# Veason-silverbullet/NNR

Hardware: NVIDIA B200
Metric: cne_sue_train_impressions_per_sec (higher is better)
Workload: dtype f32

## Files before the change

### include/nnr_b200.h

```cpp
#ifndef NNR_B200_H
#define NNR_B200_H
#include <stddef.h>
#include <stdint.h>

#ifdef __cplusplus
extern "C" {
#endif

#define NNR_ABI_VERSION 8
#define NNR_SEED_INDIRECT (1ULL << 62)

const char* nnr_last_error(void);
int nnr_abi_version(void);
uint64_t nnr_launch_count(void);
int nnr_profile_enable(int on);
int nnr_profile_read(double* out, int ntags);

int nnr_seq_prepare(uint8_t* mask, int N, int L, int32_t* len, int32_t* off, int32_t* tok_row,
                    void* stream);

int nnr_embed_gather_fwd(const float* table, const int32_t* ids, const int32_t* len,
                         const int32_t* off, int N, int L, int E, int V, float* out, float p_drop,
                         uint64_t seed, void* stream);
int nnr_embed_gather_planes_fwd(const float* table, const int32_t* ids, const int32_t* len,
                                const int32_t* off, int N, int L, int E, int V, int cap, float p_drop,
                                uint64_t seed, int algo, void* planes, size_t planes_bytes, void* stream);
size_t nnr_embed_gather_bwd_workspace_bytes(int N, int L);
int nnr_embed_gather_bwd(const float* dout, const int32_t* ids, const int32_t* len,
                         const int32_t* off, int N, int L, int E, int V, float p_drop,
                         uint64_t seed, float* dtable, int accumulate, void* workspace,
                         size_t workspace_bytes, void* stream);

enum {
  NNR_EPI_NONE = 0,
  NNR_EPI_BIAS = 1,
  NNR_EPI_BIAS_TANH = 2,
  NNR_EPI_BIAS_RELU_RES = 3,
  NNR_EPI_GATE = 4,
  NNR_EPI_ADD_AUX = 5
};
enum {
  NNR_GEMM_AUTO = 0,
  NNR_GEMM_SIMT_FP32 = 1,
  NNR_GEMM_TC_TF32X3 = 2,
  NNR_GEMM_TC_BF16 = 3,
  NNR_GEMM_TC_BF16X3 = 4
};
typedef struct {
  const float* A; int64_t lda; int32_t transA;
  const float* B; int64_t ldb; int32_t transB;
  float* C; int64_t ldc;
  int32_t M, N, K;
  const int32_t* m_dev;
  const int32_t* k_dev;
  int32_t epilogue;
  int32_t accumulate;
  const float* bias;
  const float* aux; int64_t ldaux;
  float* aux_out; int64_t ldaux_out;
  const float* rowbias; int64_t ldrowbias; const int32_t* rowmap;
  float p_drop; uint64_t seed;
  int32_t algo;
  void* workspace; size_t workspace_bytes;
  const void* A_planes; int64_t a_planes_pitch; int64_t a_planes_rows;
  const void* B_planes; int64_t b_planes_pitch; int64_t b_planes_rows;
  void* C_planes; int64_t c_planes_pitch; int64_t c_planes_rows;
} nnr_gemm_args;
size_t nnr_gemm_workspace_bytes(const nnr_gemm_args* args);
int nnr_gemm(const nnr_gemm_args* args, void* stream);
int64_t nnr_tc_split_pitch(int C, int algo);
size_t nnr_tc_split_bytes(int R, int C, int algo);
int nnr_tc_split(const float* X, int64_t ld, int R, int C, const int32_t* r_dev, int algo, void* planes,
                 size_t planes_bytes, void* stream);
typedef struct nnr_split_desc {
  const float* src; int64_t ld; int32_t rows, cols;
  void* planes; int64_t pitch;
} nnr_split_desc;
int nnr_tc_split_many(const nnr_split_desc* descs, int n, int algo, void* stream);

int nnr_length_sort_desc(const int64_t* keys, int N, int max_key, int64_t* sorted_idx, void* stream);

size_t nnr_tc_split_colsum_workspace_bytes(int R, int C, int algo);
int nnr_tc_split_colsum(const float* X, int64_t ld, int R, int C, const int32_t* r_dev, int algo, void* planes,
                        size_t planes_bytes, float* colsum, int accumulate, void* workspace, size_t workspace_bytes,
                        void* stream);
int nnr_relu_bwd_split_colsum(const float* dy, const float* relu_out, int64_t ld, int R, int C, float p_drop,
                              uint64_t seed, float* dy_dropped, int algo, void* planes, size_t planes_bytes,
                              float* colsum, int accumulate, void* workspace, size_t workspace_bytes,
                              void* stream);
int nnr_gemm_default_algo(void);

size_t nnr_colsum_workspace_bytes(int M, int N);
int nnr_colsum(const float* X, int64_t ldx, int M, int N, const int32_t* m_dev, float* out,
               int accumulate, void* workspace, size_t workspace_bytes, void* stream);
int nnr_segment_colsum(const float* X, int64_t ldx, const int32_t* off, int N, int D, float* out,
                       int64_t ldo, void* stream);

int nnr_lstm_fwd(float* gx, const float* w_hh, const int32_t* len, const int32_t* off,
                 const int32_t* order, int N, int L, int H, float* h_out, float* c_stash,
                 float* c_n, int32_t* tile_counters, void* stream);
int nnr_lstm_bwd(float* gates, const float* c_stash, const float* w_hh, const int32_t* len,
                 const int32_t* off, const int32_t* order, int N, int L, int H, const float* dh,
                 const float* dcn, int32_t* tile_counters, void* stream);
int nnr_lstm_fwd_planes_supported(int H, int algo);
int nnr_lstm_fwd_planes(float* gx, const float* w_hh, const int32_t* len, const int32_t* off, const int32_t* order,
                        int N, int L, int H, float* h_out, float* c_stash, float* c_n, int32_t* tile_counters, int cap,
                        int algo, void* planes, size_t planes_bytes, void* stream);
int nnr_lstm_bwd_planes_supported(int H, int algo);
size_t nnr_lstm_bwd_planes_workspace_bytes(int N, int H);
int nnr_lstm_bwd_planes(const float* gates, const float* c_stash, const float* w_hh, const int32_t* len,
                        const int32_t* off, const int32_t* order, int N, int L, int H, const float* dh,
                        const float* dcn, int32_t* tile_counters, int cap, int algo, void* dz_planes,
                        size_t planes_bytes, float* db, void* workspace, size_t workspace_bytes, void* stream);
int nnr_lstm_shift_h(const float* h, const int32_t* len, const int32_t* off,
                     const int32_t* tok_row, int N, int L, int H, float* hprev, void* stream);
int nnr_lstm_shift_h_planes(const float* h, const int32_t* len, const int32_t* off,
                            const int32_t* tok_row, int N, int L, int H, int cap, int algo, void* planes,
                            size_t planes_bytes, void* stream);
int nnr_gate_bwd_pre(const float* dhg, const float* h, const float* g, int64_t n_max,
                     const int32_t* n_dev, int D, float* dz, float* dh0, void* stream);
int nnr_gate_bwd_planes(const float* dhg, const float* h, const float* g, const int32_t* off, int N, int D,
                        int cap, int algo, void* dz_planes, size_t planes_bytes, float* dh0, float* dmproj,
                        int64_t lddm, void* stream);

typedef struct {
  const float* X; int64_t ldx; int32_t D;
  const int32_t* seg_off; int32_t S; int32_t fixed_len; int32_t max_len;
  int32_t mode;
  const float* U; int64_t ldu; int32_t A; const float* w2;
  const float* qvec; int64_t ldq; float scale;
  const uint8_t* mask;
  float* pooled; int64_t ldp;
  float* alpha;
  const float* dpooled; int64_t lddp;
  float* dX; int64_t lddx; int32_t accumulate_dx;
  float* dU; int64_t lddu;
  float* dw2_partial;
  float* dqvec; int64_t lddq;
  const int32_t* seg_order;
} nnr_pool_args;
int nnr_attn_pool_fwd(const nnr_pool_args* args, void* stream);
int nnr_attn_pool_bwd(const nnr_pool_args* args, void* stream);

int nnr_news_fuse_fwd(const float* t_self, const float* t_cross, const float* c_self,
                      const float* c_cross, const float* cat_table, const float* sub_table,
                      const int32_t* cat, const int32_t* sub, int N, int D2, int Ec, int Es,
                      float p_drop, uint64_t seed, float* out, void* stream);
int nnr_news_fuse_bwd(const float* dout, const int32_t* cat, const int32_t* sub, int N, int D2,
                      int Ec, int Es, int n_cat, int n_sub, float p_drop, uint64_t seed,
                      float* d_a, float* d_b, float* dcat_table, float* dsub_table,
                      int accumulate, void* stream);
int nnr_news_fuse_tables_bwd(const float* dout, const int32_t* cat, const int32_t* sub, int N, int Dout, int col0,
// ... 75 lines not shown
```

### nnr_b200/_lib.py

```python
import ctypes as C
import os

_HERE = os.path.dirname(os.path.abspath(__file__))
LIB_PATH = os.environ.get('NNR_B200_LIB') or os.path.join(_HERE, '_lib', 'libnnr_b200.so')

if not os.path.isfile(LIB_PATH):
    raise ImportError('nnr_b200: CUDA library not built (%s missing). Run nnr_b200/csrc/build.sh or '
                      '__graft_entry__.build(); there is no CPU fallback.' % LIB_PATH)

lib = C.CDLL(LIB_PATH)

vp, i32, i64, u64, f32, sz = C.c_void_p, C.c_int32, C.c_int64, C.c_uint64, C.c_float, C.c_size_t


class GemmArgs(C.Structure):
    _fields_ = [('A', vp), ('lda', i64), ('transA', i32),
                ('B', vp), ('ldb', i64), ('transB', i32),
                ('C', vp), ('ldc', i64),
                ('M', i32), ('N', i32), ('K', i32),
                ('m_dev', vp), ('k_dev', vp),
                ('epilogue', i32), ('accumulate', i32),
                ('bias', vp), ('aux', vp), ('ldaux', i64),
                ('aux_out', vp), ('ldaux_out', i64),
                ('rowbias', vp), ('ldrowbias', i64), ('rowmap', vp),
                ('p_drop', f32), ('seed', u64),
                ('algo', i32),
                ('workspace', vp), ('workspace_bytes', sz),
                ('A_planes', vp), ('a_planes_pitch', i64), ('a_planes_rows', i64),
                ('B_planes', vp), ('b_planes_pitch', i64), ('b_planes_rows', i64),
                ('C_planes', vp), ('c_planes_pitch', i64), ('c_planes_rows', i64)]


class PoolArgs(C.Structure):
    _fields_ = [('X', vp), ('ldx', i64), ('D', i32),
                ('seg_off', vp), ('S', i32), ('fixed_len', i32), ('max_len', i32),
                ('mode', i32),
                ('U', vp), ('ldu', i64), ('A', i32), ('w2', vp),
                ('qvec', vp), ('ldq', i64), ('scale', f32),
                ('mask', vp),
                ('pooled', vp), ('ldp', i64),
                ('alpha', vp),
                ('dpooled', vp), ('lddp', i64),
                ('dX', vp), ('lddx', i64), ('accumulate_dx', i32),
                ('dU', vp), ('lddu', i64),
                ('dw2_partial', vp),
                ('dqvec', vp), ('lddq', i64),
                ('seg_order', vp)]


class SplitDesc(C.Structure):
    _fields_ = [('src', vp), ('ld', i64), ('rows', i32), ('cols', i32), ('planes', vp), ('pitch', i64)]


SIGNATURES = {
    'nnr_last_error': (C.c_char_p, []),
    'nnr_abi_version': (C.c_int, []),
    'nnr_launch_count': (u64, []),
    'nnr_profile_enable': (C.c_int, [C.c_int]),
    'nnr_profile_read': (C.c_int, [C.POINTER(C.c_double), C.c_int]),
    'nnr_seq_prepare': (C.c_int, [vp, C.c_int, C.c_int, vp, vp, vp, vp]),
    'nnr_embed_gather_fwd': (C.c_int, [vp, vp, vp, vp, C.c_int, C.c_int, C.c_int, C.c_int, vp, f32, u64, vp]),
    'nnr_embed_gather_planes_fwd': (C.c_int, [vp, vp, vp, vp, C.c_int, C.c_int, C.c_int, C.c_int, C.c_int, f32, u64, C.c_int, vp, sz, vp]),
    'nnr_embed_gather_bwd_workspace_bytes': (sz, [C.c_int, C.c_int]),
    'nnr_embed_gather_bwd': (C.c_int, [vp, vp, vp, vp, C.c_int, C.c_int, C.c_int, C.c_int, f32, u64, vp, C.c_int, vp, sz, vp]),
    'nnr_gemm_workspace_bytes': (sz, [C.POINTER(GemmArgs)]),
    'nnr_gemm': (C.c_int, [C.POINTER(GemmArgs), vp]),
    'nnr_tc_split_pitch': (i64, [C.c_int, C.c_int]),
    'nnr_tc_split_bytes': (sz, [C.c_int, C.c_int, C.c_int]),
    'nnr_tc_split': (C.c_int, [vp, i64, C.c_int, C.c_int, vp, C.c_int, vp, sz, vp]),
    'nnr_tc_split_colsum_workspace_bytes': (sz, [C.c_int, C.c_int, C.c_int]),
    'nnr_tc_split_colsum': (C.c_int, [vp, i64, C.c_int, C.c_int, vp, C.c_int, vp, sz, vp, C.c_int, vp, sz, vp]),
    'nnr_relu_bwd_split_colsum': (C.c_int, [vp, vp, i64, C.c_int, C.c_int, f32, u64, vp, C.c_int, vp, sz, vp, C.c_int, vp, sz, vp]),
    'nnr_length_sort_desc': (C.c_int, [vp, C.c_int, C.c_int, vp, vp]),
    'nnr_tc_split_many': (C.c_int, [vp, C.c_int, C.c_int, vp]),
    'nnr_gemm_default_algo': (C.c_int, []),
    'nnr_colsum_workspace_bytes': (sz, [C.c_int, C.c_int]),
    'nnr_colsum': (C.c_int, [vp, i64, C.c_int, C.c_int, vp, vp, C.c_int, vp, sz, vp]),
    'nnr_segment_colsum': (C.c_int, [vp, i64, vp, C.c_int, C.c_int, vp, i64, vp]),
    'nnr_lstm_fwd': (C.c_int, [vp, vp, vp, vp, vp, C.c_int, C.c_int, C.c_int, vp, vp, vp, vp, vp]),
    'nnr_lstm_bwd': (C.c_int, [vp, vp, vp, vp, vp, vp, C.c_int, C.c_int, C.c_int, vp, vp, vp, vp]),
    'nnr_lstm_bwd_planes_supported': (C.c_int, [C.c_int, C.c_int]),
    'nnr_lstm_fwd_planes_supported': (C.c_int, [C.c_int, C.c_int]),
    'nnr_lstm_fwd_planes': (C.c_int, [vp, vp, vp, vp, vp, C.c_int, C.c_int, C.c_int, vp, vp, vp, vp, C.c_int, C.c_int, vp, sz, vp]),
    'nnr_lstm_bwd_planes_workspace_bytes': (sz, [C.c_int, C.c_int]),
    'nnr_lstm_bwd_planes': (C.c_int, [vp, vp, vp, vp, vp, vp, C.c_int, C.c_int, C.c_int, vp, vp, vp, C.c_int, C.c_int, vp, sz, vp,
                                      vp, sz, vp]),
    'nnr_lstm_shift_h_planes': (C.c_int, [vp, vp, vp, vp, C.c_int, C.c_int, C.c_int, C.c_int, C.c_int, vp, sz, vp]),
    'nnr_lstm_shift_h': (C.c_int, [vp, vp, vp, vp, C.c_int, C.c_int, C.c_int, vp, vp]),
    'nnr_gate_bwd_planes': (C.c_int, [vp, vp, vp, vp, C.c_int, C.c_int, C.c_int, C.c_int, vp, sz, vp, vp, i64, vp]),
    'nnr_gate_bwd_pre': (C.c_int, [vp, vp, vp, i64, vp, C.c_int, vp, vp, vp]),
    'nnr_attn_pool_fwd': (C.c_int, [C.POINTER(PoolArgs), vp]),
    'nnr_attn_pool_bwd': (C.c_int, [C.POINTER(PoolArgs), vp]),
    'nnr_news_fuse_fwd': (C.c_int, [vp, vp, vp, vp, vp, vp, vp, vp, C.c_int, C.c_int, C.c_int, C.c_int, f32, u64, vp, vp]),
    'nnr_news_fuse_bwd': (C.c_int, [vp, vp, vp, C.c_int, C.c_int, C.c_int, C.c_int, C.c_int, C.c_int, f32, u64, vp, vp, vp, vp, C.c_int, vp]),
    'nnr_news_fuse_tables_bwd': (C.c_int, [vp, vp, vp, C.c_int, C.c_int, C.c_int, C.c_int, C.c_int, C.c_int, C.c_int, f32, u64, vp, vp, C.c_int, vp]),
    'nnr_sue_graph_build': (C.c_int, [vp, vp, C.c_int, C.c_int, C.c_int, vp, vp, vp, vp]),
    'nnr_sue_graph_build_ex': (C.c_int, [vp, vp, C.c_int, C.c_int, C.c_int, C.c_int, vp, vp, vp, vp]),
    'nnr_ln_relu_res_fwd': (C.c_int, [vp, vp, vp, vp, C.c_int, C.c_int, f32, f32, u64, vp, vp, vp, vp, vp]),
    'nnr_ln_relu_res_bwd_workspace_bytes': (sz, [C.c_int, C.c_int]),
    'nnr_ln_relu_res_bwd': (C.c_int, [vp, vp, vp, vp, vp, vp, C.c_int, C.c_int, f32, u64, vp, vp, vp, vp, vp, sz, vp]),
    'nnr_graph_to_csr': (C.c_int, [vp, C.c_int, C.c_int, C.c_int, vp, vp, vp, vp]),
    'nnr_gcn_aggregate': (C.c_int, [vp, vp, vp, vp, C.c_int, C.c_int, C.c_int, vp, vp]),
    'nnr_gcn_aggregate_add': (C.c_int, [vp, vp, vp, vp, C.c_int, C.c_int, C.c_int, vp, vp, vp]),
    'nnr_cluster_intra_fwd': (C.c_int, [vp, vp, vp, vp, C.c_int, C.c_int, C.c_int, C.c_int, C.c_int, C.c_int, f32, vp, vp, vp]),
    'nnr_cluster_intra_bwd': (C.c_int, [vp, vp, vp, vp, vp, vp, C.c_int, C.c_int, C.c_int, C.c_int, C.c_int, C.c_int, f32, vp, vp, vp, vp, C.c_int, vp]),
    'nnr_rowdot_fwd': (C.c_int, [vp, vp, C.c_int, C.c_int, vp, vp]),
    'nnr_rowdot_bwd': (C.c_int, [vp, vp, vp, C.c_int, C.c_int, vp, C.c_int, vp, C.c_int, vp]),
    'nnr_topk_merge': (C.c_int, [vp, i64, C.c_int, C.c_int, i64, vp, vp, vp, C.c_int, C.c_int, C.c_int, vp, vp, vp]),
    'nnr_topk_merge_capped': (C.c_int, [vp, i64, C.c_int, C.c_int, i64, vp, vp, vp, C.c_int, C.c_int, C.c_int, vp, C.c_int,
                                        C.c_int, vp, vp, vp, vp]),
    'nnr_topk_merge_lists': (C.c_int, [vp, i64, C.c_int, C.c_int, vp, i64, C.c_int, C.c_int, vp, vp, vp]),
    'nnr_topk_merge_lists_capped': (C.c_int, [vp, i64, C.c_int, C.c_int, vp, i64, vp, i64, C.c_int, C.c_int, C.c_int, C.c_int,
                                              vp, vp, vp, vp]),
    'nnr_dropout': (C.c_int, [vp, i64, f32, u64, vp, vp]),
    'nnr_flat_clip_adam_workspace_bytes': (sz, [i64]),
    'nnr_flat_clip_adam': (C.c_int, [vp, vp, vp, vp, i64, f32, f32, f32, f32, f32, f32, i32, vp, vp, sz, vp]),
    'nnr_flat_clip_adam_dev': (C.c_int, [vp, vp, vp, vp, i64, f32, f32, f32, f32, f32, f32, vp, vp, vp, sz, vp]),
}

for _name, (_res, _args) in SIGNATURES.items():
    _fn = getattr(lib, _name)
    _fn.restype = _res
    _fn.argtypes = _args


def check(rc, what):
    if rc != 0:
        msg = lib.nnr_last_error()
        raise RuntimeError('%s failed (rc=%d): %s' % (what, rc, msg.decode() if msg else ''))


def launch_count():
    return int(lib.nnr_launch_count())
```

### nnr_b200/csrc/gemm_api.cu

```cuda
#include "common.cuh"
#include "../../include/nnr_b200.h"
#include <stdlib.h>
#include <string.h>

size_t nnr_gemm_simt_workspace_bytes(const nnr_gemm_args* a);
int nnr_gemm_simt(const nnr_gemm_args* a, void* stream);
int nnr_gemm_tc_supported(const nnr_gemm_args* a);
size_t nnr_gemm_tc_workspace_bytes(const nnr_gemm_args* a);
int nnr_gemm_tc(const nnr_gemm_args* a, void* stream);

extern "C" int nnr_gemm_default_algo(void);
static int default_algo() {
  static int algo = -1;
  if (algo < 0) {
    const char* e = getenv("NNR_GEMM_ALGO");
    if (e && !strcmp(e, "simt")) algo = NNR_GEMM_SIMT_FP32;
    else if (e && !strcmp(e, "tf32x3")) algo = NNR_GEMM_TC_TF32X3;
    else if (e && !strcmp(e, "bf16")) algo = NNR_GEMM_TC_BF16;
    else if (e && !strcmp(e, "bf16x3")) algo = NNR_GEMM_TC_BF16X3;
    else algo = NNR_GEMM_TC_BF16X3;
  }
  return algo;
}

static int pick_algo(const nnr_gemm_args* a) {
  int algo = a->algo == NNR_GEMM_AUTO ? default_algo() : a->algo;
  if (algo != NNR_GEMM_SIMT_FP32 && !nnr_gemm_tc_supported(a)) {
    if (a->algo == NNR_GEMM_AUTO) algo = NNR_GEMM_SIMT_FP32;
  }
  return algo;
}

static int validate(const nnr_gemm_args* a) {
  NNR_REQUIRE(a && (a->A || a->A_planes) && (a->B || a->B_planes) && a->C, NNR_ERR_ARG, "nnr_gemm: null operand");
  NNR_REQUIRE(a->M > 0 && a->N > 0 && a->K > 0, NNR_ERR_ARG, "nnr_gemm: bad shape M=%d N=%d K=%d", a->M, a->N, a->K);
  NNR_REQUIRE(a->epilogue >= NNR_EPI_NONE && a->epilogue <= NNR_EPI_ADD_AUX, NNR_ERR_ARG, "nnr_gemm: bad epilogue %d", a->epilogue);
  NNR_REQUIRE(a->lda >= (a->transA ? a->M : a->K), NNR_ERR_ARG, "nnr_gemm: lda too small");
  NNR_REQUIRE(a->ldb >= (a->transB ? a->K : a->N), NNR_ERR_ARG, "nnr_gemm: ldb too small");
  NNR_REQUIRE(a->ldc >= a->N, NNR_ERR_ARG, "nnr_gemm: ldc too small");
  if (a->epilogue == NNR_EPI_BIAS || a->epilogue == NNR_EPI_BIAS_TANH)
    NNR_REQUIRE(a->bias, NNR_ERR_ARG, "nnr_gemm: epilogue needs bias");
  if (a->epilogue == NNR_EPI_GATE)
    NNR_REQUIRE(a->rowbias && a->rowmap && a->aux, NNR_ERR_ARG, "nnr_gemm: gate epilogue needs rowbias,rowmap,aux");
  if (a->epilogue == NNR_EPI_ADD_AUX) NNR_REQUIRE(a->aux, NNR_ERR_ARG, "nnr_gemm: add_aux epilogue needs aux");
  NNR_REQUIRE(a->p_drop >= 0.f && a->p_drop < 1.f, NNR_ERR_ARG, "nnr_gemm: p_drop=%f", a->p_drop);
  return 0;
}

extern "C" int nnr_gemm_default_algo(void) { return default_algo(); }

extern "C" size_t nnr_gemm_workspace_bytes(const nnr_gemm_args* a) {
  if (!a || a->M <= 0 || a->N <= 0 || a->K <= 0) return 0;
  size_t s = nnr_gemm_simt_workspace_bytes(a);
  nnr_gemm_args b = *a;
  b.algo = pick_algo(a);
  size_t t = (b.algo != NNR_GEMM_SIMT_FP32 && nnr_gemm_tc_supported(a)) ? nnr_gemm_tc_workspace_bytes(&b) : 0;
  return s > t ? s : t;
}

extern "C" int nnr_gemm(const nnr_gemm_args* a, void* stream) {
  int rc = validate(a);
  if (rc) return rc;
  int algo = pick_algo(a);
  if (algo == NNR_GEMM_SIMT_FP32) {
    NNR_REQUIRE(a->A && a->B, NNR_ERR_UNSUPPORTED, "nnr_gemm: an operand given only as planes needs the tensor-core path");
    NNR_REQUIRE(!a->C_planes, NNR_ERR_UNSUPPORTED, "nnr_gemm: C_planes needs the tensor-core path");
    return nnr_gemm_simt(a, stream);
  }
  NNR_REQUIRE(nnr_gemm_tc_supported(a), NNR_ERR_UNSUPPORTED, "nnr_gemm: tensor-core path does not support this shape/layout");
  nnr_gemm_args b = *a;
  b.algo = algo;
  return nnr_gemm_tc(&b, stream);
}
```

### nnr_b200/csrc/gemm_tc.cu

```cuda
#include "common.cuh"
#include "gemm_epilogue.cuh"
#include <cuda.h>
#include <cuda_bf16.h>

extern "C" int nnr_gemm_default_algo(void);

#define TC_BM 128
#define TC_THREADS 320
#define TC_TMEM_COLS 512
#define TC_ACC_COLS 256
#define TC_EPI_PITCH 80
#define TC_EPI_SCRATCH (8 * 32 * TC_EPI_PITCH)
#define TC_SMEM_BUDGET (205 * 1024)
#define TC_CHAIN_K 2048

__device__ __forceinline__ uint32_t smem_u32(const void* p) { return (uint32_t)__cvta_generic_to_shared(p); }

__device__ __forceinline__ void mbar_init(uint64_t* bar, uint32_t count) {
  asm volatile("mbarrier.init.shared::cta.b64 [%0], %1;" ::"r"(smem_u32(bar)), "r"(count));
}
__device__ __forceinline__ void mbar_expect_tx(uint64_t* bar, uint32_t bytes) {
  asm volatile("mbarrier.arrive.expect_tx.shared::cta.b64 _, [%0], %1;" ::"r"(smem_u32(bar)), "r"(bytes) : "memory");
}
__device__ __forceinline__ void mbar_arrive(uint64_t* bar) {
// ... 32 lines not shown
        "r"(accumulate)
        : "memory");
  } else {
    asm volatile(
        "{\n.reg .pred p;\nsetp.ne.b32 p, %4, 0;\n"
        "tcgen05.mma.cta_group::1.kind::tf32 [%0], %1, %2, %3, p;\n}\n" ::"r"(d_tmem), "l"(a_desc), "l"(b_desc), "r"(idesc),
        "r"(accumulate)
        : "memory");
  }
}
__device__ __forceinline__ uint32_t cluster_ctarank() {
  uint32_t r;
  asm volatile("mov.u32 %0, %%cluster_ctarank;" : "=r"(r));
  return r;
}
__device__ __forceinline__ uint32_t mapa_rank(uint32_t addr, uint32_t rank) {
  uint32_t r;
  asm volatile("mapa.shared::cluster.u32 %0, %1, %2;" : "=r"(r) : "r"(addr), "r"(rank));
  return r;
}
__device__ __forceinline__ void cluster_sync_all() {
  asm volatile("barrier.cluster.arrive.release.aligned;\nbarrier.cluster.wait.acquire.aligned;" ::: "memory");
}
__device__ __forceinline__ void tma_load_3d_pair(const CUtensorMap* map, uint32_t leader_bar, uint32_t dst, int c0, int c1, int c2) {
  asm volatile(
      "cp.async.bulk.tensor.3d.cta_group::2.shared::cluster.global.mbarrier::complete_tx::bytes [%0], [%1, {%3, %4, %5}], [%2];"
      ::"r"(dst), "l"(map), "r"(leader_bar), "r"(c0), "r"(c1), "r"(c2)
      : "memory");
}
__device__ __forceinline__ void tc_commit_pair(uint64_t* bar) {
  asm volatile("tcgen05.commit.cta_group::2.mbarrier::arrive::one.shared::cluster.multicast::cluster.b64 [%0], %1;" ::"r"(smem_u32(bar)),
               "h"((uint16_t)3)
               : "memory");
}
__device__ __forceinline__ void mbar_arrive_cluster(uint32_t cluster_addr) {
  asm volatile("mbarrier.arrive.release.cluster.shared::cluster.b64 _, [%0];" ::"r"(cluster_addr) : "memory");
}
template <bool BF16>
__device__ __forceinline__ void tc_mma_pair(uint32_t d_tmem, uint64_t a_desc, uint64_t b_desc, uint32_t idesc, uint32_t accumulate) {
  if (BF16) {
    asm volatile(
        "{\n.reg .pred p;\nsetp.ne.b32 p, %4, 0;\n"
        "tcgen05.mma.cta_group::2.kind::f16 [%0], %1, %2, %3, p;\n}\n" ::"r"(d_tmem), "l"(a_desc), "l"(b_desc), "r"(idesc),
        "r"(accumulate)
        : "memory");
  } else {
    asm volatile(
        "{\n.reg .pred p;\nsetp.ne.b32 p, %4, 0;\n"
        "tcgen05.mma.cta_group::2.kind::tf32 [%0], %1, %2, %3, p;\n}\n" ::"r"(d_tmem), "l"(a_desc), "l"(b_desc), "r"(idesc),
        "r"(accumulate)
        : "memory");
  }
}

__device__ __forceinline__ void tmem_ld16(uint32_t taddr, float* v) {
  uint32_t r[16];
  asm volatile(
      "tcgen05.ld.sync.aligned.32x32b.x16.b32 {%0, %1, %2, %3, %4, %5, %6, %7, %8, %9, %10, %11, %12, %13, %14, %15}, [%16];"
      : "=r"(r[0]), "=r"(r[1]), "=r"(r[2]), "=r"(r[3]), "=r"(r[4]), "=r"(r[5]), "=r"(r[6]), "=r"(r[7]), "=r"(r[8]), "=r"(r[9]),
        "=r"(r[10]), "=r"(r[11]), "=r"(r[12]), "=r"(r[13]), "=r"(r[14]), "=r"(r[15])
      : "r"(taddr));
  asm volatile("tcgen05.wait::ld.sync.aligned;" ::: "memory");
#pragma unroll
  for (int i = 0; i < 16; ++i) v[i] = __uint_as_float(r[i]);
}

__device__ __forceinline__ uint64_t make_sw128_desc(uint32_t smem_addr, uint32_t lbo_bytes, uint32_t sbo_bytes, uint32_t layout_type) {
  uint64_t d = 0;
  d |= (uint64_t)((smem_addr & 0x3FFFF) >> 4);
  d |= (uint64_t)((lbo_bytes >> 4) & 0x3FFF) << 16;
  d |= (uint64_t)((sbo_bytes >> 4) & 0x3FFF) << 32;
  d |= (uint64_t)1 << 46;
  d |= (uint64_t)layout_type << 61;
  return d;
}

#ifdef NNR_TC_PROF
__device__ unsigned long long g_tc_prof[16];
#define TC_STAMP(i) { if (blockIdx.x == 0) g_tc_prof[i] = clock64(); }
#else
#define TC_STAMP(i) {}
#endif

struct TcParams {
  int M, N, K;
  const int32_t* m_dev;
  const int32_t* k_dev;
  int block_n, stages, nplanes;
  int a_mn, b_mn;
  int split_k;
  int chain_kb;
  uint32_t idesc;
  float* partial;
  int epi_fast;
  __nv_bfloat16* c_planes;
  long long c_pitch, c_pstride;
  int c_lo, c_rows;
  EpiP epi;
};

__device__ __forceinline__ bool al16(const void* p) { return (((uintptr_t)p) & 15) == 0; }

__device__ __forceinline__ void ld4(const float* p, int cnt, float* o) {
  if (cnt == 4 && al16(p)) {
    const float4 t = __ldg(reinterpret_cast<const float4*>(p));
    o[0] = t.x; o[1] = t.y; o[2] = t.z; o[3] = t.w;
  } else {
#pragma unroll
    for (int i = 0; i < 4; ++i) o[i] = (i < cnt) ? __ldg(p + i) : 0.f;
  }
}
__device__ __forceinline__ void st4(float* p, int cnt, const float* o) {
  if (cnt == 4 && al16(p)) {
    *reinterpret_cast<float4*>(p) = make_float4(o[0], o[1], o[2], o[3]);
  } else {
#pragma unroll
    for (int i = 0; i < 4; ++i) if (i < cnt) p[i] = o[i];
  }
}
struct Epi4In { float rb[4], ax[4], cc[4]; };
__device__ __forceinline__ void epi_load4(const EpiP& e, int m, int n, int cnt, Epi4In& in, int rmap) {
  if (e.epilogue == NNR_EPI_GATE) {
    ld4(e.rowbias + (size_t)rmap * e.ldrowbias + n, cnt, in.rb);
    ld4(e.aux + (size_t)m * e.ldaux + n, cnt, in.ax);
  } else if (e.epilogue == NNR_EPI_ADD_AUX || (e.epilogue == NNR_EPI_BIAS_RELU_RES && e.aux)) {
    ld4(e.aux + (size_t)m * e.ldaux + n, cnt, in.ax);
  }
  if (e.accumulate) ld4(e.C + (size_t)m * e.ldc + n, cnt, in.cc);
}
__device__ __forceinline__ void epi_finish4(const EpiP& e, int m, int n, float* v, int cnt, const float* bias4, const Epi4In& in) {
  if (e.epilogue == NNR_EPI_BIAS || e.epilogue == NNR_EPI_BIAS_TANH || e.epilogue == NNR_EPI_BIAS_RELU_RES) {
#pragma unroll
    for (int i = 0; i < 4; ++i) v[i] += bias4[i];
  }
  if (e.epilogue == NNR_EPI_BIAS_TANH) {
#pragma unroll
    for (int i = 0; i < 4; ++i) v[i] = tanh_fast(v[i]);
  } else if (e.epilogue == NNR_EPI_BIAS_RELU_RES) {
#pragma unroll
    for (int i = 0; i < 4; ++i) v[i] = fmaxf(v[i], 0.f);
    if (e.aux_out) st4(e.aux_out + (size_t)m * e.ldaux_out + n, cnt, v);
    if (e.aux) {
#pragma unroll
      for (int i = 0; i < 4; ++i) v[i] += in.ax[i];
    }
    if (e.p_drop > 0.f) {
      const uint64_t seed = nnr_resolve_seed(e.seed);
#pragma unroll
      for (int i = 0; i < 4; ++i) v[i] *= dropout_scale(seed, (uint64_t)m * (uint64_t)e.N + n + i, e.p_drop, e.inv_keep);
    }
  } else if (e.epilogue == NNR_EPI_GATE) {
#pragma unroll
    for (int i = 0; i < 4; ++i) v[i] = sigmoid_fast(v[i] + in.rb[i]);
    if (e.aux_out) st4(e.aux_out + (size_t)m * e.ldaux_out + n, cnt, v);
#pragma unroll
    for (int i = 0; i < 4; ++i) v[i] *= in.ax[i];
  } else if (e.epilogue == NNR_EPI_ADD_AUX) {
#pragma unroll
    for (int i = 0; i < 4; ++i) v[i] += in.ax[i];
  }
  if (e.accumulate) {
#pragma unroll
    for (int i = 0; i < 4; ++i) v[i] += in.cc[i];
  }
  st4(e.C + (size_t)m * e.ldc + n, cnt, v);
}

__device__ __forceinline__ void sts128(uint32_t a, uint32_t x, uint32_t y, uint32_t z, uint32_t w) {
  asm volatile("st.shared.v4.b32 [%0], {%1, %2, %3, %4};" ::"r"(a), "r"(x), "r"(y), "r"(z), "r"(w) : "memory");
}
__device__ __forceinline__ float4 lds128(uint32_t a) {
  float4 v;
  asm volatile("ld.shared.v4.f32 {%0, %1, %2, %3}, [%4];" : "=f"(v.x), "=f"(v.y), "=f"(v.z), "=f"(v.w) : "r"(a) : "memory");
  return v;
}
__device__ __forceinline__ void tmem_ld16_issue(uint32_t taddr, uint32_t (&r)[16]) {
  asm volatile(
      "tcgen05.ld.sync.aligned.32x32b.x16.b32 {%0, %1, %2, %3, %4, %5, %6, %7, %8, %9, %10, %11, %12, %13, %14, %15}, [%16];"
      : "=r"(r[0]), "=r"(r[1]), "=r"(r[2]), "=r"(r[3]), "=r"(r[4]), "=r"(r[5]), "=r"(r[6]), "=r"(r[7]), "=r"(r[8]), "=r"(r[9]),
        "=r"(r[10]), "=r"(r[11]), "=r"(r[12]), "=r"(r[13]), "=r"(r[14]), "=r"(r[15])
      : "r"(taddr));
}
__device__ __forceinline__ void tmem_ld16_wait(uint32_t (&r)[16]) {
  asm volatile("tcgen05.wait::ld.sync.aligned;"
               : "+r"(r[0]), "+r"(r[1]), "+r"(r[2]), "+r"(r[3]), "+r"(r[4]), "+r"(r[5]), "+r"(r[6]), "+r"(r[7]), "+r"(r[8]), "+r"(r[9]),
                 "+r"(r[10]), "+r"(r[11]), "+r"(r[12]), "+r"(r[13]), "+r"(r[14]), "+r"(r[15])
               :
               : "memory");
}

struct EpiTile {
  uint32_t o_c[4], o_aux[4], o_ao[4], o_rb[4];
  uint32_t rvalid;
  int row0;
};
template <int EP>
__device__ __forceinline__ void epi_load_in(const TcParams& p, const EpiTile& t, int n, bool has_bias, bool need_ax, bool acc_early,
                                            float4 (&ax)[4], float4 (&rb)[4], float4& bb) {
  bb = make_float4(0.f, 0.f, 0.f, 0.f);
#pragma unroll
  for (int i = 0; i < 4; ++i) { ax[i] = make_float4(0.f, 0.f, 0.f, 0.f); rb[i] = make_float4(0.f, 0.f, 0.f, 0.f); }
  if (n < p.N) {
    if (has_bias) bb = __ldg(reinterpret_cast<const float4*>(p.epi.bias + n));
#pragma unroll
    for (int i = 0; i < 4; ++i) {
      if (t.rvalid & (1u << i)) {
        if (need_ax) ax[i] = __ldg(reinterpret_cast<const float4*>(p.epi.aux + t.o_aux[i] + n));
        else if (acc_early) ax[i] = *reinterpret_cast<const float4*>(p.epi.C + t.o_c[i] + n);
        if (EP == NNR_EPI_GATE) rb[i] = __ldg(reinterpret_cast<const float4*>(p.epi.rowbias + t.o_rb[i] + n));
      }
    }
  }
}

#define TC_EPK_PARTIAL 6
template <int EP>
__device__ __forceinline__ void epi_tile_fast(const TcParams& p, const EpiTile& t, uint32_t lane_addr, bool has_k, int c_begin, int c_end,
                                              int n0, uint32_t tile_s, int lane, int M, uint64_t drop_seed, float* __restrict__ Cout) {
  const int tr = lane >> 2, tc4 = (lane & 3) * 4;
  constexpr bool PARTIAL = EP == TC_EPK_PARTIAL;
  constexpr bool BIASED = EP == NNR_EPI_BIAS || EP == NNR_EPI_BIAS_TANH || EP == NNR_EPI_BIAS_RELU_RES;
  const bool has_bias = BIASED && p.epi.bias != nullptr;
  const bool need_ax = EP == NNR_EPI_GATE || EP == NNR_EPI_ADD_AUX || (EP == NNR_EPI_BIAS_RELU_RES && p.epi.aux != nullptr);
  const bool accumulate = !PARTIAL && p.epi.accumulate != 0;
  const bool acc_early = accumulate && !need_ax;
  const bool planes = !PARTIAL && p.c_planes != nullptr;
  const bool drop = EP == NNR_EPI_BIAS_RELU_RES && p.epi.p_drop > 0.f;
  const uint32_t my_row = tile_s + (uint32_t)lane * TC_EPI_PITCH;
  const uint32_t rd_row = tile_s + (uint32_t)tr * TC_EPI_PITCH + (uint32_t)tc4 * 4;

  constexpr bool AHEAD = EP != NNR_EPI_GATE;
  uint32_t r[16];
  float4 ax[4], rb[4], bb, axn[4], rbn[4], bbn;
  if (has_k) tmem_ld16_issue(lane_addr + (uint32_t)c_begin, r);
  if (AHEAD) epi_load_in<EP>(p, t, n0 + c_begin + tc4, has_bias, need_ax, acc_early, ax, rb, bb);
  for (int c0 = c_begin; c0 < c_end; c0 += 16) {
    const bool more = c0 + 16 < c_end;
    if (AHEAD) { if (more) epi_load_in<EP>(p, t, n0 + c0 + 16 + tc4, has_bias, need_ax, acc_early, axn, rbn, bbn); }
    else epi_load_in<EP>(p, t, n0 + c0 + tc4, has_bias, need_ax, acc_early, ax, rb, bb);
    if (has_k) tmem_ld16_wait(r);
    else {
#pragma unroll
      for (int i = 0; i < 16; ++i) r[i] = 0u;
    }
#pragma unroll
    for (int qd = 0; qd < 4; ++qd) sts128(my_row + qd * 16, r[4 * qd], r[4 * qd + 1], r[4 * qd + 2], r[4 * qd + 3]);
    if (has_k && more) tmem_ld16_issue(lane_addr + (uint32_t)(c0 + 16), r);
    __syncwarp();
    float4 o[4];
#pragma unroll
    for (int i = 0; i < 4; ++i) o[i] = lds128(rd_row + (uint32_t)(8 * i) * TC_EPI_PITCH);
    const int n = n0 + c0 + tc4;
    if (n < p.N) {
#pragma unroll
      for (int i = 0; i < 4; ++i) {
        if (!(t.rvalid & (1u << i))) continue;
        float4 v = make_float4(o[i].x + bb.x, o[i].y + bb.y, o[i].z + bb.z, o[i].w + bb.w);
        if (EP == NNR_EPI_BIAS_TANH) {
          v.x = tanh_fast(v.x); v.y = tanh_fast(v.y); v.z = tanh_fast(v.z); v.w = tanh_fast(v.w);
        } else if (EP == NNR_EPI_BIAS_RELU_RES) {
          v.x = fmaxf(v.x, 0.f); v.y = fmaxf(v.y, 0.f); v.z = fmaxf(v.z, 0.f); v.w = fmaxf(v.w, 0.f);
          if (p.epi.aux_out) *reinterpret_cast<float4*>(p.epi.aux_out + t.o_ao[i] + n) = v;
          if (need_ax) { v.x += ax[i].x; v.y += ax[i].y; v.z += ax[i].z; v.w += ax[i].w; }
          if (drop) {
            const uint64_t e0 = (uint64_t)(t.row0 + 8 * i) * (uint64_t)p.epi.N + n;
            float ks[4];
            dropout_scale4(drop_seed, e0 >> 2, p.epi.p_drop, p.epi.inv_keep, ks);
            v.x *= ks[0]; v.y *= ks[1]; v.z *= ks[2]; v.w *= ks[3];
          }
        } else if (EP == NNR_EPI_GATE) {
          v.x = sigmoid_fast(v.x + rb[i].x); v.y = sigmoid_fast(v.y + rb[i].y);
          v.z = sigmoid_fast(v.z + rb[i].z); v.w = sigmoid_fast(v.w + rb[i].w);
          if (p.epi.aux_out) *reinterpret_cast<float4*>(p.epi.aux_out + t.o_ao[i] + n) = v;
          v.x *= ax[i].x; v.y *= ax[i].y; v.z *= ax[i].z; v.w *= ax[i].w;
        } else if (EP == NNR_EPI_ADD_AUX) {
          v.x += ax[i].x; v.y += ax[i].y; v.z += ax[i].z; v.w += ax[i].w;
        }
        if (acc_early) { v.x += ax[i].x; v.y += ax[i].y; v.z += ax[i].z; v.w += ax[i].w; }
        else if (accumulate) {
          const float4 cc = *reinterpret_cast<const float4*>(Cout + t.o_c[i] + n);
          v.x += cc.x; v.y += cc.y; v.z += cc.z; v.w += cc.w;
        }
        *reinterpret_cast<float4*>(Cout + t.o_c[i] + n) = v;
        if (planes) {
          const __nv_bfloat162 h01 = __floats2bfloat162_rn(v.x, v.y), h23 = __floats2bfloat162_rn(v.z, v.w);
          __nv_bfloat16* op = p.c_planes + (long long)(t.row0 + 8 * i) * p.c_pitch + n;
          uint2 hv;
          hv.x = *reinterpret_cast<const uint32_t*>(&h01); hv.y = *reinterpret_cast<const uint32_t*>(&h23);
          *reinterpret_cast<uint2*>(op) = hv;
          if (p.c_lo) {
            const __nv_bfloat162 l01 = __floats2bfloat162_rn(v.x - __low2float(h01), v.y - __high2float(h01));
            const __nv_bfloat162 l23 = __floats2bfloat162_rn(v.z - __low2float(h23), v.w - __high2float(h23));
            uint2 lv;
            lv.x = *reinterpret_cast<const uint32_t*>(&l01); lv.y = *reinterpret_cast<const uint32_t*>(&l23);
            *reinterpret_cast<uint2*>(op + p.c_pstride) = lv;
          }
        }
      }
      if (planes) {
        const int mz = min(p.c_rows, (M + 63) & ~63);
#pragma unroll
        for (int i = 0; i < 4; ++i) {
          const int mm = t.row0 + 8 * i;
          if (mm >= M && mm < mz) {
            __nv_bfloat16* op = p.c_planes + (long long)mm * p.c_pitch + n;
            *reinterpret_cast<uint2*>(op) = make_uint2(0u, 0u);
            if (p.c_lo) *reinterpret_cast<uint2*>(op + p.c_pstride) = make_uint2(0u, 0u);
          }
        }
      }
    }
    __syncwarp();
    if (AHEAD && more) {
      bb = bbn;
#pragma unroll
      for (int i = 0; i < 4; ++i) { ax[i] = axn[i]; rb[i] = rbn[i]; }
    }
  }
}

template <bool BF16, bool PAIR, int EPK>
__global__ void __launch_bounds__(TC_THREADS, 1) gemm_tc_kernel(const __grid_constant__ CUtensorMap map_a,
                                                                const __grid_constant__ CUtensorMap map_b, TcParams p) {
  extern __shared__ __align__(1024) unsigned char smem_raw[];
  constexpr int KELEM = BF16 ? 64 : 32;
  constexpr int TILE_M = PAIR ? 2 * TC_BM : TC_BM;
  int M = p.M, K = p.K;
  if (p.m_dev) M = min(M, *p.m_dev);
  if (p.k_dev) K = min(K, *p.k_dev);
  const int warp = threadIdx.x >> 5, lane = threadIdx.x & 31;
  if (threadIdx.x == 0) TC_STAMP(0)
  const uint32_t rank = PAIR ? cluster_ctarank() : 0u;
  const int sched_id = PAIR ? (int)(blockIdx.x >> 1) : (int)blockIdx.x;
  const int sched_n = PAIR ? (int)(gridDim.x >> 1) : (int)gridDim.x;
  const int b_rows = PAIR ? (p.block_n >> 1) : p.block_n;

  const int m_tiles = (M + TILE_M - 1) / TILE_M;
  const int n_tiles = (p.N + p.block_n - 1) / p.block_n;
  const int nkb = (K + KELEM - 1) / KELEM;
  const int kb_per = p.split_k ? p.chain_kb : max(nkb, 1);
  const int splits = p.split_k ? max(1, (nkb + kb_per - 1) / kb_per) : 1;
  const int total_tiles = m_tiles * n_tiles * splits;

  const uint32_t a_tile = TC_BM * 128, b_tile = (uint32_t)b_rows * 128;
  const uint32_t stage_bytes = (uint32_t)p.nplanes * (a_tile + b_tile);
  unsigned char* tiles = (unsigned char*)(((uintptr_t)smem_raw + 1023) & ~(uintptr_t)1023);
  unsigned char* epi_scratch = tiles + (size_t)p.stages * stage_bytes;
  uint64_t* full_bar = reinterpret_cast<uint64_t*>(epi_scratch + TC_EPI_SCRATCH);
  uint64_t* empty_bar = full_bar + p.stages;
  uint64_t* tmem_full = empty_bar + p.stages;
  uint64_t* tmem_empty = tmem_full + 2;
  uint32_t* tmem_slot = reinterpret_cast<uint32_t*>(tmem_empty + 2);

  if (warp == 0 && lane == 0) {
    asm volatile("prefetch.tensormap [%0];" ::"l"(&map_a) : "memory");
    asm volatile("prefetch.tensormap [%0];" ::"l"(&map_b) : "memory");
    for (int s = 0; s < p.stages; ++s) { mbar_init(&full_bar[s], 1); mbar_init(&empty_bar[s], 1); }
    for (int b = 0; b < 2; ++b) { mbar_init(&tmem_full[b], 1); mbar_init(&tmem_empty[b], PAIR ? 16 : 8); }
    asm volatile("fence.mbarrier_init.release.cluster;" ::: "memory");
  }
  if (PAIR) cluster_sync_all();
  if (warp == 1) {
    if (PAIR) {
      asm volatile("tcgen05.alloc.cta_group::2.sync.aligned.shared::cta.b32 [%0], %1;" ::"r"(smem_u32(tmem_slot)), "n"(TC_TMEM_COLS) : "memory");
      asm volatile("tcgen05.relinquish_alloc_permit.cta_group::2.sync.aligned;" ::: "memory");
    } else {
      asm volatile("tcgen05.alloc.cta_group::1.sync.aligned.shared::cta.b32 [%0], %1;" ::"r"(smem_u32(tmem_slot)), "n"(TC_TMEM_COLS) : "memory");
      asm volatile("tcgen05.relinquish_alloc_permit.cta_group::1.sync.aligned;" ::: "memory");
    }
  }
  tc_fence_before();
  __syncthreads();
  tc_fence_after();
  const uint32_t tmem_base = *tmem_slot;
  if (threadIdx.x == 0) TC_STAMP(1)

  if (warp == 0) {
    if (lane == 0) {
      int it = 0;
      for (int tile = sched_id; tile < total_tiles; tile += sched_n) {
        const int n_idx = tile % n_tiles, rest = tile / n_tiles;
        const int m0 = (rest % m_tiles) * TILE_M + (int)rank * TC_BM, n0 = n_idx * p.block_n + (int)rank * b_rows, z = rest / m_tiles;
        const int kb0 = z * kb_per, kb1 = min(nkb, kb0 + kb_per);
        for (int kb = kb0; kb < kb1; ++kb, ++it) {
          const int s = it % p.stages;
          const uint32_t ph = (it / p.stages) & 1;
          mbar_wait(&empty_bar[s], ph ^ 1);
          const uint32_t base = smem_u32(tiles + (size_t)s * stage_bytes);
          if (!PAIR) mbar_expect_tx(&full_bar[s], stage_bytes);
          else if (rank == 0) mbar_expect_tx(&full_bar[s], 2 * stage_bytes);
          const uint32_t lbar = PAIR ? mapa_rank(smem_u32(&full_bar[s]), 0) : 0u;
          auto load_a = [&](uint32_t dst, int c0, int c1, int c2) {
            if (PAIR) tma_load_3d_pair(&map_a, lbar, dst, c0, c1, c2); else tma_load_3d(&map_a, &full_bar[s], dst, c0, c1, c2);
          };
          auto load_b = [&](uint32_t dst, int c0, int c1, int c2) {
            if (PAIR) tma_load_3d_pair(&map_b, lbar, dst, c0, c1, c2); else tma_load_3d(&map_b, &full_bar[s], dst, c0, c1, c2);
          };
          for (int pl = 0; pl < p.nplanes; ++pl) {
            const uint32_t sa = base + pl * a_tile;
            const uint32_t sb = base + p.nplanes * a_tile + pl * b_tile;
            if (!p.a_mn) load_a(sa, kb * KELEM, m0, pl);
            else for (int g = 0; g < TC_BM / KELEM; ++g) load_a(sa + g * (KELEM * 128), m0 + g * KELEM, kb * KELEM, pl);
            if (!p.b_mn) load_b(sb, kb * KELEM, n0, pl);
            else for (int g = 0; g < b_rows / KELEM; ++g) load_b(sb + g * (KELEM * 128), n0 + g * KELEM, kb * KELEM, pl);
          }
        }
      }
    }
  } else if (warp == 1) {
    if (lane == 0 && rank == 0) {
      int it = 0, tl = 0;
      const uint32_t lbo = KELEM * 128;
      const uint64_t a_step = p.a_mn ? (uint64_t)((BF16 ? 2048 : 1024) >> 4) : 2;
      const uint64_t b_step = p.b_mn ? (uint64_t)((BF16 ? 2048 : 1024) >> 4) : 2;
      for (int tile = sched_id; tile < total_tiles; tile += sched_n, ++tl) {
        const int rest = tile / n_tiles;
        const int z = rest / m_tiles;
        const int kb0 = z * kb_per, kb1 = min(nkb, kb0 + kb_per);
        const int buf = tl & 1;
        mbar_wait(&tmem_empty[buf], ((tl >> 1) & 1) ^ 1);
        tc_fence_after();
        const uint32_t d_tmem = tmem_base + buf * TC_ACC_COLS;
        uint32_t first = 1;
        for (int kb = kb0; kb < kb1; ++kb, ++it) {
          const int s = it % p.stages;
          mbar_wait(&full_bar[s], (it / p.stages) & 1);
          tc_fence_after();
          if (it == 0) TC_STAMP(2)
          const uint32_t base = smem_u32(tiles + (size_t)s * stage_bytes);
          const uint32_t a_lt = (p.a_mn && !BF16) ? 1u : 2u, a_sbo = (p.a_mn && !BF16) ? 512u : 1024u;
          const uint32_t b_lt = (p.b_mn && !BF16) ? 1u : 2u, b_sbo = (p.b_mn && !BF16) ? 512u : 1024u;
          const uint64_t a_hi = make_sw128_desc(base, p.a_mn ? lbo : 0, a_sbo, a_lt);
          const uint64_t a_lo = make_sw128_desc(base + a_tile, p.a_mn ? lbo : 0, a_sbo, a_lt);
          const uint64_t b_hi = make_sw128_desc(base + p.nplanes * a_tile, p.b_mn ? lbo : 0, b_sbo, b_lt);
          const uint64_t b_lo = make_sw128_desc(base + p.nplanes * a_tile + b_tile, p.b_mn ? lbo : 0, b_sbo, b_lt);
#pragma unroll
          for (int k = 0; k < 4; ++k) {
            const uint64_t ao = a_step * k, bo = b_step * k;
            if (PAIR) tc_mma_pair<BF16>(d_tmem, a_hi + ao, b_hi + bo, p.idesc, first ? 0u : 1u);
            else tc_mma<BF16>(d_tmem, a_hi + ao, b_hi + bo, p.idesc, first ? 0u : 1u);
            first = 0;
            if (p.nplanes == 2) {
              if (PAIR) {
                tc_mma_pair<BF16>(d_tmem, a_hi + ao, b_lo + bo, p.idesc, 1u);
                tc_mma_pair<BF16>(d_tmem, a_lo + ao, b_hi + bo, p.idesc, 1u);
              } else {
                tc_mma<BF16>(d_tmem, a_hi + ao, b_lo + bo, p.idesc, 1u);
                tc_mma<BF16>(d_tmem, a_lo + ao, b_hi + bo, p.idesc, 1u);
              }
            }
          }
          if (PAIR) tc_commit_pair(&empty_bar[s]); else tc_commit(&empty_bar[s]);
        }
        if (tl < 2) TC_STAMP(3 + tl)
        if (PAIR) tc_commit_pair(&tmem_full[buf]); else tc_commit(&tmem_full[buf]);
      }
    }
  } else {
    const int q = warp & 3;
    const int chalf = (warp - 2) >> 2;
    const uint64_t drop_seed = (p.epi.p_drop > 0.f) ? nnr_resolve_seed(p.epi.seed) : 0ull;
    const int nchunks = p.block_n >> 4;
    const int c_begin = chalf ? ((nchunks + 1) >> 1) << 4 : 0;
    const int c_end = chalf ? p.block_n : ((nchunks + 1) >> 1) << 4;
    int tl = 0;
    for (int tile = sched_id; tile < total_tiles; tile += sched_n, ++tl) {
      const int n_idx = tile % n_tiles, rest = tile / n_tiles;
      const int m0 = (rest % m_tiles) * TILE_M + (int)rank * TC_BM, n0 = n_idx * p.block_n, z = rest / m_tiles;
      const int kb0 = z * kb_per, kb1 = min(nkb, kb0 + kb_per);
      const int buf = tl & 1;
      const uint32_t lane_addr = tmem_base + buf * TC_ACC_COLS + ((uint32_t)(q * 32) << 16);
      unsigned char* my_tile = epi_scratch + (size_t)(warp - 2) * 32 * TC_EPI_PITCH;
      const int tr = lane >> 2, tc4 = (lane & 3) * 4;
      int rmap[4] = {0, 0, 0, 0};
      if ((EPK < 0 || EPK == NNR_EPI_GATE) && p.epi.epilogue == NNR_EPI_GATE && !p.partial) {
#pragma unroll
        for (int i = 0; i < 4; ++i) {
          const int mm = m0 + q * 32 + tr + 8 * i;
          if (mm < M) rmap[i] = __ldg(p.epi.rowmap + mm);
        }
      }
      const bool fast = EPK >= 0;
      uint32_t o_c[4], o_aux[4], o_ao[4], o_rb[4];
      uint32_t rvalid = 0;
      if (fast) {
#pragma unroll
        for (int i = 0; i < 4; ++i) {
          const int mm = m0 + q * 32 + tr + 8 * i;
          if (mm < M) rvalid |= 1u << i;
          const uint32_t mr = (mm < M) ? (uint32_t)mm : 0u;
          o_c[i] = (EPK == TC_EPK_PARTIAL) ? ((uint32_t)z * (uint32_t)M + mr) * (uint32_t)p.N : mr * (uint32_t)p.epi.ldc;
          o_aux[i] = mr * (uint32_t)p.epi.ldaux;
          o_ao[i] = mr * (uint32_t)p.epi.ldaux_out;
          o_rb[i] = (uint32_t)rmap[i] * (uint32_t)p.epi.ldrowbias;
        }
      }
      mbar_wait(&tmem_full[buf], (tl >> 1) & 1);
      tc_fence_after();
      if (warp == 2 && lane == 0 && tl < 2) TC_STAMP(5 + 2 * tl)
      if (EPK >= 0) {
        EpiTile et;
#pragma unroll
        for (int i = 0; i < 4; ++i) { et.o_c[i] = o_c[i]; et.o_aux[i] = o_aux[i]; et.o_ao[i] = o_ao[i]; et.o_rb[i] = o_rb[i]; }
        et.rvalid = rvalid; et.row0 = m0 + q * 32 + tr;
        epi_tile_fast<(EPK >= 0 ? EPK : 0)>(p, et, lane_addr, kb1 > kb0, c_begin, c_end, n0, smem_u32(my_tile), lane, M, drop_seed,
                                            EPK == TC_EPK_PARTIAL ? p.partial : p.epi.C);
      } else
      for (int c0 = c_begin; c0 < c_end; c0 += 16) {
        float v[16];
        if (kb1 > kb0) tmem_ld16(lane_addr + (uint32_t)c0, v);
        else {
#pragma unroll
          for (int i = 0; i < 16; ++i) v[i] = 0.f;
        }
#pragma unroll
        for (int qd = 0; qd < 4; ++qd)
          *reinterpret_cast<float4*>(my_tile + lane * TC_EPI_PITCH + qd * 16) = make_float4(v[4 * qd], v[4 * qd + 1], v[4 * qd + 2], v[4 * qd + 3]);
        __syncwarp();
        const int n = n0 + c0 + tc4;
        const int cnt = min(4, p.N - n);
        float o[4][4];
#pragma unroll
        for (int i = 0; i < 4; ++i) {
          const float4 x = *reinterpret_cast<const float4*>(my_tile + (tr + 8 * i) * TC_EPI_PITCH + tc4 * 4);
          o[i][0] = x.x; o[i][1] = x.y; o[i][2] = x.z; o[i][3] = x.w;
        }
        if (cnt > 0) {
          if (p.partial) {
#pragma unroll
            for (int i = 0; i < 4; ++i) {
              const int mm = m0 + q * 32 + tr + 8 * i;
              if (mm < M) st4(p.partial + ((size_t)z * M + mm) * p.N + n, cnt, o[i]);
            }
          } else {
            Epi4In in[4];
            float bias4[4] = {0.f, 0.f, 0.f, 0.f};
            if (p.epi.bias && (p.epi.epilogue == NNR_EPI_BIAS || p.epi.epilogue == NNR_EPI_BIAS_TANH || p.epi.epilogue == NNR_EPI_BIAS_RELU_RES))
              ld4(p.epi.bias + n, cnt, bias4);
#pragma unroll
            for (int i = 0; i < 4; ++i) {
              const int mm = m0 + q * 32 + tr + 8 * i;
              if (mm < M) epi_load4(p.epi, mm, n, cnt, in[i], rmap[i]);
            }
#pragma unroll
            for (int i = 0; i < 4; ++i) {
              const int mm = m0 + q * 32 + tr + 8 * i;
              if (mm < M) epi_finish4(p.epi, mm, n, o[i], cnt, bias4, in[i]);
            }
          }
        }
        __syncwarp();
      }
      tc_fence_before();
      __syncwarp();
      if (warp == 2 && lane == 0 && tl < 2) TC_STAMP(6 + 2 * tl)
      if (lane == 0) {
        if (PAIR && rank != 0) mbar_arrive_cluster(mapa_rank(smem_u32(&tmem_empty[buf]), 0));
        else mbar_arrive(&tmem_empty[buf]);
      }
    }
  }
  tc_fence_before();
  __syncthreads();
  if (threadIdx.x == 0) TC_STAMP(9)
  if (PAIR) cluster_sync_all();
  if (warp == 1) {
    if (PAIR) asm volatile("tcgen05.dealloc.cta_group::2.sync.aligned.b32 %0, %1;" ::"r"(tmem_base), "n"(TC_TMEM_COLS) : "memory");
    else asm volatile("tcgen05.dealloc.cta_group::1.sync.aligned.b32 %0, %1;" ::"r"(tmem_base), "n"(TC_TMEM_COLS) : "memory");
  }
}

__global__ void tc_splitk_reduce_kernel(const float* __restrict__ partial, int K, const int32_t* __restrict__ k_dev, int kelem,
                                        int chain_kb, int M, int N, const int32_t* __restrict__ m_dev, EpiP epi) {
  if (m_dev) M = min(M, *m_dev);
  if (k_dev) K = min(K, *k_dev);
  const int nkb = (K + kelem - 1) / kelem;
  const int splits = max(1, (nkb + chain_kb - 1) / chain_kb);
  size_t i = (size_t)blockIdx.x * blockDim.x + threadIdx.x;
  if (i >= (size_t)M * N) return;
  int m = (int)(i / N), n = (int)(i - (size_t)m * N);
  float acc = 0.f;
  for (int s = 0; s < splits; ++s) acc += partial[((size_t)s * M + m) * N + n];
  epi_store(epi, m, n, acc);
}
__global__ void __launch_bounds__(256) tc_splitk_reduce4_kernel(const float* __restrict__ partial, int K, const int32_t* __restrict__ k_dev,
                                                                int kelem, int chain_kb, int M, int N, const int32_t* __restrict__ m_dev,
                                                                EpiP epi) {
  if (m_dev) M = min(M, *m_dev);
  if (k_dev) K = min(K, *k_dev);
  const int nkb = (K + kelem - 1) / kelem;
  const int splits = max(1, (nkb + chain_kb - 1) / chain_kb);
  const int N4 = N >> 2;
  const size_t i = (size_t)blockIdx.x * blockDim.x + threadIdx.x;
  if (i >= (size_t)M * N4) return;
  const int m = (int)(i / N4), n = (int)(i - (size_t)m * N4) * 4;
  const size_t plane = (size_t)M * N;
  const float* src = partial + (size_t)m * N + n;
  float4 acc = make_float4(0.f, 0.f, 0.f, 0.f);
  int s = 0;
  for (; s + 4 <= splits; s += 4) {
    float4 v[4];
#pragma unroll
    for (int u = 0; u < 4; ++u) v[u] = __ldg(reinterpret_cast<const float4*>(src + (size_t)(s + u) * plane));
#pragma unroll
    for (int u = 0; u < 4; ++u) { acc.x += v[u].x; acc.y += v[u].y; acc.z += v[u].z; acc.w += v[u].w; }
  }
  for (; s < splits; ++s) {
    const float4 v = __ldg(reinterpret_cast<const float4*>(src + (size_t)s * plane));
    acc.x += v.x; acc.y += v.y; acc.z += v.z; acc.w += v.w;
  }
  float o[4] = {acc.x, acc.y, acc.z, acc.w};
  float bias4[4] = {0.f, 0.f, 0.f, 0.f};
  if (epi.bias && (epi.epilogue == NNR_EPI_BIAS || epi.epilogue == NNR_EPI_BIAS_TANH || epi.epilogue == NNR_EPI_BIAS_RELU_RES))
    ld4(epi.bias + n, 4, bias4);
  Epi4In in;
  epi_load4(epi, m, n, 4, in, epi.epilogue == NNR_EPI_GATE ? __ldg(epi.rowmap + m) : 0);
  epi_finish4(epi, m, n, o, 4, bias4, in);
}

__device__ __forceinline__ float rna_tf32(float x) {
  uint32_t r;
  asm("cvt.rna.tf32.f32 %0, %1;" : "=r"(r) : "f"(x));
  return __uint_as_float(r);
}
template <int MODE>
__global__ void __launch_bounds__(256) tc_split_kernel(const float* __restrict__ src, int64_t ld, int R, int C, int Cp,
                                                       const int32_t* __restrict__ r_dev, bool vec, void* __restrict__ out,
                                                       size_t plane_stride) {
  int Rv = R;
  if (r_dev) Rv = min(R, *r_dev);
  const int Rw = r_dev ? min(R, (Rv + 63) / 64 * 64) : R;
  const int cq_per_row = Cp >> 2;
  const long long total = (long long)Rw * cq_per_row;
  const long long stride = (long long)gridDim.x * blockDim.x;
  for (long long i0 = (long long)blockIdx.x * blockDim.x + threadIdx.x; i0 < total; i0 += 4 * stride) {
    float4 x[4];
    int rr[4], cc[4];
#pragma unroll
    for (int u = 0; u < 4; ++u) {
      const long long i = i0 + u * stride;
      x[u] = make_float4(0.f, 0.f, 0.f, 0.f);
      rr[u] = -1;
      if (i < total) {
        const int r = (int)(i / cq_per_row), cq = (int)(i - (long long)r * cq_per_row) * 4;
        rr[u] = r; cc[u] = cq;
        if (r < Rv) {
          const float* sp = src + (size_t)r * ld + cq;
          if (vec && cq + 3 < C) x[u] = __ldg(reinterpret_cast<const float4*>(sp));
          else {
            if (cq < C) x[u].x = __ldg(sp);
            if (cq + 1 < C) x[u].y = __ldg(sp + 1);
            if (cq + 2 < C) x[u].z = __ldg(sp + 2);
            if (cq + 3 < C) x[u].w = __ldg(sp + 3);
          }
        }
      }
    }
#pragma unroll
    for (int u = 0; u < 4; ++u) {
      if (rr[u] < 0) continue;
      if (MODE >= 1) {
        __nv_bfloat16* ob = reinterpret_cast<__nv_bfloat16*>(out) + (size_t)rr[u] * Cp + cc[u];
        __nv_bfloat162* o = reinterpret_cast<__nv_bfloat162*>(ob);
        const __nv_bfloat162 h01 = __floats2bfloat162_rn(x[u].x, x[u].y), h23 = __floats2bfloat162_rn(x[u].z, x[u].w);
        o[0] = h01;
        o[1] = h23;
        if (MODE == 2) {
          __nv_bfloat162* l = reinterpret_cast<__nv_bfloat162*>(ob + plane_stride);
          l[0] = __floats2bfloat162_rn(x[u].x - __low2float(h01), x[u].y - __high2float(h01));
          l[1] = __floats2bfloat162_rn(x[u].z - __low2float(h23), x[u].w - __high2float(h23));
        }
      } else {
        float* hi = reinterpret_cast<float*>(out) + (size_t)rr[u] * Cp + cc[u];
        float4 h, l;
        h.x = rna_tf32(x[u].x); h.y = rna_tf32(x[u].y); h.z = rna_tf32(x[u].z); h.w = rna_tf32(x[u].w);
        l.x = rna_tf32(x[u].x - h.x); l.y = rna_tf32(x[u].y - h.y); l.z = rna_tf32(x[u].z - h.z); l.w = rna_tf32(x[u].w - h.w);
        *reinterpret_cast<float4*>(hi) = h;
        *reinterpret_cast<float4*>(hi + plane_stride) = l;
// ... 87 lines not shown
                }
              }
            }
          }
        }
      }
#pragma unroll
      for (int u = 0; u < 4; ++u) {
        const int r = rb + u * RS;
        if (r >= r1) continue;
#pragma unroll
        for (int j = 0; j < TCS_MAXG; ++j) {
          const int cq = (g + j * G) * 4;
          if (cq >= Cp) continue;
          tc_split_store4<MODE>(out, plane_stride, Cp, r, cq, x[u][j]);
          acc[j].x += x[u][j].x; acc[j].y += x[u][j].y; acc[j].z += x[u][j].z; acc[j].w += x[u][j].w;
        }
      }
    }
  }
  for (int j = 0; j < TCS_MAXG; ++j) {
    __syncthreads();
    if (active) s_acc[rs * G + g] = acc[j];
    __syncthreads();
    const int cq = (g + j * G) * 4;
    if (rs == 0 && cq < Cp) {
      float4 t = s_acc[g];
      for (int q = 1; q < RS; ++q) { const float4 o = s_acc[q * G + g]; t.x += o.x; t.y += o.y; t.z += o.z; t.w += o.w; }
      float* dst = partial + (size_t)blockIdx.x * Cp + cq;
      *reinterpret_cast<float4*>(dst) = t;
    }
  }
}
__global__ void __launch_bounds__(512) tc_split_colsum_reduce(const float* __restrict__ partial, int nblocks, int R, int C, int Cp,
                                                              const int32_t* __restrict__ r_dev, float* __restrict__ out, int accumulate) {
  __shared__ float s_sum[16][33];
  const int cl = threadIdx.x & 31, sl = threadIdx.x >> 5;
  const int c = blockIdx.x * 32 + cl;
  int Rv = R;
  if (r_dev) Rv = min(R, *r_dev);
  const int nb = min(nblocks, (Rv + tcs_rows(R) - 1) / tcs_rows(R));
  float a0 = 0.f, a1 = 0.f;
  if (c < C) {
    int b = sl;
    for (; b + 16 < nb; b += 32) { a0 += partial[(size_t)b * Cp + c]; a1 += partial[(size_t)(b + 16) * Cp + c]; }
    if (b < nb) a0 += partial[(size_t)b * Cp + c];
  }
  s_sum[sl][cl] = a0 + a1;
  __syncthreads();
  if (sl == 0 && c < C) {
    float acc = 0.f;
#pragma unroll
    for (int q = 0; q < 16; ++q) acc += s_sum[q][cl];
    out[c] = accumulate ? out[c] + acc : acc;
  }
}

typedef CUresult (*EncodeTiledFn)(CUtensorMap*, CUtensorMapDataType, cuuint32_t, void*, const cuuint64_t*, const cuuint64_t*,
                                  const cuuint32_t*, const cuuint32_t*, CUtensorMapInterleave, CUtensorMapSwizzle,
                                  CUtensorMapL2promotion, CUtensorMapFloatOOBfill);
static EncodeTiledFn get_encode() {
  static EncodeTiledFn fn = nullptr;
  static bool tried = false;
  if (!tried) {
    tried = true;
    void* p = nullptr;
    cudaDriverEntryPointQueryResult q;
    if (cudaGetDriverEntryPoint("cuTensorMapEncodeTiled", &p, cudaEnableDefault, &q) == cudaSuccess && q == cudaDriverEntryPointSuccess)
      fn = (EncodeTiledFn)p;
    else (void)cudaGetLastError();
  }
  return fn;
}

static size_t up(size_t x, size_t a) { return (x + a - 1) / a * a; }

struct TcPlan {
  bool bf16;
  int a_mn, b_mn;
  int a_rows, a_cols, b_rows, b_cols;
  int a_cp, b_cp;
  int block_n, stages, split_k, chain_kb, max_splits, nplanes, kelem;
  int pair;
  size_t a_plane, b_plane, a_off, b_off, partial_off, total, smem;
};

static int pick_block_n(int N, int step, int nplanes) {
  int best = step;
  double best_cost = 1e30;
  for (int bn = 256; bn >= 32; bn -= step) {
    double padded = (double)((N + bn - 1) / bn) * bn;
    double cost = padded * (1.0 + 40.0 / bn);
    size_t stage = (size_t)nplanes * ((size_t)TC_BM * 128 + (size_t)bn * 128);
    if (TC_SMEM_BUDGET / stage < 3) cost *= 1.3;
    if (cost < best_cost - 1e-9) { best_cost = cost; best = bn; }
  }
  return best;
}

static int pick_block_n_pair(int N, int step, int nplanes) {
  int best = 0;
  double best_cost = 1e30;
  for (int bn = 256; bn >= 64; bn -= step) {
    size_t stage = (size_t)nplanes * ((size_t)TC_BM * 128 + (size_t)(bn / 2) * 128);
    if (TC_SMEM_BUDGET / stage < 3) continue;
    double padded = (double)((N + bn - 1) / bn) * bn;
    if (padded > 1.15 * N) continue;
    double cost = padded * (1.0 + 40.0 / bn);
    if (cost < best_cost - 1e-9) { best_cost = cost; best = bn; }
  }
  return best;
}

static int algo_mode(int algo) {
  if (algo == NNR_GEMM_AUTO) algo = nnr_gemm_default_algo();
  return algo == NNR_GEMM_TC_BF16 ? 1 : (algo == NNR_GEMM_TC_BF16X3 ? 2 : 0);
}
static TcPlan make_plan(const nnr_gemm_args* a, int mode) {
  TcPlan pl;
  const bool bf16 = mode != 0;
  pl.bf16 = bf16;
  pl.kelem = bf16 ? 64 : 32;
  pl.nplanes = mode == 1 ? 1 : 2;
  pl.a_mn = a->transA ? 1 : 0;
  pl.b_mn = a->transB ? 0 : 1;
  pl.a_rows = a->transA ? a->K : a->M; pl.a_cols = a->transA ? a->M : a->K;
  pl.b_rows = a->transB ? a->N : a->K; pl.b_cols = a->transB ? a->K : a->N;
  const size_t pad = bf16 ? 8 : 4;
  pl.a_cp = (int)up((size_t)pl.a_cols, pad);
  pl.b_cp = (int)up((size_t)pl.b_cols, pad);
  pl.block_n = pick_block_n(a->N, pl.b_mn ? pl.kelem : 16, pl.nplanes);
  pl.pair = 0;
  if (a->M >= 2 * TC_BM * 148 && !(a->transA) && a->k_dev == nullptr) {
    int bnp = pick_block_n_pair(a->N, pl.b_mn ? 2 * pl.kelem : 16, pl.nplanes);
    if (bnp) { pl.pair = 1; pl.block_n = bnp; }
  }
  long tiles = (long)((a->M + TC_BM - 1) / TC_BM) * ((a->N + pl.block_n - 1) / pl.block_n);
  int nkb_cap = (a->K + pl.kelem - 1) / pl.kelem;
  pl.split_k = 0;
  pl.chain_kb = TC_CHAIN_K / pl.kelem;
  if (!pl.pair && tiles * 2 <= 148 && nkb_cap >= 8) {
    int target = (int)((148 + tiles - 1) / tiles);
    int chain = (nkb_cap + target - 1) / target;
    if (chain < 4) chain = 4;
    if (chain > TC_CHAIN_K / pl.kelem) chain = TC_CHAIN_K / pl.kelem;
    if (chain < nkb_cap) { pl.split_k = 1; pl.chain_kb = chain; }
  }
  pl.max_splits = pl.split_k ? (nkb_cap + pl.chain_kb - 1) / pl.chain_kb : 1;
  size_t stage = (size_t)pl.nplanes * ((size_t)TC_BM * 128 + (size_t)(pl.pair ? pl.block_n / 2 : pl.block_n) * 128);
  int stages = (int)(TC_SMEM_BUDGET / stage);
  if (stages < 2) stages = 2;
  if (stages > 6) stages = 6;
  pl.stages = stages;
  pl.smem = 1024 + (size_t)stages * stage + TC_EPI_SCRATCH + (2 * stages + 4) * 8 + 16;
  const size_t esz = bf16 ? 2 : 4;
  pl.a_plane = (size_t)pl.a_rows * pl.a_cp;
  pl.b_plane = (size_t)pl.b_rows * pl.b_cp;
  size_t o = 0;
  pl.a_off = o; if (!a->A_planes) o = up(o + pl.a_plane * esz * pl.nplanes, 1024);
  pl.b_off = o; if (!a->B_planes) o = up(o + pl.b_plane * esz * pl.nplanes, 1024);
  pl.partial_off = o;
  if (pl.split_k) o = up(o + (size_t)pl.max_splits * a->M * a->N * sizeof(float), 1024);
  pl.total = o;
  return pl;
}

int nnr_gemm_tc_supported(const nnr_gemm_args* a) {
  if (!get_encode()) return 0;
  if ((double)a->M * a->N * a->K < 2.0e6 && a->A && a->B) return 0;
  if (a->K < 8) return 0;
  if (a->m_dev && a->transA) return 0;
  if (a->k_dev && !(a->transA && !a->transB)) return 0;
  return 1;
}

size_t nnr_gemm_tc_workspace_bytes(const nnr_gemm_args* a) { return make_plan(a, algo_mode(a->algo)).total; }

static int encode_map(CUtensorMap* map, const void* base, bool bf16, int cols, int64_t pitch, int rows, int64_t plane_rows,
                      int nplanes, int box_c, int box_r, bool mn) {
  cuuint64_t gdim[3] = {(cuuint64_t)cols, (cuuint64_t)rows, (cuuint64_t)nplanes};
  const size_t esz = bf16 ? 2 : 4;
  cuuint64_t gstr[2] = {(cuuint64_t)pitch * esz, (cuuint64_t)pitch * esz * (cuuint64_t)plane_rows};
  cuuint32_t box[3] = {(cuuint32_t)box_c, (cuuint32_t)box_r, 1};
  cuuint32_t estr[3] = {1, 1, 1};
  CUresult r = get_encode()(map, bf16 ? CU_TENSOR_MAP_DATA_TYPE_BFLOAT16 : CU_TENSOR_MAP_DATA_TYPE_FLOAT32, 3, const_cast<void*>(base), gdim, gstr,
                            box, estr, CU_TENSOR_MAP_INTERLEAVE_NONE,
                            (mn && !bf16) ? CU_TENSOR_MAP_SWIZZLE_128B_ATOM_32B : CU_TENSOR_MAP_SWIZZLE_128B,
                            CU_TENSOR_MAP_L2_PROMOTION_L2_256B, CU_TENSOR_MAP_FLOAT_OOB_FILL_NONE);
  if (r != CUDA_SUCCESS) { nnr_set_error("nnr_gemm(tc): cuTensorMapEncodeTiled failed (%d)", (int)r); return NNR_ERR_ARG; }
  return 0;
}

template <int MODE>
static int split_operand(const float* X, int64_t ld, int R, int C, int Cp, const int32_t* r_dev, void* out, size_t plane_stride,
                         cudaStream_t st) {
  bool vec = nnr_aligned16(X) && (ld % 4 == 0);
  long long total = (long long)R * (Cp / 4);
  long long want = (total + 256 * 4 - 1) / (256 * 4);
  int grid = (int)(want < 148 * 16 ? want : 148 * 16);
  if (grid < 1) grid = 1;
  void* ph = nnr_prof_begin(1, 0.0, st);
  tc_split_kernel<MODE><<<grid, 256, 0, st>>>(X, ld, R, C, Cp, r_dev, vec, out, plane_stride);
  nnr_prof_end(ph, st);
  NNR_LAUNCH_CHECK("tc_split_kernel");
  return 0;
}

template <bool BF16, bool PAIR>
static const void* tc_kernel_ptr2(int epk) {
  if (!BF16) return (const void*)gemm_tc_kernel<BF16, PAIR, -1>;
  switch (epk) {
    case NNR_EPI_NONE: return (const void*)gemm_tc_kernel<BF16, PAIR, BF16 ? NNR_EPI_NONE : -1>;
    case NNR_EPI_BIAS: return (const void*)gemm_tc_kernel<BF16, PAIR, BF16 ? NNR_EPI_BIAS : -1>;
    case NNR_EPI_BIAS_TANH: return (const void*)gemm_tc_kernel<BF16, PAIR, BF16 ? NNR_EPI_BIAS_TANH : -1>;
    case NNR_EPI_BIAS_RELU_RES: return (const void*)gemm_tc_kernel<BF16, PAIR, BF16 ? NNR_EPI_BIAS_RELU_RES : -1>;
    case NNR_EPI_GATE: return (const void*)gemm_tc_kernel<BF16, PAIR, BF16 ? NNR_EPI_GATE : -1>;
    case NNR_EPI_ADD_AUX: return (const void*)gemm_tc_kernel<BF16, PAIR, BF16 ? NNR_EPI_ADD_AUX : -1>;
    case TC_EPK_PARTIAL: return (const void*)gemm_tc_kernel<BF16, PAIR, BF16 ? TC_EPK_PARTIAL : -1>;
    default: return (const void*)gemm_tc_kernel<BF16, PAIR, -1>;
  }
}
template <bool BF16>
static const void* tc_kernel_ptr(bool pair, int epk) {
  return pair ? tc_kernel_ptr2<BF16, true>(epk) : tc_kernel_ptr2<BF16, false>(epk);
}

template <int MODE>
static int run_tc(const nnr_gemm_args* a, cudaStream_t st) {
  constexpr bool BF16 = MODE != 0;
  TcPlan pl = make_plan(a, MODE);
  NNR_REQUIRE(pl.total == 0 || (a->workspace && a->workspace_bytes >= pl.total), NNR_ERR_WORKSPACE,
              "nnr_gemm(tc): workspace %zu < %zu", a->workspace_bytes, pl.total);
  NNR_REQUIRE(nnr_aligned16(a->workspace), NNR_ERR_ALIGN, "nnr_gemm(tc): workspace must be 16B aligned");
  NNR_REQUIRE(nnr_aligned16(a->A_planes) && nnr_aligned16(a->B_planes) && a->a_planes_pitch % (BF16 ? 8 : 4) == 0 &&
                  a->b_planes_pitch % (BF16 ? 8 : 4) == 0,
              NNR_ERR_ALIGN, "nnr_gemm(tc): operand planes must be 16B aligned with a 16B pitch");
  NNR_REQUIRE(pl.smem <= 227 * 1024, NNR_ERR_UNSUPPORTED, "nnr_gemm(tc): smem plan too large");
  char* ws = (char*)a->workspace;
  const void* pa = a->A_planes;
  const void* pb = a->B_planes;
  int64_t a_pitch = a->a_planes_pitch, a_prow = a->a_planes_rows, b_pitch = a->b_planes_pitch, b_prow = a->b_planes_rows;
  int rc;
  if (!pa) {
    void* w = ws + pl.a_off;
    rc = split_operand<MODE>(a->A, a->lda, pl.a_rows, pl.a_cols, pl.a_cp, pl.a_mn ? a->k_dev : a->m_dev, w, pl.a_plane, st);
    if (rc) return rc;
    pa = w; a_pitch = pl.a_cp; a_prow = pl.a_rows;
  }
  if (!pb) {
    void* w = ws + pl.b_off;
    rc = split_operand<MODE>(a->B, a->ldb, pl.b_rows, pl.b_cols, pl.b_cp, pl.b_mn ? a->k_dev : nullptr, w, pl.b_plane, st);
    if (rc) return rc;
    pb = w; b_pitch = pl.b_cp; b_prow = pl.b_rows;
  }
  CUtensorMap map_a, map_b;
  const int ke = pl.kelem;
  rc = encode_map(&map_a, pa, BF16, pl.a_cols, a_pitch, pl.a_rows, a_prow, pl.nplanes, ke, pl.a_mn ? ke : TC_BM, pl.a_mn != 0);
  if (rc) return rc;
  rc = encode_map(&map_b, pb, BF16, pl.b_cols, b_pitch, pl.b_rows, b_prow, pl.nplanes, ke,
                  pl.b_mn ? ke : (pl.pair ? pl.block_n / 2 : pl.block_n), pl.b_mn != 0);
  if (rc) return rc;
  TcParams p;
  p.M = a->M; p.N = a->N; p.K = a->K; p.m_dev = a->m_dev; p.k_dev = a->k_dev;
  p.block_n = pl.block_n; p.stages = pl.stages; p.nplanes = pl.nplanes;
  p.a_mn = pl.a_mn; p.b_mn = pl.b_mn; p.split_k = pl.split_k; p.chain_kb = pl.chain_kb;
  const uint32_t fmt = BF16 ? 1u : 2u;
  p.idesc = (1u << 4) | (fmt << 7) | (fmt << 10) | ((uint32_t)pl.a_mn << 15) | ((uint32_t)pl.b_mn << 16) |
            ((uint32_t)(pl.block_n >> 3) << 17) | ((uint32_t)((pl.pair ? 2 * TC_BM : TC_BM) >> 4) << 24);
  p.partial = pl.split_k ? (float*)(ws + pl.partial_off) : nullptr;
  p.epi = make_epi(a);
  {
    auto ok = [](const void* ptr, int64_t ld) { return !ptr || (nnr_aligned16(ptr) && ld % 4 == 0); };
    p.epi_fast = (a->N % 4 == 0) && ok(a->C, a->ldc) && ok(a->aux, a->ldaux) && ok(a->aux_out, a->ldaux_out) &&
                 ok(a->rowbias, a->ldrowbias) && ok(a->bias, 4);
    if (a->epilogue == NNR_EPI_GATE && !(a->rowbias && a->rowmap && a->aux)) p.epi_fast = 0;
    if (a->epilogue == NNR_EPI_ADD_AUX && !a->aux) p.epi_fast = 0;
    const double lim = 4294967296.0;
    if ((double)a->M * (double)a->ldc >= lim || (double)a->M * (double)a->ldaux >= lim || (double)a->M * (double)a->ldaux_out >= lim ||
        (double)a->M * (double)a->ldrowbias >= lim)
      p.epi_fast = 0;
  }
  p.c_planes = nullptr; p.c_pitch = 0; p.c_pstride = 0; p.c_lo = 0; p.c_rows = 0;
  if (a->C_planes) {
    NNR_REQUIRE(BF16 && p.epi_fast && !pl.split_k && a->N % 8 == 0 && a->c_planes_pitch >= a->N && a->c_planes_pitch % 8 == 0 &&
                    a->c_planes_rows >= a->M && nnr_aligned16(a->C_planes),
                NNR_ERR_UNSUPPORTED, "nnr_gemm: C_planes needs a bf16 tensor-core algo, N %% 8 == 0, aligned epilogue operands, no split-K");
    p.c_planes = (__nv_bfloat16*)a->C_planes;
    p.c_pitch = a->c_planes_pitch;
    p.c_pstride = a->c_planes_rows * a->c_planes_pitch;
    p.c_lo = pl.nplanes == 2;
    p.c_rows = (int)a->c_planes_rows;
  }
  static bool attr_set[16][2][2][8] = {};
  static int num_sms_tab[16] = {};
  int dev = 0;
  NNR_CUDA(cudaGetDevice(&dev));
  dev &= 15;
  int epk = (BF16 && p.epi_fast && !pl.split_k) ? a->epilogue : -1;
  if (BF16 && pl.split_k && a->N % 4 == 0 && nnr_aligned16(p.partial) &&
      (double)pl.max_splits * (double)a->M * (double)a->N < 4294967296.0)
    epk = TC_EPK_PARTIAL;
  const void* kernel = tc_kernel_ptr<BF16>(pl.pair != 0, epk);
  if (!attr_set[dev][BF16 ? 1 : 0][pl.pair][epk + 1]) {
    NNR_CUDA(cudaFuncSetAttribute(kernel, cudaFuncAttributeMaxDynamicSharedMemorySize, 227 * 1024));
    attr_set[dev][BF16 ? 1 : 0][pl.pair][epk + 1] = true;
  }
  if (num_sms_tab[dev] == 0) NNR_CUDA(cudaDeviceGetAttribute(&num_sms_tab[dev], cudaDevAttrMultiProcessorCount, dev));
  const int num_sms = num_sms_tab[dev];
  void* ph = nnr_prof_begin(0, -1.0, st);
  {
    cudaLaunchConfig_t cfg = {};
    cudaLaunchAttribute attr[1];
    if (pl.pair) {
      long cap_tiles = (long)((a->M + 2 * TC_BM - 1) / (2 * TC_BM)) * ((a->N + pl.block_n - 1) / pl.block_n);
      long pairs = cap_tiles < num_sms / 2 ? cap_tiles : num_sms / 2;
      attr[0].id = cudaLaunchAttributeClusterDimension;
      attr[0].val.clusterDim.x = 2; attr[0].val.clusterDim.y = 1; attr[0].val.clusterDim.z = 1;
      cfg.attrs = attr; cfg.numAttrs = 1;
      cfg.gridDim = dim3((unsigned)(2 * pairs));
    } else {
      long cap_tiles = (long)((a->M + TC_BM - 1) / TC_BM) * ((a->N + pl.block_n - 1) / pl.block_n) * pl.max_splits;
      cfg.gridDim = dim3((unsigned)(cap_tiles < num_sms ? cap_tiles : num_sms));
    }
    cfg.blockDim = dim3(TC_THREADS); cfg.dynamicSmemBytes = pl.smem; cfg.stream = st;
    void* kargs[] = {(void*)&map_a, (void*)&map_b, (void*)&p};
    cudaError_t e = cudaLaunchKernelExC(&cfg, kernel, kargs);
    nnr_count_launch(1);
    if (e != cudaSuccess) { nnr_set_error("gemm_tc_kernel(%s): launch failed: %s", pl.pair ? "pair" : "single", cudaGetErrorString(e)); return (int)e; }
    nnr_prof_end(ph, st);
  }
  if (pl.split_k) {
    size_t tot = (size_t)a->M * a->N;
    void* ph2 = nnr_prof_begin(2, 0.0, st);
    if (a->N % 4 == 0 && nnr_aligned16(p.partial))
      tc_splitk_reduce4_kernel<<<(unsigned)((tot / 4 + 255) / 256), 256, 0, st>>>(p.partial, a->K, a->k_dev, pl.kelem, pl.chain_kb, a->M,
                                                                                 a->N, a->m_dev, p.epi);
    else
      tc_splitk_reduce_kernel<<<(unsigned)((tot + 255) / 256), 256, 0, st>>>(p.partial, a->K, a->k_dev, pl.kelem, pl.chain_kb, a->M,
                                                                            a->N, a->m_dev, p.epi);
    nnr_prof_end(ph2, st);
    NNR_LAUNCH_CHECK("tc_splitk_reduce_kernel");
  }
  return 0;
}

int nnr_gemm_tc(const nnr_gemm_args* a, void* stream) {
  cudaStream_t st = (cudaStream_t)stream;
  const int mode = algo_mode(a->algo);
  if (mode == 1) return run_tc<1>(a, st);
  if (mode == 2) return run_tc<2>(a, st);
  return run_tc<0>(a, st);
}

extern "C" int64_t nnr_tc_split_pitch(int C, int algo) { return (int64_t)up((size_t)C, algo_mode(algo) ? 8 : 4); }
extern "C" size_t nnr_tc_split_bytes(int R, int C, int algo) {
  if (R <= 0 || C <= 0) return 0;
  const int mode = algo_mode(algo);
  return (size_t)R * (size_t)nnr_tc_split_pitch(C, algo) * (mode == 0 ? 8 : (mode == 1 ? 2 : 4));
}
extern "C" int nnr_tc_split(const float* X, int64_t ld, int R, int C, const int32_t* r_dev, int algo, void* planes,
                            size_t planes_bytes, void* stream) {
  NNR_REQUIRE(X && planes && R > 0 && C > 0 && ld >= C, NNR_ERR_ARG, "nnr_tc_split: bad arguments");
  NNR_REQUIRE(planes_bytes >= nnr_tc_split_bytes(R, C, algo), NNR_ERR_WORKSPACE, "nnr_tc_split: planes buffer too small");
  NNR_REQUIRE(nnr_aligned16(planes), NNR_ERR_ALIGN, "nnr_tc_split: planes must be 16B aligned");
  const int mode = algo_mode(algo);
  int Cp = (int)nnr_tc_split_pitch(C, algo);
  if (mode == 1) return split_operand<1>(X, ld, R, C, Cp, r_dev, planes, (size_t)R * Cp, (cudaStream_t)stream);
  if (mode == 2) return split_operand<2>(X, ld, R, C, Cp, r_dev, planes, (size_t)R * Cp, (cudaStream_t)stream);
  return split_operand<0>(X, ld, R, C, Cp, r_dev, planes, (size_t)R * Cp, (cudaStream_t)stream);
}

extern "C" size_t nnr_tc_split_colsum_workspace_bytes(int R, int C, int algo) {
  if (R <= 0 || C <= 0) return 0;
  return (size_t)((R + tcs_rows(R) - 1) / tcs_rows(R)) * (size_t)nnr_tc_split_pitch(C, algo) * sizeof(float);
}
extern "C" int nnr_tc_split_colsum(const float* X, int64_t ld, int R, int C, const int32_t* r_dev, int algo, void* planes,
                                   size_t planes_bytes, float* colsum, int accumulate, void* workspace, size_t workspace_bytes,
                                   void* stream) {
  NNR_REQUIRE(X && planes && colsum && workspace && R > 0 && C > 0 && ld >= C, NNR_ERR_ARG, "nnr_tc_split_colsum: bad arguments");
  NNR_REQUIRE(planes_bytes >= nnr_tc_split_bytes(R, C, algo), NNR_ERR_WORKSPACE, "nnr_tc_split_colsum: planes buffer too small");
  NNR_REQUIRE(workspace_bytes >= nnr_tc_split_colsum_workspace_bytes(R, C, algo), NNR_ERR_WORKSPACE,
              "nnr_tc_split_colsum: workspace too small");
  NNR_REQUIRE(nnr_aligned16(planes) && nnr_aligned16(workspace) && nnr_aligned16(X) && ld % 4 == 0, NNR_ERR_ALIGN,
              "nnr_tc_split_colsum: X, planes, workspace must be 16B aligned and ld %% 4 == 0");
  const int mode = algo_mode(algo);
  const int Cp = (int)nnr_tc_split_pitch(C, algo);
  NNR_REQUIRE(Cp <= 4 * 256 * TCS_MAXG, NNR_ERR_UNSUPPORTED, "nnr_tc_split_colsum: more than %d columns", 4 * 256 * TCS_MAXG);
  cudaStream_t st = (cudaStream_t)stream;
  const int nblocks = (R + tcs_rows(R) - 1) / tcs_rows(R);
  void* ph = nnr_prof_begin(1, 0.0, st);
  if (mode == 1) tc_split_colsum_kernel<1, false><<<nblocks, 256, 0, st>>>(X, ld, R, C, Cp, r_dev, planes, (size_t)R * Cp, (float*)workspace, SplitPre{});
  else if (mode == 2) tc_split_colsum_kernel<2, false><<<nblocks, 256, 0, st>>>(X, ld, R, C, Cp, r_dev, planes, (size_t)R * Cp, (float*)workspace, SplitPre{});
  else tc_split_colsum_kernel<0, false><<<nblocks, 256, 0, st>>>(X, ld, R, C, Cp, r_dev, planes, (size_t)R * Cp, (float*)workspace, SplitPre{});
  nnr_prof_end(ph, st);
  NNR_LAUNCH_CHECK("tc_split_colsum_kernel");
  tc_split_colsum_reduce<<<(C + 31) / 32, 512, 0, st>>>((const float*)workspace, nblocks, R, C, Cp, r_dev, colsum, accumulate);
  NNR_LAUNCH_CHECK("tc_split_colsum_reduce");
  return 0;
}

extern "C" int nnr_relu_bwd_split_colsum(const float* dy, const float* relu_out, int64_t ld, int R, int C, float p_drop,
                                         uint64_t seed, float* dy_dropped, int algo, void* planes, size_t planes_bytes,
                                         float* colsum, int accumulate, void* workspace, size_t workspace_bytes, void* stream) {
  NNR_REQUIRE(dy && relu_out && planes && colsum && workspace && R > 0 && C > 0 && ld >= C, NNR_ERR_ARG,
              "nnr_relu_bwd_split_colsum: bad arguments");
  NNR_REQUIRE(p_drop >= 0.f && p_drop < 1.f, NNR_ERR_ARG, "nnr_relu_bwd_split_colsum: p_drop=%f", p_drop);
  NNR_REQUIRE(algo == NNR_GEMM_TC_TF32X3 || algo == NNR_GEMM_TC_BF16 || algo == NNR_GEMM_TC_BF16X3, NNR_ERR_UNSUPPORTED,
              "nnr_relu_bwd_split_colsum: planes exist only for the tensor-core GEMM algorithms");
  NNR_REQUIRE(planes_bytes >= nnr_tc_split_bytes(R, C, algo), NNR_ERR_WORKSPACE, "nnr_relu_bwd_split_colsum: planes buffer too small");
  NNR_REQUIRE(workspace_bytes >= nnr_tc_split_colsum_workspace_bytes(R, C, algo), NNR_ERR_WORKSPACE,
              "nnr_relu_bwd_split_colsum: workspace too small");
  NNR_REQUIRE(nnr_aligned16(planes) && nnr_aligned16(workspace) && nnr_aligned16(dy) && ld % 4 == 0, NNR_ERR_ALIGN,
              "nnr_relu_bwd_split_colsum: dy, planes, workspace must be 16B aligned and ld %% 4 == 0");
  const int mode = algo_mode(algo);
  const int Cp = (int)nnr_tc_split_pitch(C, algo);
  NNR_REQUIRE(Cp <= 4 * 256 * TCS_MAXG, NNR_ERR_UNSUPPORTED, "nnr_relu_bwd_split_colsum: more than %d columns", 4 * 256 * TCS_MAXG);
  cudaStream_t st = (cudaStream_t)stream;
  const int nblocks = (R + tcs_rows(R) - 1) / tcs_rows(R);
  SplitPre pre;
  pre.relu_out = relu_out; pre.dropped = dy_dropped; pre.p = p_drop; pre.inv_keep = 1.0f / (1.0f - p_drop); pre.seed = seed;
  if (mode == 1) tc_split_colsum_kernel<1, true><<<nblocks, 256, 0, st>>>(dy, ld, R, C, Cp, nullptr, planes, (size_t)R * Cp, (float*)workspace, pre);
  else if (mode == 2) tc_split_colsum_kernel<2, true><<<nblocks, 256, 0, st>>>(dy, ld, R, C, Cp, nullptr, planes, (size_t)R * Cp, (float*)workspace, pre);
  else tc_split_colsum_kernel<0, true><<<nblocks, 256, 0, st>>>(dy, ld, R, C, Cp, nullptr, planes, (size_t)R * Cp, (float*)workspace, pre);
  NNR_LAUNCH_CHECK("tc_split_colsum_kernel");
  tc_split_colsum_reduce<<<(C + 31) / 32, 512, 0, st>>>((const float*)workspace, nblocks, R, C, Cp, nullptr, colsum, accumulate);
  NNR_LAUNCH_CHECK("tc_split_colsum_reduce");
  return 0;
}

template <int MODE>
__global__ void __launch_bounds__(256) embed_gather_planes_kernel(const float* __restrict__ table, const int32_t* __restrict__ ids,
                                                                  const int32_t* __restrict__ len, const int32_t* __restrict__ off,
                                                                  int N, int L, int E, int V, int cap, int Cp, void* __restrict__ out,
                                                                  size_t plane_stride, float p, float inv_keep, uint64_t seed) {
// ... 220 lines not shown
```

### nnr_b200/engine.py

```python
import math
import os
import weakref

import torch

from . import ops
from .ops import (EPI_ADD_AUX, EPI_BIAS, EPI_BIAS_RELU_RES, EPI_BIAS_TANH, EPI_GATE, EPI_NONE)

sort_fn = torch.sort

class SeedSource:
    INDIRECT = 1 << 62
    _GOLDEN = 0x9E3779B97F4A7C15 - (1 << 64)

    def __init__(self, device):
        self.base = torch.randint(0, 2 ** 62, (1,), dtype=torch.int64).to(device)
        self.site = 0

    def advance(self):
        self.base.add_(self._GOLDEN)
        self.site = 0

    def next(self):
        self.site += 1
# ... 77 lines not shown


_weight_planes = {}
_weight_epoch = 0


grads_ready = None


def _notify(stage):
    if grads_ready is not None:
        grads_ready(stage)


def _param_grads(P, names, G):
    if _flat_grads(P, names):
        live = [k for k in names if G.get(k) is not None]
        torch._foreach_add_([P[k].grad for k in live], [G[k] for k in live])
        return (None,) * len(names)
    return tuple(G.get(k) for k in names)


def _shared_split(x, rows, cols, colsum_out=None):
    return ops.tc_split(x, rows, cols, x.stride(0), colsum_out=colsum_out)


def _fused_relu_bwd(dy, cols):
    return (ops.default_algo() != ops.ALGO_SIMT and cols <= 2048 and cols % 4 == 0 and dy.is_contiguous()
            and dy.data_ptr() % 16 == 0)


def _flat_grads(P, names):
    return all(getattr(P[k], '_nnr_flat_grad', False) and P[k].grad is not None for k in names)


def weights_changed():
    global _weight_epoch
    _weight_epoch += 1
    _weight_planes.clear()


def install_weight_planes(W, planes):
    _weight_planes[id(W)] = ((_weight_epoch, W._version, W.data_ptr(), W.shape[0], W.shape[1], W.stride(0)), planes, weakref.ref(W))


def weight_planes(W):
    if not (isinstance(W, torch.nn.Parameter) or (W.is_leaf and W.requires_grad)) or W.dim() != 2 or W.stride(1) != 1 or not W.is_cuda:
        return None
    key = id(W)
    tag = (_weight_epoch, W._version, W.data_ptr(), W.shape[0], W.shape[1], W.stride(0))
    hit = _weight_planes.get(key)
    if hit is not None and hit[0] == tag and hit[2]() is W:
        return hit[1]
    planes = ops.tc_split(W, W.shape[0], W.shape[1], W.stride(0))
    if len(_weight_planes) > 4096:
        _weight_planes.clear()
    _weight_planes[key] = (tag, planes, weakref.ref(W))
    return planes


def linear(x, W, M, m_dev=None, bias=None, epilogue=None, out=None, x_planes=None, w_planes=None, **epi):
    N, K = W.shape
    if out is None:
        out = _empty((M, N), W.device)
    if epilogue is None:
        epilogue = EPI_BIAS if bias is not None else EPI_NONE
    ops.gemm(x, W, out, M, N, K, x.stride(0) if x is not None else K, W.stride(0), out.stride(0), False, True, epilogue, bias=bias,
             m_dev=m_dev, a_planes=x_planes, b_planes=w_planes if w_planes is not None else weight_planes(W), **epi)
    return out


def matmul_nn(x, W, M, m_dev=None, out=None, x_planes=None, w_planes=None, **epi):
    N, K = W.shape
    if out is None:
        out = _empty((M, K), W.device)
    ops.gemm(x, W, out, M, K, N, x.stride(0) if x is not None else x_planes.pitch, W.stride(0), out.stride(0), False, False, m_dev=m_dev,
             a_planes=x_planes, b_planes=w_planes if w_planes is not None else weight_planes(W), **epi)
    return out


def wgrad(dy, x, M, N, K, k_dev=None, out=None, accumulate=False, dy_planes=None, x_planes=None):
    if out is None:
        out = _empty((N, K), dy.device if dy is not None else dy_planes.buf.device)
    ops.gemm(dy, x, out, N, K, M, dy.stride(0) if dy is not None else dy_planes.pitch, x.stride(0) if x is not None else K,
             out.stride(0), True, False, k_dev=k_dev,
             accumulate=accumulate, a_planes=dy_planes, b_planes=x_planes)
    return out


def split_tokens(x, cap, cols, ntok, colsum_out=None):
    return ops.tc_split(x, cap, cols, x.stride(0), ntok, colsum_out=colsum_out)


def colsum(X, M, N, m_dev=None, out=None, accumulate=False):
    if out is None:
        out = _empty((N,), X.device)
    ops.colsum(X, X.stride(0), M, N, out, accumulate, m_dev)
    return out


CNE_PARAM_NAMES = (
    ['word_embedding.weight', 'category_embedding.weight', 'subCategory_embedding.weight']
    + ['%s_lstm.%s_l0%s' % (x, w, s) for x in ('title', 'content') for s in ('', '_reverse')
       for w in ('weight_ih', 'weight_hh', 'bias_ih', 'bias_hh')]
    + ['%s_%s' % (x, w) for x in ('title', 'content') for w in ('H.weight', 'M.weight', 'M.bias')]
    + ['%s_self_attention.%s' % (x, w) for x in ('title', 'content') for w in ('affine1.weight', 'affine1.bias', 'affine2.weight')]
)
CNE_CROSS_PARAM_NAMES = ['%s_cross_attention.%s' % (x, w) for x in ('title', 'content') for w in ('K.weight', 'Q.weight', 'Q.bias')]
CNE_GATE_PARAM_NAMES = ['%s_%s' % (x, w) for x in ('title', 'content') for w in ('H.weight', 'M.weight', 'M.bias')]


def cne_param_names(cross_attention=True, gate=True, modalities=('title', 'content')):
    single = len(modalities) == 1
    names = [n for n in CNE_PARAM_NAMES if (gate and not single) or n not in CNE_GATE_PARAM_NAMES]
    names += CNE_CROSS_PARAM_NAMES if (cross_attention and not single) else []
    if single:
        drop = 'content_' if modalities[0] == 'title' else 'title_'
        names = [n for n in names if not n.startswith(drop)]
    return names


class _Mod:
    pass


def _sort_desc(keys, max_key):
    if sort_fn is torch.sort and keys.is_cuda and keys.numel() <= 8192 and max_key <= 1024:
        return ops.length_sort_desc(keys.contiguous(), max_key)
    return sort_fn(keys, descending=True)[1]


def _domain_sorts(len64, domains, max_key):
    sorted_idx, desorted_idx = [], []
    for start, count in domains:
        si = _sort_desc(len64[start:start + count], max_key)
        di = torch.empty_like(si).scatter_(0, si, torch.arange(count, device=si.device))
        sorted_idx.append(si + start)
        desorted_idx.append(di)
    return sorted_idx, desorted_idx


def _cne_prepare(ids, mask_u8, N, L, domains):
    dev = ids.device
    cap = N * L
    m = _Mod()
    m.L, m.cap, m.ids = L, cap, ids
    m.len = _empty((N,), dev, torch.int32)
    m.off = _empty((N + 1,), dev, torch.int32)
    m.tok_row = _empty((cap,), dev, torch.int32)
    ops.seq_prepare(mask_u8, m.len, m.off, m.tok_row)
    m.ntok = m.off[N:]
    len64 = m.len.long()
    m.sorted_idx, m.desorted_idx = _domain_sorts(len64, domains, L)
    if len(domains) == 1:
        m.order = m.sorted_idx[0].to(torch.int32)
    else:
        m.order = _sort_desc(len64, L).to(torch.int32)
    return m


def _cne_recurrent(P, x, m, N, E, Hd, training, p_drop, seed, want_h_planes=False):
    dev = m.ids.device
    ids, L, cap = m.ids, m.L, m.cap
    m.seed = seed
    m.p = p_drop if training else 0.0
    table = P['word_embedding.weight']
    fused_planes = ops.default_algo() != ops.ALGO_SIMT and E % 4 == 0 and table.data_ptr() % 16 == 0
    if fused_planes:
        m.emb = None
        m.emb_pl = ops.embed_gather_planes_fwd(table, ids, m.len, m.off, cap, m.p, seed)
# ... 182 lines not shown
            return matmul_nn(dq, P[ca + 'Q.weight'], N, epilogue=EPI_ADD_AUX, aux=d_out[other[x]], ldaux=D2, x_planes=dq_pl)

        if cross:
            r = staged(cross_bwd)
            d_self = {'content': r['title'], 'title': r['content']}

        def self_gate_bwd(x, m, d_self_x):
            sa = x + '_self_attention.'
            dU = _empty((m.cap, A), dev)
            dw2p = _empty((N, A), dev)
            ops.attn_pool_bwd(X=m.hg, ldx=D2, D=D2, S=N, max_len=m.L, mode=0, seg_off=m.off, seg_order=m.order, U=m.u, ldu=A, A=A,
                              w2=P[sa + 'affine2.weight'], alpha=m.alpha_self, dpooled=d_self_x, lddp=D2, dX=m.dhg,
                              lddx=D2, accumulate_dx=dhg_written[x], dU=dU, lddu=A, dw2_partial=dw2p)
            G[sa + 'affine2.weight'] = colsum(dw2p, N, A).view(1, A)
            db1 = _empty((A,), dev)
            dU_pl = split_tokens(dU, m.cap, A, m.ntok, colsum_out=db1)
            matmul_nn(dU, P[sa + 'affine1.weight'], m.cap, m.ntok, out=m.dhg, accumulate=True, x_planes=dU_pl)
            G[sa + 'affine1.weight'] = lanes.leaf(wgrad, dU, m.hg, m.cap, A, D2, k_dev=m.ntok, dy_planes=dU_pl, x_planes=m.hg_pl)
            G[sa + 'affine1.bias'] = db1
            lanes.keep.extend((dU, dU_pl, m.hg_pl))
            m.hg_pl = None
            if not gate:
                m.dh = m.dhg
                return None
            dh0 = _empty((m.cap, D2), dev)
            dmproj = _empty((N, D2), dev)
            if ops.default_algo() != ops.ALGO_SIMT:
                dz = None
                dz_pl = ops.gate_bwd_planes(m.dhg, m.h, m.g, m.off, N, D2, m.cap, dh0, dmproj)
            else:
                dz = _empty((m.cap, D2), dev)
                ops.gate_bwd_pre(m.dhg, m.h, m.g, m.cap * D2, m.ntok, D2, dz, dh0)
                dz_pl = split_tokens(dz, m.cap, D2, m.ntok)
                ops.segment_colsum(dz, D2, m.off, N, D2, dmproj, D2)
            m.dh = matmul_nn(dz, P[x + '_H.weight'], m.cap, m.ntok, epilogue=EPI_ADD_AUX, aux=dh0, ldaux=D2, out=m.dhg,
                             x_planes=dz_pl)
            G[x + '_H.weight'] = lanes.leaf(wgrad, dz, m.h, m.cap, D2, D2, k_dev=m.ntok, dy_planes=dz_pl, x_planes=m.h_pl)
            lanes.keep.extend((m.h_pl, dz, dz_pl))
            m.h_pl = None
            dbm = _empty((D2,), dev)
            dmproj_pl = _shared_split(dmproj, N, D2, colsum_out=dbm)
            G[x + '_M.weight'] = wgrad(dmproj, m.cm_sel, N, D2, D2, dy_planes=dmproj_pl, x_planes=m.cm_sel_pl)
            G[x + '_M.bias'] = dbm
            return matmul_nn(dmproj, P[x + '_M.weight'], N, x_planes=dmproj_pl)

        d_cm_sel = staged(self_gate_bwd, d_self)
        if gate:
            dcn = {'content': d_cm_sel['title'].index_select(0, c.partner),
                   'title': d_cm_sel['content'].index_select(0, t.partner)}
        else:
            dcn = {x: torch.zeros(N, D2, device=dev) for x in mods}

        in_place = _flat_grads(P, ctx.names) and wemb.grad.is_contiguous() and wemb.grad.data_ptr() % 16 == 0
        dtable = wemb.grad if in_place else _empty(wemb.shape, dev)
        first = [not in_place]

        def recurrence_bwd(x, m, dcn_x):
            db = _empty((8 * Hd,), dev)
            if m.emb is None and ops.lstm_bwd_planes_supported(Hd):
                dz = None
                dz_pl = ops.lstm_bwd_planes(m.gates, m.c_stash, m.w_hh, m.len, m.off, m.order, N, m.L, Hd, m.dh,
                                            dcn_x.contiguous(), m.cap, db)
            else:
                ops.lstm_bwd(m.gates, m.c_stash, m.w_hh, m.len, m.off, m.order, N, m.L, Hd, m.dh, dcn_x.contiguous())
                dz = m.gates
                dz_pl = split_tokens(dz, m.cap, 8 * Hd, m.ntok, colsum_out=db)
            demb = matmul_nn(dz, m.w_ih, m.cap, m.ntok, x_planes=dz_pl, w_planes=m.w_ih_pl)
            return dz, dz_pl, db, demb

        def scatter(x, m, demb):
            ops.embed_gather_bwd(demb, m.ids, m.len, m.off, dtable, m.p, m.seed, not first[0])
            first[0] = False

        def shifted_h(m, planes):
            if planes:
                return None, ops.lstm_shift_h_planes(m.h, m.len, m.off, m.tok_row, N, m.L, Hd, m.cap)
            hprev = _empty((m.cap, D2), dev)
            ops.lstm_shift_h(m.h, m.len, m.off, m.tok_row, N, m.L, Hd, hprev)
            return hprev, None

        def weight_grads(x, m, dz, dz_pl, db, hp=None):
            pre = x + '_lstm.'
            hprev, hprev_pl = hp if hp is not None else shifted_h(m, dz_pl is not None and Hd % 8 == 0)
            for d, sfx in enumerate(('', '_reverse')):
                G[pre + 'weight_hh_l0' + sfx] = wgrad(dz[:, d * 4 * Hd:(d + 1) * 4 * Hd] if dz is not None else None,
                                                     hprev[:, d * Hd:(d + 1) * Hd] if hprev is not None else None,
                                                     m.cap, 4 * Hd, Hd, k_dev=m.ntok,
                                                     dy_planes=dz_pl.cols(d * 4 * Hd, (d + 1) * 4 * Hd) if dz_pl else None,
                                                     x_planes=hprev_pl.cols(d * Hd, (d + 1) * Hd) if hprev_pl else None)
            dwih = wgrad(dz, m.emb, m.cap, 8 * Hd, E, k_dev=m.ntok, dy_planes=dz_pl, x_planes=m.emb_pl)
            lanes.keep.extend((m.emb_pl, hprev, hprev_pl))
            m.emb_pl = None
            for d, sfx in enumerate(('', '_reverse')):
                G[pre + 'weight_ih_l0' + sfx] = dwih[d * 4 * Hd:(d + 1) * 4 * Hd]
                G[pre + 'bias_ih_l0' + sfx] = db[d * 4 * Hd:(d + 1) * 4 * Hd]
                G[pre + 'bias_hh_l0' + sfx] = db[d * 4 * Hd:(d + 1) * 4 * Hd]

        if single:
            x = modalities[0]
            dz, dz_pl, db, demb = recurrence_bwd(x, mods[x], dcn[x])
            scatter(x, mods[x], demb)
            weight_grads(x, mods[x], dz, dz_pl, db)
        else:
            lanes.fork()
            planes = t.emb is None and ops.lstm_bwd_planes_supported(Hd)
            thp = lanes.on_side(shifted_h, t, planes)
            dz, dz_pl, db, demb = recurrence_bwd('content', c, dcn['content'])
            tz, tz_pl, tdb, tdemb = lanes.on_side(recurrence_bwd, 'title', t, dcn['title'])
            lanes.on_side(scatter, 'title', t, tdemb)
            lanes.fork(2, after=1)
            lanes.on_side(weight_grads, 'title', t, tz, tz_pl, tdb, thp, lane=2)
            lanes.keep.extend((tz, tz_pl, tdemb, dz, dz_pl, demb, thp))
            lanes.fork()
            lanes.on_side(scatter, 'content', c, demb)
            if in_place:
                lanes.on_side(_notify, 'table')
            weight_grads('content', c, dz, dz_pl, db)
        lanes.join()
        G['word_embedding.weight'] = None if in_place else dtable
        ctx.t = ctx.c = None
        pg = _param_grads(P, ctx.names, G)
        if in_place:
            _notify('cne')
            if single:
                _notify('table')
        return (None,) * 7 + pg


def _gcn_param_names(L, layer_norm=False):
    names = []
    for l in range(L):
        names += ['gcn.gcn_layers.%d.W.weight' % l, 'gcn.gcn_layers.%d.W.bias' % l]
        if layer_norm:
            names += ['gcn.gcn_layers.%d.layer_normalization.weight' % l, 'gcn.gcn_layers.%d.layer_normalization.bias' % l]
    return names


def sue_param_names(L, layer_norm=False):
    return (['proxy_node_embedding'] + _gcn_param_names(L, layer_norm)
            + ['intraCluster_K.weight', 'intraCluster_Q.weight', 'intraCluster_Q.bias', 'clusterFeatureAffine.weight',
               'clusterFeatureAffine.bias', 'interClusterAttention.K.weight', 'interClusterAttention.Q.weight',
               'interClusterAttention.Q.bias'])


def sue_wo_gcn_param_names():
    return ['intraCluster_K.weight', 'intraCluster_K.bias', 'intraCluster_Q.weight', 'intraCluster_Q.bias',
            'clusterFeatureAffine.weight', 'clusterFeatureAffine.bias', 'interClusterAttention.K.weight',
            'interClusterAttention.Q.weight', 'interClusterAttention.Q.bias']


def sue_wo_hca_param_names(L, layer_norm=False):
    return (['proxy_node_embedding'] + _gcn_param_names(L, layer_norm)
            + ['attention.affine1.weight', 'attention.affine1.bias', 'attention.affine2.weight'])


def sue_names(meta):
    gcn, ln = meta.get('gcn', True), meta.get('layer_norm', False)
    L = meta['gcn_layers'] if gcn else 0
    return (sue_param_names(L, ln) if meta['hca'] else sue_wo_hca_param_names(L, ln)) if gcn else sue_wo_gcn_param_names()


class SUEFunction(torch.autograd.Function):

    @staticmethod
    def forward(ctx, meta, hist, cand, graph, cmask, cidx, *params):
        hca = meta['hca']
        gcn = meta.get('gcn', True)
        L = meta['gcn_layers'] if gcn else 0
        names = sue_names(meta)
        P = dict(zip(names, params))
        B, H, D = hist.shape
        n = cand.shape[1]
        C = P['proxy_node_embedding'].shape[0] if gcn else meta['category_num']
        Gn, C1 = H + C, C + 1
        dev = hist.device
        training, p = meta['training'], meta['p_drop']
        pe = p if training else 0.0
        seeds = [fresh_seed() for _ in range(L + 2)] if pe > 0 else [0] * (L + 2)
        hist = hist.contiguous()
        cand = cand.contiguous()
        if not gcn:
            return SUEFunction._clusters_forward(ctx, meta, P, names, hist, cand, cmask, cidx, seeds, (B, H, D, n, C, Gn, C1), L, pe)
        lanes = Lanes(dev)
        pre = None
        if hca:
            lanes.fork()
            pre = lanes.on_side(SUEFunction._cand_side, P, cand, B, n, D)
        gfeat, graph, xs, rs, aggs, lns = SUEFunction._gcn(meta, P, hist, graph, seeds, L, pe)
        ctx.meta, ctx.P, ctx.names = meta, P, names
        ctx.dims = (B, H, D, n, C, Gn, C1)
        ctx.seeds, ctx.graph = seeds, graph
        ctx.xs, ctx.rs, ctx.aggs, ctx.lns = xs, rs, aggs, lns
        ctx.gfeat, ctx.cand = gfeat, cand
        if not hca:
            pooled, ctx.u, ctx.alpha = SUEFunction._history_pool(P, gfeat)
            return pooled.unsqueeze(1).repeat(1, n, 1)
        lanes.join()
        return SUEFunction._clusters_tail(ctx, P, gfeat, cand, cmask, cidx, seeds, (B, H, D, n, C, Gn, C1), L, pe, pre)

    @staticmethod
# ... 300 lines not shown
```

### nnr_b200/ops.py

```python
import ctypes as C

import torch

from . import _lib
from ._lib import GemmArgs, PoolArgs, check, lib

EPI_NONE, EPI_BIAS, EPI_BIAS_TANH, EPI_BIAS_RELU_RES, EPI_GATE, EPI_ADD_AUX = range(6)
ALGO_AUTO, ALGO_SIMT, ALGO_TF32X3, ALGO_BF16, ALGO_BF16X3 = range(5)

_F32, _I32, _I64, _U8 = torch.float32, torch.int32, torch.int64, torch.uint8


def _p(t, dtype=None):
    if t is None:
        return None
    if not t.is_cuda:
        raise RuntimeError('nnr_b200 ops need CUDA tensors (no CPU fallback)')
    if dtype is not None and t.dtype != dtype:
        if not (dtype == _U8 and t.dtype == torch.bool):
            raise RuntimeError('nnr_b200: expected %s, got %s' % (dtype, t.dtype))
    return t.data_ptr()


_raw_stream = getattr(torch._C, '_cuda_getCurrentRawStream', None)
# ... 61 lines not shown

    def ptr(self):
        return self.buf.data_ptr() + self.col_off * self.esz

    def cols(self, a, b):
        return Planes(self.buf, self.rows, b - a, self.pitch, self.esz, self.col_off + a)


def default_algo():
    return int(lib.nnr_gemm_default_algo())


def planes_empty(rows, cols, device):
    algo = default_algo()
    if algo not in (ALGO_BF16, ALGO_BF16X3):
        return None
    buf = torch.empty(int(lib.nnr_tc_split_bytes(rows, cols, algo)), dtype=torch.uint8, device=device)
    return Planes(buf, rows, cols, int(lib.nnr_tc_split_pitch(cols, algo)), 2)


def tc_split(x, rows, cols, ld, r_dev=None, colsum_out=None, accumulate=False):
    algo = default_algo()
    if algo == ALGO_SIMT:
        if colsum_out is not None:
            colsum(x, ld, rows, cols, colsum_out, accumulate, r_dev)
        return None
    nbytes = int(lib.nnr_tc_split_bytes(rows, cols, algo))
    buf = torch.empty(nbytes, dtype=torch.uint8, device=x.device)
    if colsum_out is not None and cols <= 2048 and ld % 4 == 0 and x.data_ptr() % 16 == 0:
        wsb = int(lib.nnr_tc_split_colsum_workspace_bytes(rows, cols, algo))
        ws = workspace(wsb, x.device, 'split_colsum')
        check(lib.nnr_tc_split_colsum(_p(x, _F32), ld, rows, cols, _p(r_dev, _I32), algo, buf.data_ptr(), nbytes,
                                      _p(colsum_out, _F32), int(accumulate), ws.data_ptr(), ws.numel(), _stream()),
              'nnr_tc_split_colsum')
        return Planes(buf, rows, cols, int(lib.nnr_tc_split_pitch(cols, algo)), 2 if algo in (ALGO_BF16, ALGO_BF16X3) else 4)
    if colsum_out is not None:
        colsum(x, ld, rows, cols, colsum_out, accumulate, r_dev)
    check(lib.nnr_tc_split(_p(x, _F32), ld, rows, cols, _p(r_dev, _I32), algo, buf.data_ptr(), nbytes, _stream()),
          'nnr_tc_split')
    return Planes(buf, rows, cols, int(lib.nnr_tc_split_pitch(cols, algo)), 2 if algo in (ALGO_BF16, ALGO_BF16X3) else 4)


def relu_bwd_split_colsum(dy, relu_out, rows, cols, p_drop, seed, dy_dropped, colsum_out):
    algo = default_algo()
    nbytes = int(lib.nnr_tc_split_bytes(rows, cols, algo))
    buf = torch.empty(nbytes, dtype=torch.uint8, device=dy.device)
    wsb = int(lib.nnr_tc_split_colsum_workspace_bytes(rows, cols, algo))
    ws = workspace(wsb, dy.device, 'split_colsum')
    check(lib.nnr_relu_bwd_split_colsum(_p(dy, _F32), _p(relu_out, _F32), dy.stride(0), rows, cols, float(p_drop), int(seed),
                                        _p(dy_dropped, _F32), algo, buf.data_ptr(), nbytes, _p(colsum_out, _F32), 0,
                                        ws.data_ptr(), ws.numel(), _stream()), 'nnr_relu_bwd_split_colsum')
    return Planes(buf, rows, cols, int(lib.nnr_tc_split_pitch(cols, algo)), 2 if algo in (ALGO_BF16, ALGO_BF16X3) else 4)


class SplitMany:

    def __init__(self, mats):
        import ctypes as C_
        from ._lib import SplitDesc
        self.algo = default_algo()
        self.planes = []
        self.n = 0
        if self.algo == ALGO_SIMT or not mats:
            return
        dev = mats[0].device
        arr = (SplitDesc * len(mats))()
        esz = 2 if self.algo in (ALGO_BF16, ALGO_BF16X3) else 4
        for i, w in enumerate(mats):
            rows, cols = w.shape
            pitch = int(lib.nnr_tc_split_pitch(cols, self.algo))
            buf = torch.empty(int(lib.nnr_tc_split_bytes(rows, cols, self.algo)), dtype=torch.uint8, device=dev)
            arr[i].src, arr[i].ld, arr[i].rows, arr[i].cols = w.data_ptr(), w.stride(0), rows, cols
            arr[i].planes, arr[i].pitch = buf.data_ptr(), pitch
            self.planes.append(Planes(buf, rows, cols, pitch, esz))
        raw = bytes(arr)
        self.descs = torch.frombuffer(bytearray(raw), dtype=torch.uint8).to(dev)
        self.n = len(mats)

    def refresh(self):
        if self.n:
            check(lib.nnr_tc_split_many(self.descs.data_ptr(), self.n, self.algo, _stream()), 'nnr_tc_split_many')


def gemm(A, B, Cout, M, N, K, lda, ldb, ldc, transA, transB, epilogue=EPI_NONE, accumulate=False, bias=None,
         aux=None, ldaux=0, aux_out=None, ldaux_out=0, rowbias=None, ldrowbias=0, rowmap=None, m_dev=None,
         k_dev=None, p_drop=0.0, seed=0, algo=ALGO_AUTO, a_planes=None, b_planes=None, c_planes=None):
    a = GemmArgs()
    a.A, a.lda, a.transA = _p(A, _F32), lda, int(transA)
    a.B, a.ldb, a.transB = _p(B, _F32), ldb, int(transB)
    a.C, a.ldc = _p(Cout, _F32), ldc
    a.M, a.N, a.K = M, N, K
    a.m_dev, a.k_dev = _p(m_dev, _I32), _p(k_dev, _I32)
    a.epilogue, a.accumulate = epilogue, int(accumulate)
    a.bias = _p(bias, _F32)
    a.aux, a.ldaux = _p(aux, _F32), ldaux
    a.aux_out, a.ldaux_out = _p(aux_out, _F32), ldaux_out
    a.rowbias, a.ldrowbias, a.rowmap = _p(rowbias, _F32), ldrowbias, _p(rowmap, _I32)
    a.p_drop, a.seed, a.algo = float(p_drop), int(seed), algo
    if a_planes is not None and algo == ALGO_AUTO:
        a.A_planes, a.a_planes_pitch, a.a_planes_rows = a_planes.ptr(), a_planes.pitch, a_planes.rows
    if b_planes is not None and algo == ALGO_AUTO:
        a.B_planes, a.b_planes_pitch, a.b_planes_rows = b_planes.ptr(), b_planes.pitch, b_planes.rows
    if c_planes is not None:
        a.C_planes, a.c_planes_pitch, a.c_planes_rows = c_planes.ptr(), c_planes.pitch, c_planes.rows
    nbytes = lib.nnr_gemm_workspace_bytes(C.byref(a))
    if nbytes:
        ws = workspace(nbytes, Cout.device, 'gemm')
        a.workspace, a.workspace_bytes = ws.data_ptr(), ws.numel()
    check(lib.nnr_gemm(C.byref(a), _stream()), 'nnr_gemm')


def colsum(X, ldx, M, N, out, accumulate=False, m_dev=None):
    nbytes = lib.nnr_colsum_workspace_bytes(M, N)
    ws = workspace(nbytes, X.device, 'colsum')
    check(lib.nnr_colsum(_p(X, _F32), ldx, M, N, _p(m_dev, _I32), _p(out, _F32), int(accumulate), ws.data_ptr(),
                         ws.numel(), _stream()), 'nnr_colsum')


def length_sort_desc(len64, max_key):
    N = len64.numel()
    out = torch.empty(N, dtype=torch.int64, device=len64.device)
    check(lib.nnr_length_sort_desc(_p(len64, _I64), N, int(max_key), _p(out, _I64), _stream()), 'nnr_length_sort_desc')
    return out


def segment_colsum(X, ldx, off, N, D, out, ldo):
    check(lib.nnr_segment_colsum(_p(X, _F32), ldx, _p(off, _I32), N, D, _p(out, _F32), ldo, _stream()),
          'nnr_segment_colsum')


def _tile_counters(dev):
    return workspace(64, dev, 'lstm_counters').view(torch.int32)


def lstm_fwd(gx, w_hh, len_, off, order, N, L, H, h_out, c_stash, c_n):
    check(lib.nnr_lstm_fwd(_p(gx, _F32), _p(w_hh, _F32), _p(len_, _I32), _p(off, _I32), _p(order, _I32), N, L, H,
                           _p(h_out, _F32), _p(c_stash, _F32), _p(c_n, _F32), _tile_counters(gx.device).data_ptr(),
                           _stream()), 'nnr_lstm_fwd')


def lstm_fwd_planes_supported(H):
    return bool(lib.nnr_lstm_fwd_planes_supported(H, default_algo()))


def lstm_fwd_planes(gx, w_hh, len_, off, order, N, L, H, h_out, c_stash, c_n, cap):
    algo = default_algo()
    nbytes = int(lib.nnr_tc_split_bytes(cap, 2 * H, algo))
    buf = torch.empty(nbytes, dtype=torch.uint8, device=gx.device)
    check(lib.nnr_lstm_fwd_planes(_p(gx, _F32), _p(w_hh, _F32), _p(len_, _I32), _p(off, _I32), _p(order, _I32), N, L, H,
                                  _p(h_out, _F32), _p(c_stash, _F32), _p(c_n, _F32), _tile_counters(gx.device).data_ptr(), cap, algo,
                                  buf.data_ptr(), nbytes, _stream()), 'nnr_lstm_fwd_planes')
    return Planes(buf, cap, 2 * H, int(lib.nnr_tc_split_pitch(2 * H, algo)), 2)


def lstm_bwd(gates, c_stash, w_hh, len_, off, order, N, L, H, dh, dcn):
    check(lib.nnr_lstm_bwd(_p(gates, _F32), _p(c_stash, _F32), _p(w_hh, _F32), _p(len_, _I32), _p(off, _I32),
                           _p(order, _I32), N, L, H, _p(dh, _F32), _p(dcn, _F32), _tile_counters(gates.device).data_ptr(),
                           _stream()), 'nnr_lstm_bwd')


def lstm_bwd_planes_supported(H):
    return bool(lib.nnr_lstm_bwd_planes_supported(H, default_algo()))


def lstm_bwd_planes(gates, c_stash, w_hh, len_, off, order, N, L, H, dh, dcn, cap, db):
    algo = default_algo()
    nbytes = int(lib.nnr_tc_split_bytes(cap, 8 * H, algo))
    buf = torch.empty(nbytes, dtype=torch.uint8, device=gates.device)
    wsb = int(lib.nnr_lstm_bwd_planes_workspace_bytes(N, H))
    ws = workspace(wsb, gates.device, 'lstm_db')
    check(lib.nnr_lstm_bwd_planes(_p(gates, _F32), _p(c_stash, _F32), _p(w_hh, _F32), _p(len_, _I32), _p(off, _I32),
                                  _p(order, _I32), N, L, H, _p(dh, _F32), _p(dcn, _F32),
                                  _tile_counters(gates.device).data_ptr(), cap, algo, buf.data_ptr(), nbytes, _p(db, _F32),
                                  ws.data_ptr(), ws.numel(), _stream()), 'nnr_lstm_bwd_planes')
    return Planes(buf, cap, 8 * H, int(lib.nnr_tc_split_pitch(8 * H, algo)), 2)


def lstm_shift_h(h, len_, off, tok_row, N, L, H, hprev):
    check(lib.nnr_lstm_shift_h(_p(h, _F32), _p(len_, _I32), _p(off, _I32), _p(tok_row, _I32), N, L, H,
                               _p(hprev, _F32), _stream()), 'nnr_lstm_shift_h')


def lstm_shift_h_planes(h, len_, off, tok_row, N, L, H, cap):
    algo = default_algo()
    nbytes = int(lib.nnr_tc_split_bytes(cap, 2 * H, algo))
    buf = torch.empty(nbytes, dtype=torch.uint8, device=h.device)
    check(lib.nnr_lstm_shift_h_planes(_p(h, _F32), _p(len_, _I32), _p(off, _I32), _p(tok_row, _I32), N, L, H, cap, algo,
                                      buf.data_ptr(), nbytes, _stream()), 'nnr_lstm_shift_h_planes')
    return Planes(buf, cap, 2 * H, int(lib.nnr_tc_split_pitch(2 * H, algo)), 2 if algo in (ALGO_BF16, ALGO_BF16X3) else 4)


def gate_bwd_pre(dhg, h, g, n_max, n_dev, D, dz, dh0):
# ... 278 lines not shown
```

### nnr_b200/profiler.py

```python
import contextlib
import ctypes
import json
import os

import torch

from . import _lib, ops

_KERNEL_TAGS = ['gemm_tc_kernel', 'tc_split_kernel', 'tc_splitk_reduce_kernel', 'gemm_simt_kernel']


def _tc_class(M, N, K, transA, transB, m_dev, k_dev):
    if os.environ.get('NNR_GEMM_ALGO') == 'simt':
        return False
    if float(M) * N * K < 2.0e6 or K < 8:
        return False
    if m_dev is not None and transA:
        return False
    if k_dev is not None and not (transA and not transB):
        return False
    return True

_TIMED = ['seq_prepare', 'embed_gather_fwd', 'embed_gather_planes_fwd', 'embed_gather_bwd', 'gemm', 'colsum', 'segment_colsum', 'lstm_fwd', 'lstm_fwd_planes',
          'lstm_bwd', 'lstm_bwd_planes', 'lstm_shift_h', 'lstm_shift_h_planes', 'gate_bwd_pre', 'gate_bwd_planes', 'attn_pool_fwd', 'attn_pool_bwd', 'news_fuse_fwd', 'news_fuse_bwd', 'news_fuse_split_bwd', 'news_fuse_tables_bwd',
          'graph_to_csr', 'gcn_aggregate', 'cluster_intra_fwd', 'cluster_intra_bwd', 'rowdot_fwd', 'rowdot_bwd',
          'dropout', 'flat_clip_adam', 'sue_graph_build', 'relu_bwd_split_colsum']


def _dev_int(t):
    return int(t.item()) if t is not None else None


class Capture:
    def __init__(self):
        self.records = []
        self.t0 = self.t1 = None

    def _work(self, name, args, kw):
        if name == 'gemm':
            A, B, C, M, N, K = args[:6]
            m_dev, k_dev = kw.get('m_dev'), kw.get('k_dev')
            tc = _tc_class(M, N, K, args[9], args[10], m_dev, k_dev)
            return lambda: (2.0 * (min(M, _dev_int(m_dev)) if m_dev is not None else M) * N *
                            (min(K, _dev_int(k_dev)) if k_dev is not None else K), None, tc)
        if name in ('lstm_fwd', 'lstm_fwd_planes', 'lstm_bwd', 'lstm_bwd_planes'):
            if name in ('lstm_fwd', 'lstm_fwd_planes'):
                off, N, H = args[3], args[5], args[7]
            else:
                off, N, H = args[4], args[6], args[8]
            return lambda: (2.0 * 4 * H * H * 2 * int(off[N].item()), None)
        if name in ('embed_gather_fwd', 'embed_gather_planes_fwd'):
            table, ids, len_, off = args[:4]
            E = table.shape[1]
            return lambda: (None, float(off[ids.shape[0]].item()) * (4 + 8 * E))
        if name == 'embed_gather_bwd':
            dout, ids, len_, off, dtable = args[:5]
            V, E = dtable.shape
            return lambda: (None, float(off[ids.shape[0]].item()) * (4 + 4 * E) + V * E * 4.0)
        if name in ('attn_pool_fwd', 'attn_pool_bwd'):
            S, D, A = kw['S'], kw['D'], kw.get('A', 0) or 0
            seg_off, fixed = kw.get('seg_off'), kw.get('fixed_len', 0)
            mode0 = kw.get('mode') == 0
            fwd = name == 'attn_pool_fwd'
            acc = bool(kw.get('accumulate_dx', False))

            def pool_bytes():
                rows = float(seg_off[S].item()) if seg_off is not None else float(S * fixed)
                per_row = D * 4 + (A * 4 if mode0 else 0) + 4
                if not fwd:
                    per_row += D * 4 * (2 if acc else 1) + (A * 4 if mode0 else 0)
                return (None, rows * per_row + S * D * 4.0)
            return pool_bytes
        if name == 'colsum':
            X, ldx, M, N = args[:4]
            m_dev = kw.get('m_dev', args[6] if len(args) > 6 else None)
            return lambda: (None, (min(M, _dev_int(m_dev)) if m_dev is not None else M) * N * 4.0)
        if name == 'flat_clip_adam':
            n = args[0].numel()
            return lambda: (None, n * 28.0)
        if name == 'gcn_aggregate':
            B, Gn, D = args[4], args[5], args[6]
            return lambda: (None, 2.0 * B * Gn * D * 4)
        return lambda: (None, None)

    def wrap(self, name, fn):
        def wrapped(*args, **kw):
            e0, e1 = torch.cuda.Event(enable_timing=True), torch.cuda.Event(enable_timing=True)
            work = self._work(name, args, kw)
            e0.record()
            r = fn(*args, **kw)
            e1.record()
            label = name
            if name == 'gemm':
                label = 'gemm[%dx%dx%d %s%s e%d]' % (args[3], args[4], args[5], 'T' if args[9] else 'N', 'T' if args[10] else 'N',
                                                   kw.get('epilogue', args[11] if len(args) > 11 else 0))
            alias = {'embed_gather_planes_fwd': 'embed_gather_fwd', 'lstm_bwd_planes': 'lstm_bwd', 'lstm_fwd_planes': 'lstm_fwd', 'lstm_shift_h_planes': 'lstm_shift_h',
                     'gate_bwd_planes': 'gate_bwd_pre'}
            self.records.append((alias.get(name, name), e0, e1, work, label))
            return r
        return wrapped

    def summary(self, steps=1):
        torch.cuda.synchronize()
        agg = {}
        self.detail = {}
        tc_flops = simt_flops = 0.0
        for name, e0, e1, work, label in self.records:
            ms = e0.elapsed_time(e1)
            w = work()
            fl, by = w[0], w[1]
            if name == 'gemm':
                if w[2]:
                    tc_flops += fl
                else:
                    simt_flops += fl
            for key, table in ((name, agg), (label, self.detail)):
                a = table.setdefault(key, {'ms': 0.0, 'calls': 0, 'flops': 0.0, 'bytes': 0.0})
                a['ms'] += ms
                a['calls'] += 1
                a['flops'] += fl or 0.0
                a['bytes'] += by or 0.0
        self.detail = {k: {'ms': round(a['ms'] / steps, 3), 'calls': a['calls'] / steps,
                           'tflops': round(a['flops'] / max(a['ms'], 1e-9) / 1e9, 1)}
                       for k, a in sorted(self.detail.items(), key=lambda kv: -kv[1]['ms']) if k.startswith('gemm[')}
        buf = (ctypes.c_double * (3 * len(_KERNEL_TAGS)))()
        _lib.lib.nnr_profile_read(buf, len(_KERNEL_TAGS))
        if 'gemm' in agg:
            agg['gemm (op total: split + main + reduce)'] = agg.pop('gemm')
            agg['gemm (op total: split + main + reduce)']['flops'] = 0.0
        for i, tag in enumerate(_KERNEL_TAGS):
            if buf[3 * i + 1] > 0:
                agg[tag] = {'ms': buf[3 * i], 'calls': buf[3 * i + 1], 'bytes': 0.0,
                            'flops': tc_flops if tag == 'gemm_tc_kernel' else (simt_flops if tag == 'gemm_simt_kernel' else 0.0)}
        out = {}
        for k, a in sorted(agg.items(), key=lambda kv: -kv[1]['ms'] if not kv[0].startswith('gemm (op') else 1.0):
            out[k] = {'ms': a['ms'] / steps, 'calls': a['calls'] / steps}
            if a['flops']:
                out[k]['tflops'] = a['flops'] / (a['ms'] * 1e-3) / 1e12
            if a['bytes']:
                out[k]['gbs'] = a['bytes'] / (a['ms'] * 1e-3) / 1e9
        return out


@contextlib.contextmanager
def capture():
    from . import engine
    cap = Capture()
    _lib.lib.nnr_profile_enable(1)
    saved = {}
    lanes_were = engine.concurrent
    engine.concurrent = False
    for name in _TIMED:
        saved[name] = getattr(ops, name)
        setattr(ops, name, cap.wrap(name, saved[name]))
    try:
        yield cap
    finally:
        _lib.lib.nnr_profile_enable(0)
        engine.concurrent = lanes_were
        for name, fn in saved.items():
            setattr(ops, name, fn)


def measured_peaks(root):
    path = os.path.join(root, 'MEASURED_PEAKS.json')
    if os.path.isfile(path):
        with open(path) as f:
            p = json.load(f)
        return {'hbm_gbs': p['hbm_gbs'], 'bf16_tflops': p.get('bf16_tflops_sustained', p['bf16_tflops']), 'source': 'measured'}
    return {'hbm_gbs': 6650.0, 'bf16_tflops': 1400.0, 'source': 'fallback'}


def _ncu_traffic(root, kernel):
    path = os.path.join(root, 'profiles', 'traffic.json')
    if not os.path.isfile(path):
        return None
    with open(path) as f:
        entry = json.load(f).get(kernel)
    return entry['dram_bytes_per_launch'] if entry else None


def _ncu_traffic_source(root, kernel):
    path = os.path.join(root, 'profiles', 'traffic.json')
    if not os.path.isfile(path):
        return None
    with open(path) as f:
        entry = json.load(f).get(kernel)
    return ('static: ' + entry['source']) if entry else None


def roofline(breakdown, tokens_per_step, batch, root):
    if not breakdown:
        return None
    name, top = next(iter(breakdown.items()))
# ... 43 lines not shown
```

Baseline: 9688.

## Group LSTM weight-gradient GEMMs into a single persistent tensor-core launch

Adds a grouped weight-gradient entry point that runs up to four transposed-A GEMMs sharing one K and token count in a single persistent tcgen05 kernel. Work units from all problems are spread over one grid through a per-CTA schedule table. The backward pass uses it to merge the two hh-weight grads and the ih-weight grad per LSTM, and reorders side-stream work so the shifted-h for the content LSTM is computed on a side lane. The aim is fewer launches and better SM fill for small split-K wgrad GEMMs, at the cost of a more complex scheduler and larger kernel parameters.

```diff
diff --git a/include/nnr_b200.h b/include/nnr_b200.h
--- a/include/nnr_b200.h
+++ b/include/nnr_b200.h
@@ -7,7 +7,7 @@
 extern "C" {
 #endif
 
-#define NNR_ABI_VERSION 8
+#define NNR_ABI_VERSION 9
 #define NNR_SEED_INDIRECT (1ULL << 62)
 
 const char* nnr_last_error(void);
@@ -68,6 +68,9 @@
 } nnr_gemm_args;
 size_t nnr_gemm_workspace_bytes(const nnr_gemm_args* args);
 int nnr_gemm(const nnr_gemm_args* args, void* stream);
+#define NNR_WGRAD_GROUP_MAX 4
+size_t nnr_wgrad_group_workspace_bytes(const nnr_gemm_args* args, int n);
+int nnr_wgrad_group(const nnr_gemm_args* args, int n, void* workspace, size_t workspace_bytes, void* stream);
 int64_t nnr_tc_split_pitch(int C, int algo);
 size_t nnr_tc_split_bytes(int R, int C, int algo);
 int nnr_tc_split(const float* X, int64_t ld, int R, int C, const int32_t* r_dev, int algo, void* planes,
diff --git a/nnr_b200/_lib.py b/nnr_b200/_lib.py
--- a/nnr_b200/_lib.py
+++ b/nnr_b200/_lib.py
@@ -65,6 +65,8 @@
     'nnr_embed_gather_bwd': (C.c_int, [vp, vp, vp, vp, C.c_int, C.c_int, C.c_int, C.c_int, f32, u64, vp, C.c_int, vp, sz, vp]),
     'nnr_gemm_workspace_bytes': (sz, [C.POINTER(GemmArgs)]),
     'nnr_gemm': (C.c_int, [C.POINTER(GemmArgs), vp]),
+    'nnr_wgrad_group_workspace_bytes': (sz, [C.POINTER(GemmArgs), C.c_int]),
+    'nnr_wgrad_group': (C.c_int, [C.POINTER(GemmArgs), C.c_int, vp, sz, vp]),
     'nnr_tc_split_pitch': (i64, [C.c_int, C.c_int]),
     'nnr_tc_split_bytes': (sz, [C.c_int, C.c_int, C.c_int]),
     'nnr_tc_split': (C.c_int, [vp, i64, C.c_int, C.c_int, vp, C.c_int, vp, sz, vp]),
diff --git a/nnr_b200/csrc/gemm_api.cu b/nnr_b200/csrc/gemm_api.cu
--- a/nnr_b200/csrc/gemm_api.cu
+++ b/nnr_b200/csrc/gemm_api.cu
@@ -8,6 +8,8 @@
 int nnr_gemm_tc_supported(const nnr_gemm_args* a);
 size_t nnr_gemm_tc_workspace_bytes(const nnr_gemm_args* a);
 int nnr_gemm_tc(const nnr_gemm_args* a, void* stream);
+int nnr_gemm_tc_split_k(const nnr_gemm_args* a);
+int nnr_gemm_tc_group(const nnr_gemm_args* a, int n, void* stream);
 
 extern "C" int nnr_gemm_default_algo(void);
 static int default_algo() {
@@ -72,3 +74,55 @@
   b.algo = algo;
   return nnr_gemm_tc(&b, stream);
 }
+
+static int validate_group(const nnr_gemm_args* a, int n) {
+  NNR_REQUIRE(a && n >= 1 && n <= NNR_WGRAD_GROUP_MAX, NNR_ERR_ARG, "nnr_wgrad_group: need 1 <= n <= %d problems", NNR_WGRAD_GROUP_MAX);
+  for (int g = 0; g < n; ++g) {
+    int rc = validate(&a[g]);
+    if (rc) return rc;
+    NNR_REQUIRE(a[g].transA && !a[g].transB, NNR_ERR_ARG, "nnr_wgrad_group: problem %d: weight gradients take transA = 1, transB = 0", g);
+    NNR_REQUIRE(a[g].k_dev, NNR_ERR_ARG, "nnr_wgrad_group: problem %d: k_dev (device token count) is required", g);
+    NNR_REQUIRE(a[g].k_dev == a[0].k_dev && a[g].K == a[0].K, NNR_ERR_ARG, "nnr_wgrad_group: problem %d: K / k_dev differ from problem 0", g);
+    NNR_REQUIRE(a[g].algo == a[0].algo, NNR_ERR_ARG, "nnr_wgrad_group: problem %d: algo differs from problem 0", g);
+    NNR_REQUIRE(!a[g].m_dev && !a[g].C_planes, NNR_ERR_ARG, "nnr_wgrad_group: problem %d: m_dev and C_planes are not supported", g);
+  }
+  return 0;
+}
+
+static bool in_group_launch(const nnr_gemm_args* a, nnr_gemm_args* b) {
+  *b = *a;
+  b->algo = pick_algo(a);
+  return b->algo != NNR_GEMM_SIMT_FP32 && nnr_gemm_tc_supported(a) && nnr_gemm_tc_split_k(b);
+}
+
+static size_t up1024(size_t x) { return (x + 1023) & ~(size_t)1023; }
+
+extern "C" size_t nnr_wgrad_group_workspace_bytes(const nnr_gemm_args* args, int n) {
+  if (validate_group(args, n)) return 0;
+  size_t o = 0;
+  for (int g = 0; g < n; ++g) o = up1024(o + nnr_gemm_workspace_bytes(&args[g]));
+  return o;
+}
+
+extern "C" int nnr_wgrad_group(const nnr_gemm_args* args, int n, void* workspace, size_t workspace_bytes, void* stream) {
+  int rc = validate_group(args, n);
+  if (rc) return rc;
+  const size_t need = nnr_wgrad_group_workspace_bytes(args, n);
+  NNR_REQUIRE(need == 0 || (workspace && workspace_bytes >= need), NNR_ERR_WORKSPACE, "nnr_wgrad_group: workspace %zu < %zu",
+              workspace_bytes, need);
+  NNR_REQUIRE(nnr_aligned16(workspace), NNR_ERR_ALIGN, "nnr_wgrad_group: workspace must be 16B aligned");
+  nnr_gemm_args grp[NNR_WGRAD_GROUP_MAX];
+  int ng = 0;
+  size_t o = 0;
+  for (int g = 0; g < n; ++g) {
+    const size_t bytes = nnr_gemm_workspace_bytes(&args[g]);
+    nnr_gemm_args b;
+    const bool grouped = in_group_launch(&args[g], &b);
+    b.workspace = bytes ? (char*)workspace + o : nullptr;
+    b.workspace_bytes = bytes;
+    o = up1024(o + bytes);
+    if (grouped) grp[ng++] = b;
+    else if ((rc = nnr_gemm(&b, stream))) return rc;
+  }
+  return ng ? nnr_gemm_tc_group(grp, ng, stream) : 0;
+}
diff --git a/nnr_b200/csrc/gemm_tc.cu b/nnr_b200/csrc/gemm_tc.cu
--- a/nnr_b200/csrc/gemm_tc.cu
+++ b/nnr_b200/csrc/gemm_tc.cu
@@ -138,21 +138,32 @@
 #define TC_STAMP(i) {}
 #endif
 
-struct TcParams {
-  int M, N, K;
-  const int32_t* m_dev;
-  const int32_t* k_dev;
-  int block_n, stages, nplanes;
-  int a_mn, b_mn;
+#define TC_GROUP_MAX NNR_WGRAD_GROUP_MAX
+struct TcProb {
+  int M, N;
+  int block_n;
   int split_k;
   int chain_kb;
   uint32_t idesc;
   float* partial;
+  EpiP epi;
+};
+struct TcParams {
+  int K;
+  const int32_t* m_dev;
+  const int32_t* k_dev;
+  int ng;
+  int stages, nplanes;
+  uint32_t stage_bytes;
+  int a_mn, b_mn;
   int epi_fast;
   __nv_bfloat16* c_planes;
   long long c_pitch, c_pstride;
   int c_lo, c_rows;
-  EpiP epi;
+  TcProb pr[TC_GROUP_MAX];
+};
+struct TcMaps {
+  CUtensorMap a[TC_GROUP_MAX], b[TC_GROUP_MAX];
 };
 
 __device__ __forceinline__ bool al16(const void* p) { return (((uintptr_t)p) & 15) == 0; }
@@ -251,19 +262,19 @@
   int row0;
 };
 template <int EP>
-__device__ __forceinline__ void epi_load_in(const TcParams& p, const EpiTile& t, int n, bool has_bias, bool need_ax, bool acc_early,
+__device__ __forceinline__ void epi_load_in(const TcProb& q, const EpiTile& t, int n, bool has_bias, bool need_ax, bool acc_early,
                                             float4 (&ax)[4], float4 (&rb)[4], float4& bb) {
   bb = make_float4(0.f, 0.f, 0.f, 0.f);
 #pragma unroll
   for (int i = 0; i < 4; ++i) { ax[i] = make_float4(0.f, 0.f, 0.f, 0.f); rb[i] = make_float4(0.f, 0.f, 0.f, 0.f); }
-  if (n < p.N) {
-    if (has_bias) bb = __ldg(reinterpret_cast<const float4*>(p.epi.bias + n));
+  if (n < q.N) {
+    if (has_bias) bb = __ldg(reinterpret_cast<const float4*>(q.epi.bias + n));
 #pragma unroll
     for (int i = 0; i < 4; ++i) {
       if (t.rvalid & (1u << i)) {
-        if (need_ax) ax[i] = __ldg(reinterpret_cast<const float4*>(p.epi.aux + t.o_aux[i] + n));
-        else if (acc_early) ax[i] = *reinterpret_cast<const float4*>(p.epi.C + t.o_c[i] + n);
-        if (EP == NNR_EPI_GATE) rb[i] = __ldg(reinterpret_cast<const float4*>(p.epi.rowbias + t.o_rb[i] + n));
+        if (need_ax) ax[i] = __ldg(reinterpret_cast<const float4*>(q.epi.aux + t.o_aux[i] + n));
+        else if (acc_early) ax[i] = *reinterpret_cast<const float4*>(q.epi.C + t.o_c[i] + n);
+        if (EP == NNR_EPI_GATE) rb[i] = __ldg(reinterpret_cast<const float4*>(q.epi.rowbias + t.o_rb[i] + n));
       }
     }
   }
@@ -271,17 +282,17 @@
 
 #define TC_EPK_PARTIAL 6
 template <int EP>
-__device__ __forceinline__ void epi_tile_fast(const TcParams& p, const EpiTile& t, uint32_t lane_addr, bool has_k, int c_begin, int c_end,
+__device__ __forceinline__ void epi_tile_fast(const TcParams& p, const TcProb& q, const EpiTile& t, uint32_t lane_addr, bool has_k, int c_begin, int c_end,
                                               int n0, uint32_t tile_s, int lane, int M, uint64_t drop_seed, float* __restrict__ Cout) {
   const int tr = lane >> 2, tc4 = (lane & 3) * 4;
   constexpr bool PARTIAL = EP == TC_EPK_PARTIAL;
   constexpr bool BIASED = EP == NNR_EPI_BIAS || EP == NNR_EPI_BIAS_TANH || EP == NNR_EPI_BIAS_RELU_RES;
-  const bool has_bias = BIASED && p.epi.bias != nullptr;
-  const bool need_ax = EP == NNR_EPI_GATE || EP == NNR_EPI_ADD_AUX || (EP == NNR_EPI_BIAS_RELU_RES && p.epi.aux != nullptr);
-  const bool accumulate = !PARTIAL && p.epi.accumulate != 0;
+  const bool has_bias = BIASED && q.epi.bias != nullptr;
+  const bool need_ax = EP == NNR_EPI_GATE || EP == NNR_EPI_ADD_AUX || (EP == NNR_EPI_BIAS_RELU_RES && q.epi.aux != nullptr);
+  const bool accumulate = !PARTIAL && q.epi.accumulate != 0;
   const bool acc_early = accumulate && !need_ax;
   const bool planes = !PARTIAL && p.c_planes != nullptr;
-  const bool drop = EP == NNR_EPI_BIAS_RELU_RES && p.epi.p_drop > 0.f;
+  const bool drop = EP == NNR_EPI_BIAS_RELU_RES && q.epi.p_drop > 0.f;
   const uint32_t my_row = tile_s + (uint32_t)lane * TC_EPI_PITCH;
   const uint32_t rd_row = tile_s + (uint32_t)tr * TC_EPI_PITCH + (uint32_t)tc4 * 4;
 
@@ -289,11 +300,11 @@
   uint32_t r[16];
   float4 ax[4], rb[4], bb, axn[4], rbn[4], bbn;
   if (has_k) tmem_ld16_issue(lane_addr + (uint32_t)c_begin, r);
-  if (AHEAD) epi_load_in<EP>(p, t, n0 + c_begin + tc4, has_bias, need_ax, acc_early, ax, rb, bb);
+  if (AHEAD) epi_load_in<EP>(q, t, n0 + c_begin + tc4, has_bias, need_ax, acc_early, ax, rb, bb);
   for (int c0 = c_begin; c0 < c_end; c0 += 16) {
     const bool more = c0 + 16 < c_end;
-    if (AHEAD) { if (more) epi_load_in<EP>(p, t, n0 + c0 + 16 + tc4, has_bias, need_ax, acc_early, axn, rbn, bbn); }
-    else epi_load_in<EP>(p, t, n0 + c0 + tc4, has_bias, need_ax, acc_early, ax, rb, bb);
+    if (AHEAD) { if (more) epi_load_in<EP>(q, t, n0 + c0 + 16 + tc4, has_bias, need_ax, acc_early, axn, rbn, bbn); }
+    else epi_load_in<EP>(q, t, n0 + c0 + tc4, has_bias, need_ax, acc_early, ax, rb, bb);
     if (has_k) tmem_ld16_wait(r);
     else {
 #pragma unroll
@@ -307,7 +318,7 @@
 #pragma unroll
     for (int i = 0; i < 4; ++i) o[i] = lds128(rd_row + (uint32_t)(8 * i) * TC_EPI_PITCH);
     const int n = n0 + c0 + tc4;
-    if (n < p.N) {
+    if (n < q.N) {
 #pragma unroll
       for (int i = 0; i < 4; ++i) {
         if (!(t.rvalid & (1u << i))) continue;
@@ -316,18 +327,18 @@
           v.x = tanh_fast(v.x); v.y = tanh_fast(v.y); v.z = tanh_fast(v.z); v.w = tanh_fast(v.w);
         } else if (EP == NNR_EPI_BIAS_RELU_RES) {
           v.x = fmaxf(v.x, 0.f); v.y = fmaxf(v.y, 0.f); v.z = fmaxf(v.z, 0.f); v.w = fmaxf(v.w, 0.f);
-          if (p.epi.aux_out) *reinterpret_cast<float4*>(p.epi.aux_out + t.o_ao[i] + n) = v;
+          if (q.epi.aux_out) *reinterpret_cast<float4*>(q.epi.aux_out + t.o_ao[i] + n) = v;
           if (need_ax) { v.x += ax[i].x; v.y += ax[i].y; v.z += ax[i].z; v.w += ax[i].w; }
           if (drop) {
-            const uint64_t e0 = (uint64_t)(t.row0 + 8 * i) * (uint64_t)p.epi.N + n;
+            const uint64_t e0 = (uint64_t)(t.row0 + 8 * i) * (uint64_t)q.epi.N + n;
             float ks[4];
-            dropout_scale4(drop_seed, e0 >> 2, p.epi.p_drop, p.epi.inv_keep, ks);
+            dropout_scale4(drop_seed, e0 >> 2, q.epi.p_drop, q.epi.inv_keep, ks);
             v.x *= ks[0]; v.y *= ks[1]; v.z *= ks[2]; v.w *= ks[3];
           }
         } else if (EP == NNR_EPI_GATE) {
           v.x = sigmoid_fast(v.x + rb[i].x); v.y = sigmoid_fast(v.y + rb[i].y);
           v.z = sigmoid_fast(v.z + rb[i].z); v.w = sigmoid_fast(v.w + rb[i].w);
-          if (p.epi.aux_out) *reinterpret_cast<float4*>(p.epi.aux_out + t.o_ao[i] + n) = v;
+          if (q.epi.aux_out) *reinterpret_cast<float4*>(q.epi.aux_out + t.o_ao[i] + n) = v;
           v.x *= ax[i].x; v.y *= ax[i].y; v.z *= ax[i].z; v.w *= ax[i].w;
         } else if (EP == NNR_EPI_ADD_AUX) {
           v.x += ax[i].x; v.y += ax[i].y; v.z += ax[i].z; v.w += ax[i].w;
@@ -375,31 +386,45 @@
   }
 }
 
+struct TcGroupTab {
+  int m_tiles[TC_GROUP_MAX], n_tiles[TC_GROUP_MAX], splits[TC_GROUP_MAX], kb_per[TC_GROUP_MAX], M[TC_GROUP_MAX], wsum[TC_GROUP_MAX];
+  int total;
+};
+struct TcUnit { int g, m_idx, n_idx, z; };
+__device__ __forceinline__ TcUnit tc_unit(const TcGroupTab& t, int ng, int u) {
+  TcUnit r;
+  int zlo = 0, j = 0;
+  r.z = 0;
+  for (; j < ng; ++j) {
+    const int seg = (t.splits[j] - zlo) * t.wsum[j];
+    if (u < seg) { r.z = zlo + u / t.wsum[j]; u -= (r.z - zlo) * t.wsum[j]; break; }
+    u -= seg;
+    zlo = t.splits[j];
+  }
+  int g = j;
+  while (g + 1 < ng && u >= t.m_tiles[g] * t.n_tiles[g]) { u -= t.m_tiles[g] * t.n_tiles[g]; ++g; }
+  r.g = g;
+  r.m_idx = u / t.n_tiles[g];
+  r.n_idx = u - r.m_idx * t.n_tiles[g];
+  return r;
+}
+
 template <bool BF16, bool PAIR, int EPK>
-__global__ void __launch_bounds__(TC_THREADS, 1) gemm_tc_kernel(const __grid_constant__ CUtensorMap map_a,
-                                                                const __grid_constant__ CUtensorMap map_b, TcParams p) {
+__global__ void __launch_bounds__(TC_THREADS, 1) gemm_tc_kernel(const __grid_constant__ TcMaps maps, const __grid_constant__ TcParams p) {
   extern __shared__ __align__(1024) unsigned char smem_raw[];
   constexpr int KELEM = BF16 ? 64 : 32;
   constexpr int TILE_M = PAIR ? 2 * TC_BM : TC_BM;
-  int M = p.M, K = p.K;
-  if (p.m_dev) M = min(M, *p.m_dev);
+  int K = p.K;
   if (p.k_dev) K = min(K, *p.k_dev);
   const int warp = threadIdx.x >> 5, lane = threadIdx.x & 31;
   if (threadIdx.x == 0) TC_STAMP(0)
   const uint32_t rank = PAIR ? cluster_ctarank() : 0u;
   const int sched_id = PAIR ? (int)(blockIdx.x >> 1) : (int)blockIdx.x;
   const int sched_n = PAIR ? (int)(gridDim.x >> 1) : (int)gridDim.x;
-  const int b_rows = PAIR ? (p.block_n >> 1) : p.block_n;
-
-  const int m_tiles = (M + TILE_M - 1) / TILE_M;
-  const int n_tiles = (p.N + p.block_n - 1) / p.block_n;
   const int nkb = (K + KELEM - 1) / KELEM;
-  const int kb_per = p.split_k ? p.chain_kb : max(nkb, 1);
-  const int splits = p.split_k ? max(1, (nkb + kb_per - 1) / kb_per) : 1;
-  const int total_tiles = m_tiles * n_tiles * splits;
-
-  const uint32_t a_tile = TC_BM * 128, b_tile = (uint32_t)b_rows * 128;
-  const uint32_t stage_bytes = (uint32_t)p.nplanes * (a_tile + b_tile);
+
+  const uint32_t a_tile = TC_BM * 128;
+  const uint32_t stage_bytes = p.stage_bytes;
   unsigned char* tiles = (unsigned char*)(((uintptr_t)smem_raw + 1023) & ~(uintptr_t)1023);
   unsigned char* epi_scratch = tiles + (size_t)p.stages * stage_bytes;
   uint64_t* full_bar = reinterpret_cast<uint64_t*>(epi_scratch + TC_EPI_SCRATCH);
@@ -407,13 +432,31 @@
   uint64_t* tmem_full = empty_bar + p.stages;
   uint64_t* tmem_empty = tmem_full + 2;
   uint32_t* tmem_slot = reinterpret_cast<uint32_t*>(tmem_empty + 2);
+  TcGroupTab* tab = reinterpret_cast<TcGroupTab*>(tmem_empty + 4);
 
   if (warp == 0 && lane == 0) {
-    asm volatile("prefetch.tensormap [%0];" ::"l"(&map_a) : "memory");
-    asm volatile("prefetch.tensormap [%0];" ::"l"(&map_b) : "memory");
+    for (int g = 0; g < p.ng; ++g) {
+      asm volatile("prefetch.tensormap [%0];" ::"l"(&maps.a[g]) : "memory");
+      asm volatile("prefetch.tensormap [%0];" ::"l"(&maps.b[g]) : "memory");
+    }
     for (int s = 0; s < p.stages; ++s) { mbar_init(&full_bar[s], 1); mbar_init(&empty_bar[s], 1); }
     for (int b = 0; b < 2; ++b) { mbar_init(&tmem_full[b], 1); mbar_init(&tmem_empty[b], PAIR ? 16 : 8); }
     asm volatile("fence.mbarrier_init.release.cluster;" ::: "memory");
+    int total = 0;
+    for (int g = 0; g < p.ng; ++g) {
+      const TcProb& q = p.pr[g];
+      const int M = p.m_dev ? min(q.M, *p.m_dev) : q.M;
+      const int kb_per = q.split_k ? q.chain_kb : max(nkb, 1);
+      tab->M[g] = M;
+      tab->m_tiles[g] = (M + TILE_M - 1) / TILE_M;
+      tab->n_tiles[g] = (q.N + q.block_n - 1) / q.block_n;
+      tab->kb_per[g] = kb_per;
+      tab->splits[g] = q.split_k ? max(1, (nkb + kb_per - 1) / kb_per) : 1;
+      total += tab->m_tiles[g] * tab->n_tiles[g] * tab->splits[g];
+    }
+    int w = 0;
+    for (int g = p.ng - 1; g >= 0; --g) { w += tab->m_tiles[g] * tab->n_tiles[g]; tab->wsum[g] = w; }
+    tab->total = total;
   }
   if (PAIR) cluster_sync_all();
   if (warp == 1) {
@@ -429,28 +472,35 @@
   __syncthreads();
   tc_fence_after();
   const uint32_t tmem_base = *tmem_slot;
+  const int total_units = tab->total;
   if (threadIdx.x == 0) TC_STAMP(1)
 
   if (warp == 0) {
     if (lane == 0) {
       int it = 0;
-      for (int tile = sched_id; tile < total_tiles; tile += sched_n) {
-        const int n_idx = tile % n_tiles, rest = tile / n_tiles;
-        const int m0 = (rest % m_tiles) * TILE_M + (int)rank * TC_BM, n0 = n_idx * p.block_n + (int)rank * b_rows, z = rest / m_tiles;
-        const int kb0 = z * kb_per, kb1 = min(nkb, kb0 + kb_per);
+      for (int unit = sched_id; unit < total_units; unit += sched_n) {
+        const TcUnit u = tc_unit(*tab, p.ng, unit);
+        const int bn = p.pr[u.g].block_n;
+        const int b_rows = PAIR ? (bn >> 1) : bn;
+        const uint32_t b_tile = (uint32_t)b_rows * 128;
+        const uint32_t tx_bytes = (uint32_t)p.nplanes * (a_tile + b_tile);
+        const CUtensorMap* map_a = &maps.a[u.g];
+        const CUtensorMap* map_b = &maps.b[u.g];
+        const int m0 = u.m_idx * TILE_M + (int)rank * TC_BM, n0 = u.n_idx * bn + (int)rank * b_rows;
+        const int kb0 = u.z * tab->kb_per[u.g], kb1 = min(nkb, kb0 + tab->kb_per[u.g]);
         for (int kb = kb0; kb < kb1; ++kb, ++it) {
           const int s = it % p.stages;
           const uint32_t ph = (it / p.stages) & 1;
           mbar_wait(&empty_bar[s], ph ^ 1);
           const uint32_t base = smem_u32(tiles + (size_t)s * stage_bytes);
-          if (!PAIR) mbar_expect_tx(&full_bar[s], stage_bytes);
-          else if (rank == 0) mbar_expect_tx(&full_bar[s], 2 * stage_bytes);
+          if (!PAIR) mbar_expect_tx(&full_bar[s], tx_bytes);
+          else if (rank == 0) mbar_expect_tx(&full_bar[s], 2 * tx_bytes);
           const uint32_t lbar = PAIR ? mapa_rank(smem_u32(&full_bar[s]), 0) : 0u;
           auto load_a = [&](uint32_t dst, int c0, int c1, int c2) {
-            if (PAIR) tma_load_3d_pair(&map_a, lbar, dst, c0, c1, c2); else tma_load_3d(&map_a, &full_bar[s], dst, c0, c1, c2);
+            if (PAIR) tma_load_3d_pair(map_a, lbar, dst, c0, c1, c2); else tma_load_3d(map_a, &full_bar[s], dst, c0, c1, c2);
           };
           auto load_b = [&](uint32_t dst, int c0, int c1, int c2) {
-            if (PAIR) tma_load_3d_pair(&map_b, lbar, dst, c0, c1, c2); else tma_load_3d(&map_b, &full_bar[s], dst, c0, c1, c2);
+            if (PAIR) tma_load_3d_pair(map_b, lbar, dst, c0, c1, c2); else tma_load_3d(map_b, &full_bar[s], dst, c0, c1, c2);
           };
           for (int pl = 0; pl < p.nplanes; ++pl) {
             const uint32_t sa = base + pl * a_tile;
@@ -469,10 +519,11 @@
       const uint32_t lbo = KELEM * 128;
       const uint64_t a_step = p.a_mn ? (uint64_t)((BF16 ? 2048 : 1024) >> 4) : 2;
       const uint64_t b_step = p.b_mn ? (uint64_t)((BF16 ? 2048 : 1024) >> 4) : 2;
-      for (int tile = sched_id; tile < total_tiles; tile += sched_n, ++tl) {
-        const int rest = tile / n_tiles;
-        const int z = rest / m_tiles;
-        const int kb0 = z * kb_per, kb1 = min(nkb, kb0 + kb_per);
+      for (int unit = sched_id; unit < total_units; unit += sched_n, ++tl) {
+        const TcUnit u = tc_unit(*tab, p.ng, unit);
+        const uint32_t idesc = p.pr[u.g].idesc;
+        const uint32_t b_tile = (uint32_t)(PAIR ? (p.pr[u.g].block_n >> 1) : p.pr[u.g].block_n) * 128;
+        const int kb0 = u.z * tab->kb_per[u.g], kb1 = min(nkb, kb0 + tab->kb_per[u.g]);
         const int buf = tl & 1;
         mbar_wait(&tmem_empty[buf], ((tl >> 1) & 1) ^ 1);
         tc_fence_after();
@@ -493,16 +544,16 @@
 #pragma unroll
           for (int k = 0; k < 4; ++k) {
             const uint64_t ao = a_step * k, bo = b_step * k;
-            if (PAIR) tc_mma_pair<BF16>(d_tmem, a_hi + ao, b_hi + bo, p.idesc, first ? 0u : 1u);
-            else tc_mma<BF16>(d_tmem, a_hi + ao, b_hi + bo, p.idesc, first ? 0u : 1u);
+            if (PAIR) tc_mma_pair<BF16>(d_tmem, a_hi + ao, b_hi + bo, idesc, first ? 0u : 1u);
+            else tc_mma<BF16>(d_tmem, a_hi + ao, b_hi + bo, idesc, first ? 0u : 1u);
             first = 0;
             if (p.nplanes == 2) {
               if (PAIR) {
-                tc_mma_pair<BF16>(d_tmem, a_hi + ao, b_lo + bo, p.idesc, 1u);
-                tc_mma_pair<BF16>(d_tmem, a_lo + ao, b_hi + bo, p.idesc, 1u);
+                tc_mma_pair<BF16>(d_tmem, a_hi + ao, b_lo + bo, idesc, 1u);
+                tc_mma_pair<BF16>(d_tmem, a_lo + ao, b_hi + bo, idesc, 1u);
               } else {
-                tc_mma<BF16>(d_tmem, a_hi + ao, b_lo + bo, p.idesc, 1u);
-                tc_mma<BF16>(d_tmem, a_lo + ao, b_hi + bo, p.idesc, 1u);
+                tc_mma<BF16>(d_tmem, a_hi + ao, b_lo + bo, idesc, 1u);
+                tc_mma<BF16>(d_tmem, a_lo + ao, b_hi + bo, idesc, 1u);
               }
             }
           }
@@ -515,25 +566,27 @@
   } else {
     const int q = warp & 3;
     const int chalf = (warp - 2) >> 2;
-    const uint64_t drop_seed = (p.epi.p_drop > 0.f) ? nnr_resolve_seed(p.epi.seed) : 0ull;
-    const int nchunks = p.block_n >> 4;
-    const int c_begin = chalf ? ((nchunks + 1) >> 1) << 4 : 0;
-    const int c_end = chalf ? p.block_n : ((nchunks + 1) >> 1) << 4;
+    const uint64_t drop_seed = (p.pr[0].epi.p_drop > 0.f) ? nnr_resolve_seed(p.pr[0].epi.seed) : 0ull;
     int tl = 0;
-    for (int tile = sched_id; tile < total_tiles; tile += sched_n, ++tl) {
-      const int n_idx = tile % n_tiles, rest = tile / n_tiles;
-      const int m0 = (rest % m_tiles) * TILE_M + (int)rank * TC_BM, n0 = n_idx * p.block_n, z = rest / m_tiles;
-      const int kb0 = z * kb_per, kb1 = min(nkb, kb0 + kb_per);
+    for (int unit = sched_id; unit < total_units; unit += sched_n, ++tl) {
+      const TcUnit u = tc_unit(*tab, p.ng, unit);
+      const TcProb& pr = p.pr[u.g];
+      const int M = tab->M[u.g];
+      const int nchunks = pr.block_n >> 4;
+      const int c_begin = chalf ? ((nchunks + 1) >> 1) << 4 : 0;
+      const int c_end = chalf ? pr.block_n : ((nchunks + 1) >> 1) << 4;
+      const int m0 = u.m_idx * TILE_M + (int)rank * TC_BM, n0 = u.n_idx * pr.block_n, z = u.z;
+      const int kb0 = z * tab->kb_per[u.g], kb1 = min(nkb, kb0 + tab->kb_per[u.g]);
       const int buf = tl & 1;
       const uint32_t lane_addr = tmem_base + buf * TC_ACC_COLS + ((uint32_t)(q * 32) << 16);
       unsigned char* my_tile = epi_scratch + (size_t)(warp - 2) * 32 * TC_EPI_PITCH;
       const int tr = lane >> 2, tc4 = (lane & 3) * 4;
       int rmap[4] = {0, 0, 0, 0};
-      if ((EPK < 0 || EPK == NNR_EPI_GATE) && p.epi.epilogue == NNR_EPI_GATE && !p.partial) {
+      if ((EPK < 0 || EPK == NNR_EPI_GATE) && pr.epi.epilogue == NNR_EPI_GATE && !pr.partial) {
 #pragma unroll
         for (int i = 0; i < 4; ++i) {
           const int mm = m0 + q * 32 + tr + 8 * i;
-          if (mm < M) rmap[i] = __ldg(p.epi.rowmap + mm);
+          if (mm < M) rmap[i] = __ldg(pr.epi.rowmap + mm);
         }
       }
       const bool fast = EPK >= 0;
@@ -545,10 +598,10 @@
           const int mm = m0 + q * 32 + tr + 8 * i;
           if (mm < M) rvalid |= 1u << i;
           const uint32_t mr = (mm < M) ? (uint32_t)mm : 0u;
-          o_c[i] = (EPK == TC_EPK_PARTIAL) ? ((uint32_t)z * (uint32_t)M + mr) * (uint32_t)p.N : mr * (uint32_t)p.epi.ldc;
-          o_aux[i] = mr * (uint32_t)p.epi.ldaux;
-          o_ao[i] = mr * (uint32_t)p.epi.ldaux_out;
-          o_rb[i] = (uint32_t)rmap[i] * (uint32_t)p.epi.ldrowbias;
+          o_c[i] = (EPK == TC_EPK_PARTIAL) ? ((uint32_t)z * (uint32_t)M + mr) * (uint32_t)pr.N : mr * (uint32_t)pr.epi.ldc;
+          o_aux[i] = mr * (uint32_t)pr.epi.ldaux;
+          o_ao[i] = mr * (uint32_t)pr.epi.ldaux_out;
+          o_rb[i] = (uint32_t)rmap[i] * (uint32_t)pr.epi.ldrowbias;
         }
       }
       mbar_wait(&tmem_full[buf], (tl >> 1) & 1);
@@ -559,8 +612,8 @@
 #pragma unroll
         for (int i = 0; i < 4; ++i) { et.o_c[i] = o_c[i]; et.o_aux[i] = o_aux[i]; et.o_ao[i] = o_ao[i]; et.o_rb[i] = o_rb[i]; }
         et.rvalid = rvalid; et.row0 = m0 + q * 32 + tr;
-        epi_tile_fast<(EPK >= 0 ? EPK : 0)>(p, et, lane_addr, kb1 > kb0, c_begin, c_end, n0, smem_u32(my_tile), lane, M, drop_seed,
-                                            EPK == TC_EPK_PARTIAL ? p.partial : p.epi.C);
+        epi_tile_fast<(EPK >= 0 ? EPK : 0)>(p, pr, et, lane_addr, kb1 > kb0, c_begin, c_end, n0, smem_u32(my_tile), lane, M, drop_seed,
+                                            EPK == TC_EPK_PARTIAL ? pr.partial : pr.epi.C);
       } else
       for (int c0 = c_begin; c0 < c_end; c0 += 16) {
         float v[16];
@@ -574,7 +627,7 @@
           *reinterpret_cast<float4*>(my_tile + lane * TC_EPI_PITCH + qd * 16) = make_float4(v[4 * qd], v[4 * qd + 1], v[4 * qd + 2], v[4 * qd + 3]);
         __syncwarp();
         const int n = n0 + c0 + tc4;
-        const int cnt = min(4, p.N - n);
+        const int cnt = min(4, pr.N - n);
         float o[4][4];
 #pragma unroll
         for (int i = 0; i < 4; ++i) {
@@ -582,26 +635,26 @@
           o[i][0] = x.x; o[i][1] = x.y; o[i][2] = x.z; o[i][3] = x.w;
         }
         if (cnt > 0) {
-          if (p.partial) {
+          if (pr.partial) {
 #pragma unroll
             for (int i = 0; i < 4; ++i) {
               const int mm = m0 + q * 32 + tr + 8 * i;
-              if (mm < M) st4(p.partial + ((size_t)z * M + mm) * p.N + n, cnt, o[i]);
+              if (mm < M) st4(pr.partial + ((size_t)z * M + mm) * pr.N + n, cnt, o[i]);
             }
           } else {
             Epi4In in[4];
             float bias4[4] = {0.f, 0.f, 0.f, 0.f};
-            if (p.epi.bias && (p.epi.epilogue == NNR_EPI_BIAS || p.epi.epilogue == NNR_EPI_BIAS_TANH || p.epi.epilogue == NNR_EPI_BIAS_RELU_RES))
-              ld4(p.epi.bias + n, cnt, bias4);
+            if (pr.epi.bias && (pr.epi.epilogue == NNR_EPI_BIAS || pr.epi.epilogue == NNR_EPI_BIAS_TANH || pr.epi.epilogue == NNR_EPI_BIAS_RELU_RES))
+              ld4(pr.epi.bias + n, cnt, bias4);
 #pragma unroll
             for (int i = 0; i < 4; ++i) {
               const int mm = m0 + q * 32 + tr + 8 * i;
-              if (mm < M) epi_load4(p.epi, mm, n, cnt, in[i], rmap[i]);
+              if (mm < M) epi_load4(pr.epi, mm, n, cnt, in[i], rmap[i]);
             }
 #pragma unroll
             for (int i = 0; i < 4; ++i) {
               const int mm = m0 + q * 32 + tr + 8 * i;
-              if (mm < M) epi_finish4(p.epi, mm, n, o[i], cnt, bias4, in[i]);
+              if (mm < M) epi_finish4(pr.epi, mm, n, o[i], cnt, bias4, in[i]);
             }
           }
         }
@@ -626,30 +679,38 @@
   }
 }
 
-__global__ void tc_splitk_reduce_kernel(const float* __restrict__ partial, int K, const int32_t* __restrict__ k_dev, int kelem,
-                                        int chain_kb, int M, int N, const int32_t* __restrict__ m_dev, EpiP epi) {
-  if (m_dev) M = min(M, *m_dev);
-  if (k_dev) K = min(K, *k_dev);
-  const int nkb = (K + kelem - 1) / kelem;
-  const int splits = max(1, (nkb + chain_kb - 1) / chain_kb);
-  size_t i = (size_t)blockIdx.x * blockDim.x + threadIdx.x;
-  if (i >= (size_t)M * N) return;
-  int m = (int)(i / N), n = (int)(i - (size_t)m * N);
-  float acc = 0.f;
-  for (int s = 0; s < splits; ++s) acc += partial[((size_t)s * M + m) * N + n];
-  epi_store(epi, m, n, acc);
-}
-__global__ void __launch_bounds__(256) tc_splitk_reduce4_kernel(const float* __restrict__ partial, int K, const int32_t* __restrict__ k_dev,
-                                                                int kelem, int chain_kb, int M, int N, const int32_t* __restrict__ m_dev,
-                                                                EpiP epi) {
-  if (m_dev) M = min(M, *m_dev);
-  if (k_dev) K = min(K, *k_dev);
-  const int nkb = (K + kelem - 1) / kelem;
-  const int splits = max(1, (nkb + chain_kb - 1) / chain_kb);
+struct TcReduceGroup {
+  int ng, K, kelem;
+  const int32_t* k_dev;
+  const int32_t* m_dev;
+  long long item0[TC_GROUP_MAX + 1];
+  int M[TC_GROUP_MAX], N[TC_GROUP_MAX], chain_kb[TC_GROUP_MAX], vec[TC_GROUP_MAX];
+  const float* partial[TC_GROUP_MAX];
+  EpiP epi[TC_GROUP_MAX];
+};
+__global__ void __launch_bounds__(256) tc_splitk_reduce_kernel(const __grid_constant__ TcReduceGroup r) {
+  const long long i = (long long)blockIdx.x * blockDim.x + threadIdx.x;
+  int g = 0;
+  while (g + 1 < r.ng && i >= r.item0[g + 1]) ++g;
+  if (i >= r.item0[g + 1]) return;
+  const int K = r.k_dev ? min(r.K, *r.k_dev) : r.K;
+  const int M = r.m_dev ? min(r.M[g], *r.m_dev) : r.M[g], N = r.N[g];
+  const int nkb = (K + r.kelem - 1) / r.kelem;
+  const int splits = max(1, (nkb + r.chain_kb[g] - 1) / r.chain_kb[g]);
+  const float* partial = r.partial[g];
+  const EpiP& epi = r.epi[g];
+  const long long j = i - r.item0[g];
+  if (!r.vec[g]) {
+    if (j >= (long long)M * N) return;
+    const int m = (int)(j / N), n = (int)(j - (long long)m * N);
+    float acc = 0.f;
+    for (int s = 0; s < splits; ++s) acc += partial[((size_t)s * M + m) * N + n];
+    epi_store(epi, m, n, acc);
+    return;
+  }
   const int N4 = N >> 2;
-  const size_t i = (size_t)blockIdx.x * blockDim.x + threadIdx.x;
-  if (i >= (size_t)M * N4) return;
-  const int m = (int)(i / N4), n = (int)(i - (size_t)m * N4) * 4;
+  if (j >= (long long)M * N4) return;
+  const int m = (int)(j / N4), n = (int)(j - (long long)m * N4) * 4;
   const size_t plane = (size_t)M * N;
   const float* src = partial + (size_t)m * N + n;
   float4 acc = make_float4(0.f, 0.f, 0.f, 0.f);
@@ -903,8 +964,12 @@
   int a_cp, b_cp;
   int block_n, stages, split_k, chain_kb, max_splits, nplanes, kelem;
   int pair;
-  size_t a_plane, b_plane, a_off, b_off, partial_off, total, smem;
+  size_t stage, a_plane, b_plane, a_off, b_off, partial_off, total, smem;
 };
+
+static size_t tc_smem(int stages, size_t stage) {
+  return 1024 + (size_t)stages * stage + TC_EPI_SCRATCH + (2 * stages + 4) * 8 + 16 + sizeof(TcGroupTab);
+}
 
 static int pick_block_n(int N, int step, int nplanes) {
   int best = step;
@@ -973,7 +1038,8 @@
   if (stages < 2) stages = 2;
   if (stages > 6) stages = 6;
   pl.stages = stages;
-  pl.smem = 1024 + (size_t)stages * stage + TC_EPI_SCRATCH + (2 * stages + 4) * 8 + 16;
+  pl.stage = stage;
+  pl.smem = tc_smem(stages, stage);
   const size_t esz = bf16 ? 2 : 4;
   pl.a_plane = (size_t)pl.a_rows * pl.a_cp;
   pl.b_plane = (size_t)pl.b_rows * pl.b_cp;
@@ -1046,10 +1112,19 @@
   return pair ? tc_kernel_ptr2<BF16, true>(epk) : tc_kernel_ptr2<BF16, false>(epk);
 }
 
+struct TcProbHost {
+  TcPlan pl;
+  CUtensorMap map_a, map_b;
+  TcProb q;
+  int vec;
+  int partial_epk;
+};
+
 template <int MODE>
-static int run_tc(const nnr_gemm_args* a, cudaStream_t st) {
+static int tc_prepare(const nnr_gemm_args* a, cudaStream_t st, TcProbHost& h) {
   constexpr bool BF16 = MODE != 0;
-  TcPlan pl = make_plan(a, MODE);
+  TcPlan& pl = h.pl;
+  pl = make_plan(a, MODE);
   NNR_REQUIRE(pl.total == 0 || (a->workspace && a->workspace_bytes >= pl.total), NNR_ERR_WORKSPACE,
               "nnr_gemm(tc): workspace %zu < %zu", a->workspace_bytes, pl.total);
   NNR_REQUIRE(nnr_aligned16(a->workspace), NNR_ERR_ALIGN, "nnr_gemm(tc): workspace must be 16B aligned");
@@ -1074,22 +1149,107 @@
     if (rc) return rc;
     pb = w; b_pitch = pl.b_cp; b_prow = pl.b_rows;
   }
-  CUtensorMap map_a, map_b;
   const int ke = pl.kelem;
-  rc = encode_map(&map_a, pa, BF16, pl.a_cols, a_pitch, pl.a_rows, a_prow, pl.nplanes, ke, pl.a_mn ? ke : TC_BM, pl.a_mn != 0);
+  rc = encode_map(&h.map_a, pa, BF16, pl.a_cols, a_pitch, pl.a_rows, a_prow, pl.nplanes, ke, pl.a_mn ? ke : TC_BM, pl.a_mn != 0);
   if (rc) return rc;
-  rc = encode_map(&map_b, pb, BF16, pl.b_cols, b_pitch, pl.b_rows, b_prow, pl.nplanes, ke,
+  rc = encode_map(&h.map_b, pb, BF16, pl.b_cols, b_pitch, pl.b_rows, b_prow, pl.nplanes, ke,
                   pl.b_mn ? ke : (pl.pair ? pl.block_n / 2 : pl.block_n), pl.b_mn != 0);
   if (rc) return rc;
+  TcProb& q = h.q;
+  q.M = a->M; q.N = a->N;
+  q.block_n = pl.block_n; q.split_k = pl.split_k; q.chain_kb = pl.chain_kb;
+  const uint32_t fmt = BF16 ? 1u : 2u;
+  q.idesc = (1u << 4) | (fmt << 7) | (fmt << 10) | ((uint32_t)pl.a_mn << 15) | ((uint32_t)pl.b_mn << 16) |
+            ((uint32_t)(pl.block_n >> 3) << 17) | ((uint32_t)((pl.pair ? 2 * TC_BM : TC_BM) >> 4) << 24);
+  q.partial = pl.split_k ? (float*)(ws + pl.partial_off) : nullptr;
+  q.epi = make_epi(a);
+  h.vec = a->N % 4 == 0 && nnr_aligned16(q.partial);
+  h.partial_epk = BF16 && pl.split_k && a->N % 4 == 0 && nnr_aligned16(q.partial) &&
+                  (double)pl.max_splits * (double)a->M * (double)a->N < 4294967296.0;
+  return 0;
+}
+
+template <int MODE>
+static int tc_launch(TcProbHost* h, int ng, TcParams& p, int epk, const int32_t* m_dev, const int32_t* k_dev, int K, cudaStream_t st) {
+  constexpr bool BF16 = MODE != 0;
+  const bool pair = h[0].pl.pair != 0;
+  TcMaps maps;
+  p.K = K; p.m_dev = m_dev; p.k_dev = k_dev; p.ng = ng;
+  p.nplanes = h[0].pl.nplanes; p.a_mn = h[0].pl.a_mn; p.b_mn = h[0].pl.b_mn;
+  size_t stage = 0;
+  long cap_units = 0;
+  for (int g = 0; g < ng; ++g) {
+    maps.a[g] = h[g].map_a; maps.b[g] = h[g].map_b; p.pr[g] = h[g].q;
+    stage = stage > h[g].pl.stage ? stage : h[g].pl.stage;
+    cap_units += (long)((h[g].q.M + TC_BM - 1) / TC_BM) * ((h[g].q.N + h[g].pl.block_n - 1) / h[g].pl.block_n) * h[g].pl.max_splits;
+  }
+  int stages = (int)(TC_SMEM_BUDGET / stage);
+  if (stages < 2) stages = 2;
+  if (stages > 6) stages = 6;
+  p.stages = stages;
+  p.stage_bytes = (uint32_t)stage;
+  const size_t smem = tc_smem(stages, stage);
+  NNR_REQUIRE(smem <= 227 * 1024, NNR_ERR_UNSUPPORTED, "nnr_gemm(tc): smem plan too large");
+  static bool attr_set[16][2][2][8] = {};
+  static int num_sms_tab[16] = {};
+  int dev = 0;
+  NNR_CUDA(cudaGetDevice(&dev));
+  dev &= 15;
+  const void* kernel = tc_kernel_ptr<BF16>(pair, epk);
+  if (!attr_set[dev][BF16 ? 1 : 0][pair][epk + 1]) {
+    NNR_CUDA(cudaFuncSetAttribute(kernel, cudaFuncAttributeMaxDynamicSharedMemorySize, 227 * 1024));
+    attr_set[dev][BF16 ? 1 : 0][pair][epk + 1] = true;
+  }
+  if (num_sms_tab[dev] == 0) NNR_CUDA(cudaDeviceGetAttribute(&num_sms_tab[dev], cudaDevAttrMultiProcessorCount, dev));
+  const int num_sms = num_sms_tab[dev];
+  void* ph = nnr_prof_begin(0, -1.0, st);
+  {
+    cudaLaunchConfig_t cfg = {};
+    cudaLaunchAttribute attr[1];
+    if (pair) {
+      long cap_tiles = (long)((h[0].q.M + 2 * TC_BM - 1) / (2 * TC_BM)) * ((h[0].q.N + h[0].pl.block_n - 1) / h[0].pl.block_n);
+      long pairs = cap_tiles < num_sms / 2 ? cap_tiles : num_sms / 2;
+      attr[0].id = cudaLaunchAttributeClusterDimension;
+      attr[0].val.clusterDim.x = 2; attr[0].val.clusterDim.y = 1; attr[0].val.clusterDim.z = 1;
+      cfg.attrs = attr; cfg.numAttrs = 1;
+      cfg.gridDim = dim3((unsigned)(2 * pairs));
+    } else {
+      cfg.gridDim = dim3((unsigned)(cap_units < num_sms ? cap_units : num_sms));
+    }
+    cfg.blockDim = dim3(TC_THREADS); cfg.dynamicSmemBytes = smem; cfg.stream = st;
+    void* kargs[] = {(void*)&maps, (void*)&p};
+    cudaError_t e = cudaLaunchKernelExC(&cfg, kernel, kargs);
+    nnr_count_launch(1);
+    if (e != cudaSuccess) { nnr_set_error("gemm_tc_kernel(%s): launch failed: %s", pair ? "pair" : "single", cudaGetErrorString(e)); return (int)e; }
+    nnr_prof_end(ph, st);
+  }
+  TcReduceGroup r;
+  r.ng = 0; r.K = K; r.kelem = h[0].pl.kelem; r.k_dev = k_dev; r.m_dev = m_dev;
+  r.item0[0] = 0;
+  for (int g = 0; g < ng; ++g) {
+    if (!h[g].pl.split_k) continue;
+    const int j = r.ng++;
+    r.M[j] = h[g].q.M; r.N[j] = h[g].q.N; r.chain_kb[j] = h[g].pl.chain_kb; r.vec[j] = h[g].vec;
+    r.partial[j] = h[g].q.partial; r.epi[j] = h[g].q.epi;
+    r.item0[j + 1] = r.item0[j] + (long long)h[g].q.M * (h[g].vec ? h[g].q.N / 4 : h[g].q.N);
+  }
+  if (r.ng) {
+    void* ph2 = nnr_prof_begin(2, 0.0, st);
+    tc_splitk_reduce_kernel<<<(unsigned)((r.item0[r.ng] + 255) / 256), 256, 0, st>>>(r);
+    nnr_prof_end(ph2, st);
+    NNR_LAUNCH_CHECK("tc_splitk_reduce_kernel");
+  }
+  return 0;
+}
+
+template <int MODE>
+static int run_tc(const nnr_gemm_args* a, cudaStream_t st) {
+  constexpr bool BF16 = MODE != 0;
+  TcProbHost h;
+  int rc = tc_prepare<MODE>(a, st, h);
+  if (rc) return rc;
+  const TcPlan& pl = h.pl;
   TcParams p;
-  p.M = a->M; p.N = a->N; p.K = a->K; p.m_dev = a->m_dev; p.k_dev = a->k_dev;
-  p.block_n = pl.block_n; p.stages = pl.stages; p.nplanes = pl.nplanes;
-  p.a_mn = pl.a_mn; p.b_mn = pl.b_mn; p.split_k = pl.split_k; p.chain_kb = pl.chain_kb;
-  const uint32_t fmt = BF16 ? 1u : 2u;
-  p.idesc = (1u << 4) | (fmt << 7) | (fmt << 10) | ((uint32_t)pl.a_mn << 15) | ((uint32_t)pl.b_mn << 16) |
-            ((uint32_t)(pl.block_n >> 3) << 17) | ((uint32_t)((pl.pair ? 2 * TC_BM : TC_BM) >> 4) << 24);
-  p.partial = pl.split_k ? (float*)(ws + pl.partial_off) : nullptr;
-  p.epi = make_epi(a);
   {
     auto ok = [](const void* ptr, int64_t ld) { return !ptr || (nnr_aligned16(ptr) && ld % 4 == 0); };
     p.epi_fast = (a->N % 4 == 0) && ok(a->C, a->ldc) && ok(a->aux, a->ldaux) && ok(a->aux_out, a->ldaux_out) &&
@@ -1112,57 +1272,9 @@
     p.c_lo = pl.nplanes == 2;
     p.c_rows = (int)a->c_planes_rows;
   }
-  static bool attr_set[16][2][2][8] = {};
-  static int num_sms_tab[16] = {};
-  int dev = 0;
-  NNR_CUDA(cudaGetDevice(&dev));
-  dev &= 15;
   int epk = (BF16 && p.epi_fast && !pl.split_k) ? a->epilogue : -1;
-  if (BF16 && pl.split_k && a->N % 4 == 0 && nnr_aligned16(p.partial) &&
-      (double)pl.max_splits * (double)a->M * (double)a->N < 4294967296.0)
-    epk = TC_EPK_PARTIAL;
-  const void* kernel = tc_kernel_ptr<BF16>(pl.pair != 0, epk);
-  if (!attr_set[dev][BF16 ? 1 : 0][pl.pair][epk + 1]) {
-    NNR_CUDA(cudaFuncSetAttribute(kernel, cudaFuncAttributeMaxDynamicSharedMemorySize, 227 * 1024));
-    attr_set[dev][BF16 ? 1 : 0][pl.pair][epk + 1] = true;
-  }
-  if (num_sms_tab[dev] == 0) NNR_CUDA(cudaDeviceGetAttribute(&num_sms_tab[dev], cudaDevAttrMultiProcessorCount, dev));
-  const int num_sms = num_sms_tab[dev];
-  void* ph = nnr_prof_begin(0, -1.0, st);
-  {
-    cudaLaunchConfig_t cfg = {};
-    cudaLaunchAttribute attr[1];
-    if (pl.pair) {
-      long cap_tiles = (long)((a->M + 2 * TC_BM - 1) / (2 * TC_BM)) * ((a->N + pl.block_n - 1) / pl.block_n);
-      long pairs = cap_tiles < num_sms / 2 ? cap_tiles : num_sms / 2;
-      attr[0].id = cudaLaunchAttributeClusterDimension;
-      attr[0].val.clusterDim.x = 2; attr[0].val.clusterDim.y = 1; attr[0].val.clusterDim.z = 1;
-      cfg.attrs = attr; cfg.numAttrs = 1;
-      cfg.gridDim = dim3((unsigned)(2 * pairs));
-    } else {
-      long cap_tiles = (long)((a->M + TC_BM - 1) / TC_BM) * ((a->N + pl.block_n - 1) / pl.block_n) * pl.max_splits;
-      cfg.gridDim = dim3((unsigned)(cap_tiles < num_sms ? cap_tiles : num_sms));
-    }
-    cfg.blockDim = dim3(TC_THREADS); cfg.dynamicSmemBytes = pl.smem; cfg.stream = st;
-    void* kargs[] = {(void*)&map_a, (void*)&map_b, (void*)&p};
-    cudaError_t e = cudaLaunchKernelExC(&cfg, kernel, kargs);
-    nnr_count_launch(1);
-    if (e != cudaSuccess) { nnr_set_error("gemm_tc_kernel(%s): launch failed: %s", pl.pair ? "pair" : "single", cudaGetErrorString(e)); return (int)e; }
-    nnr_prof_end(ph, st);
-  }
-  if (pl.split_k) {
-    size_t tot = (size_t)a->M * a->N;
-    void* ph2 = nnr_prof_begin(2, 0.0, st);
-    if (a->N % 4 == 0 && nnr_aligned16(p.partial))
-      tc_splitk_reduce4_kernel<<<(unsigned)((tot / 4 + 255) / 256), 256, 0, st>>>(p.partial, a->K, a->k_dev, pl.kelem, pl.chain_kb, a->M,
-                                                                                 a->N, a->m_dev, p.epi);
-    else
-      tc_splitk_reduce_kernel<<<(unsigned)((tot + 255) / 256), 256, 0, st>>>(p.partial, a->K, a->k_dev, pl.kelem, pl.chain_kb, a->M,
-                                                                            a->N, a->m_dev, p.epi);
-    nnr_prof_end(ph2, st);
-    NNR_LAUNCH_CHECK("tc_splitk_reduce_kernel");
-  }
-  return 0;
+  if (h.partial_epk) epk = TC_EPK_PARTIAL;
+  return tc_launch<MODE>(&h, 1, p, epk, a->m_dev, a->k_dev, a->K, st);
 }
 
 int nnr_gemm_tc(const nnr_gemm_args* a, void* stream) {
@@ -1171,6 +1283,32 @@
   if (mode == 1) return run_tc<1>(a, st);
   if (mode == 2) return run_tc<2>(a, st);
   return run_tc<0>(a, st);
+}
+
+int nnr_gemm_tc_split_k(const nnr_gemm_args* a) { return make_plan(a, algo_mode(a->algo)).split_k; }
+
+template <int MODE>
+static int run_tc_group(const nnr_gemm_args* a, int n, cudaStream_t st) {
+  TcProbHost h[TC_GROUP_MAX];
+  for (int g = 0; g < n; ++g) {
+    int rc = tc_prepare<MODE>(&a[g], st, h[g]);
+    if (rc) return rc;
+    for (int j = g; j > 0 && h[j - 1].pl.chain_kb < h[j].pl.chain_kb; --j) { TcProbHost t = h[j]; h[j] = h[j - 1]; h[j - 1] = t; }
+  }
+  TcParams p;
+  p.epi_fast = 0;
+  p.c_planes = nullptr; p.c_pitch = 0; p.c_pstride = 0; p.c_lo = 0; p.c_rows = 0;
+  int epk = TC_EPK_PARTIAL;
+  for (int g = 0; g < n; ++g) if (!h[g].partial_epk) epk = -1;
+  return tc_launch<MODE>(h, n, p, epk, nullptr, a[0].k_dev, a[0].K, st);
+}
+
+int nnr_gemm_tc_group(const nnr_gemm_args* a, int n, void* stream) {
+  cudaStream_t st = (cudaStream_t)stream;
+  const int mode = algo_mode(a[0].algo);
+  if (mode == 1) return run_tc_group<1>(a, n, st);
+  if (mode == 2) return run_tc_group<2>(a, n, st);
+  return run_tc_group<0>(a, n, st);
 }
 
 extern "C" int64_t nnr_tc_split_pitch(int C, int algo) { return (int64_t)up((size_t)C, algo_mode(algo) ? 8 : 4); }
diff --git a/nnr_b200/engine.py b/nnr_b200/engine.py
--- a/nnr_b200/engine.py
+++ b/nnr_b200/engine.py
@@ -183,10 +183,15 @@
 def wgrad(dy, x, M, N, K, k_dev=None, out=None, accumulate=False, dy_planes=None, x_planes=None):
     if out is None:
         out = _empty((N, K), dy.device if dy is not None else dy_planes.buf.device)
-    ops.gemm(dy, x, out, N, K, M, dy.stride(0) if dy is not None else dy_planes.pitch, x.stride(0) if x is not None else K,
-             out.stride(0), True, False, k_dev=k_dev,
-             accumulate=accumulate, a_planes=dy_planes, b_planes=x_planes)
+    a, kw = wgrad_args(dy, x, M, N, K, out, k_dev, accumulate, dy_planes, x_planes)
+    ops.gemm(*a, **kw)
     return out
+
+
+def wgrad_args(dy, x, M, N, K, out, k_dev=None, accumulate=False, dy_planes=None, x_planes=None):
+    return ((dy, x, out, N, K, M, dy.stride(0) if dy is not None else dy_planes.pitch, x.stride(0) if x is not None else K,
+             out.stride(0), True, False),
+            dict(k_dev=k_dev, accumulate=accumulate, a_planes=dy_planes, b_planes=x_planes))
 
 
 def split_tokens(x, cap, cols, ntok, colsum_out=None):
@@ -535,13 +540,17 @@
         def weight_grads(x, m, dz, dz_pl, db, hp=None):
             pre = x + '_lstm.'
             hprev, hprev_pl = hp if hp is not None else shifted_h(m, dz_pl is not None and Hd % 8 == 0)
+            group = []
             for d, sfx in enumerate(('', '_reverse')):
-                G[pre + 'weight_hh_l0' + sfx] = wgrad(dz[:, d * 4 * Hd:(d + 1) * 4 * Hd] if dz is not None else None,
-                                                     hprev[:, d * Hd:(d + 1) * Hd] if hprev is not None else None,
-                                                     m.cap, 4 * Hd, Hd, k_dev=m.ntok,
-                                                     dy_planes=dz_pl.cols(d * 4 * Hd, (d + 1) * 4 * Hd) if dz_pl else None,
-                                                     x_planes=hprev_pl.cols(d * Hd, (d + 1) * Hd) if hprev_pl else None)
-            dwih = wgrad(dz, m.emb, m.cap, 8 * Hd, E, k_dev=m.ntok, dy_planes=dz_pl, x_planes=m.emb_pl)
+                G[pre + 'weight_hh_l0' + sfx] = _empty((4 * Hd, Hd), dev)
+                group.append(wgrad_args(dz[:, d * 4 * Hd:(d + 1) * 4 * Hd] if dz is not None else None,
+                                        hprev[:, d * Hd:(d + 1) * Hd] if hprev is not None else None,
+                                        m.cap, 4 * Hd, Hd, G[pre + 'weight_hh_l0' + sfx], k_dev=m.ntok,
+                                        dy_planes=dz_pl.cols(d * 4 * Hd, (d + 1) * 4 * Hd) if dz_pl else None,
+                                        x_planes=hprev_pl.cols(d * Hd, (d + 1) * Hd) if hprev_pl else None))
+            dwih = _empty((8 * Hd, E), dev)
+            group.append(wgrad_args(dz, m.emb, m.cap, 8 * Hd, E, dwih, k_dev=m.ntok, dy_planes=dz_pl, x_planes=m.emb_pl))
+            ops.wgrad_group(group)
             lanes.keep.extend((m.emb_pl, hprev, hprev_pl))
             m.emb_pl = None
             for d, sfx in enumerate(('', '_reverse')):
@@ -556,19 +565,22 @@
             weight_grads(x, mods[x], dz, dz_pl, db)
         else:
             lanes.fork()
+            lanes.fork(2)
             planes = t.emb is None and ops.lstm_bwd_planes_supported(Hd)
+            chp = lanes.on_side(shifted_h, c, ops.default_algo() != ops.ALGO_SIMT and Hd % 8 == 0, lane=2)
             thp = lanes.on_side(shifted_h, t, planes)
             dz, dz_pl, db, demb = recurrence_bwd('content', c, dcn['content'])
             tz, tz_pl, tdb, tdemb = lanes.on_side(recurrence_bwd, 'title', t, dcn['title'])
-            lanes.on_side(scatter, 'title', t, tdemb)
+            lanes.join(2)
             lanes.fork(2, after=1)
             lanes.on_side(weight_grads, 'title', t, tz, tz_pl, tdb, thp, lane=2)
-            lanes.keep.extend((tz, tz_pl, tdemb, dz, dz_pl, demb, thp))
+            lanes.on_side(scatter, 'title', t, tdemb)
+            lanes.keep.extend((tz, tz_pl, tdemb, dz, dz_pl, demb, thp, chp))
             lanes.fork()
             lanes.on_side(scatter, 'content', c, demb)
             if in_place:
                 lanes.on_side(_notify, 'table')
-            weight_grads('content', c, dz, dz_pl, db)
+            weight_grads('content', c, dz, dz_pl, db, chp)
         lanes.join()
         G['word_embedding.weight'] = None if in_place else dtable
         ctx.t = ctx.c = None
diff --git a/nnr_b200/ops.py b/nnr_b200/ops.py
--- a/nnr_b200/ops.py
+++ b/nnr_b200/ops.py
@@ -167,10 +167,11 @@
             check(lib.nnr_tc_split_many(self.descs.data_ptr(), self.n, self.algo, _stream()), 'nnr_tc_split_many')
 
 
-def gemm(A, B, Cout, M, N, K, lda, ldb, ldc, transA, transB, epilogue=EPI_NONE, accumulate=False, bias=None,
-         aux=None, ldaux=0, aux_out=None, ldaux_out=0, rowbias=None, ldrowbias=0, rowmap=None, m_dev=None,
-         k_dev=None, p_drop=0.0, seed=0, algo=ALGO_AUTO, a_planes=None, b_planes=None, c_planes=None):
-    a = GemmArgs()
+def _gemm_args(A, B, Cout, M, N, K, lda, ldb, ldc, transA, transB, epilogue=EPI_NONE, accumulate=False, bias=None,
+               aux=None, ldaux=0, aux_out=None, ldaux_out=0, rowbias=None, ldrowbias=0, rowmap=None, m_dev=None,
+               k_dev=None, p_drop=0.0, seed=0, algo=ALGO_AUTO, a_planes=None, b_planes=None, c_planes=None, a=None):
+    if a is None:
+        a = GemmArgs()
     a.A, a.lda, a.transA = _p(A, _F32), lda, int(transA)
     a.B, a.ldb, a.transB = _p(B, _F32), ldb, int(transB)
     a.C, a.ldc = _p(Cout, _F32), ldc
@@ -188,11 +189,25 @@
         a.B_planes, a.b_planes_pitch, a.b_planes_rows = b_planes.ptr(), b_planes.pitch, b_planes.rows
     if c_planes is not None:
         a.C_planes, a.c_planes_pitch, a.c_planes_rows = c_planes.ptr(), c_planes.pitch, c_planes.rows
+    return a
+
+
+def gemm(A, B, Cout, M, N, K, lda, ldb, ldc, transA, transB, *rest, **kw):
+    a = _gemm_args(A, B, Cout, M, N, K, lda, ldb, ldc, transA, transB, *rest, **kw)
     nbytes = lib.nnr_gemm_workspace_bytes(C.byref(a))
     if nbytes:
         ws = workspace(nbytes, Cout.device, 'gemm')
         a.workspace, a.workspace_bytes = ws.data_ptr(), ws.numel()
     check(lib.nnr_gemm(C.byref(a), _stream()), 'nnr_gemm')
+
+
+def wgrad_group(problems):
+    arr = (GemmArgs * len(problems))()
+    for i, (args, kw) in enumerate(problems):
+        _gemm_args(*args, a=arr[i], **kw)
+    nbytes = lib.nnr_wgrad_group_workspace_bytes(arr, len(problems))
+    ws = workspace(nbytes, problems[0][0][2].device, 'gemm')
+    check(lib.nnr_wgrad_group(arr, len(problems), ws.data_ptr(), ws.numel(), _stream()), 'nnr_wgrad_group')
 
 
 def colsum(X, ldx, M, N, out, accumulate=False, m_dev=None):
diff --git a/nnr_b200/profiler.py b/nnr_b200/profiler.py
--- a/nnr_b200/profiler.py
+++ b/nnr_b200/profiler.py
@@ -24,7 +24,7 @@
 _TIMED = ['seq_prepare', 'embed_gather_fwd', 'embed_gather_planes_fwd', 'embed_gather_bwd', 'gemm', 'colsum', 'segment_colsum', 'lstm_fwd', 'lstm_fwd_planes',
           'lstm_bwd', 'lstm_bwd_planes', 'lstm_shift_h', 'lstm_shift_h_planes', 'gate_bwd_pre', 'gate_bwd_planes', 'attn_pool_fwd', 'attn_pool_bwd', 'news_fuse_fwd', 'news_fuse_bwd', 'news_fuse_split_bwd', 'news_fuse_tables_bwd',
           'graph_to_csr', 'gcn_aggregate', 'cluster_intra_fwd', 'cluster_intra_bwd', 'rowdot_fwd', 'rowdot_bwd',
-          'dropout', 'flat_clip_adam', 'sue_graph_build', 'relu_bwd_split_colsum']
+          'dropout', 'flat_clip_adam', 'sue_graph_build', 'relu_bwd_split_colsum', 'wgrad_group']
 
 
 def _dev_int(t):
@@ -43,6 +43,13 @@
             tc = _tc_class(M, N, K, args[9], args[10], m_dev, k_dev)
             return lambda: (2.0 * (min(M, _dev_int(m_dev)) if m_dev is not None else M) * N *
                             (min(K, _dev_int(k_dev)) if k_dev is not None else K), None, tc)
+        if name == 'wgrad_group':
+            parts = [self._work('gemm', a, k) for a, k in args[0]]
+
+            def group_work():
+                w = [p() for p in parts]
+                return (sum(x[0] for x in w), None, all(x[2] for x in w))
+            return group_work
         if name in ('lstm_fwd', 'lstm_fwd_planes', 'lstm_bwd', 'lstm_bwd_planes'):
             if name in ('lstm_fwd', 'lstm_fwd_planes'):
                 off, N, H = args[3], args[5], args[7]
@@ -109,7 +116,7 @@
             ms = e0.elapsed_time(e1)
             w = work()
             fl, by = w[0], w[1]
-            if name == 'gemm':
+            if name in ('gemm', 'wgrad_group'):
                 if w[2]:
                     tc_flops += fl
                 else:
```

Result: slower. 9354, median of 6 (-3.4%).
